# elizabethfong/SparkSmithWaterman

Hardware: AMD Instinct MI355X
Metric: GCUPS (higher is better)
Workload: dtype int32

## Files before the change

### include/swmi.h

```cpp
#ifndef SWMI_H
#define SWMI_H

#include <stddef.h>
#include <stdint.h>

#ifdef __cplusplus
extern "C" {
#endif

#define SWMI_ABI_VERSION 3

typedef enum swmi_status {
    SWMI_OK               =  0,
    SWMI_ERR_INVALID      = -1,
    SWMI_ERR_NO_DEVICE    = -2,
    SWMI_ERR_HIP          = -3,
    SWMI_ERR_NOMEM        = -4,
    SWMI_ERR_UNSUPPORTED  = -5,
    SWMI_ERR_RANGE        = -6
} swmi_status;

#define SWMI_ALIGN_LOCAL  0
#define SWMI_ALIGN_FIT    1
#define SWMI_ALIGN_GLOBAL 2

#define SWMI_TIE_SERIAL 0
#define SWMI_TIE_STRICT 1

typedef struct swmi_params {
    int32_t match;
    int32_t mismatch;
    int32_t gap;
    int32_t tie_mode;
    char    types[4];
} swmi_params;

typedef struct swmi_ctx    swmi_ctx;
typedef struct swmi_batch  swmi_batch;

int         swmi_abi_version(void);
const char *swmi_last_error(void);
int         swmi_device_count(int *count);
int         swmi_create(int device, swmi_ctx **out);
void        swmi_destroy(swmi_ctx *ctx);
void        swmi_default_params(swmi_params *p);

int         swmi_set_option(swmi_ctx *ctx, const char *name, int64_t value);

int         swmi_set_score_matrix(swmi_ctx *ctx, const uint8_t *alphabet, uint32_t n, const int32_t *scores);

int  swmi_batch_upload(swmi_ctx *ctx,
                       const uint8_t *ref_bytes, const uint64_t *ref_off, uint32_t n_refs,
                       const uint8_t *read_bytes, const uint64_t *read_off, uint32_t n_reads,
                       swmi_batch **out);
#define SWMI_SPEC_REVERSE 0x1u
#define SWMI_SPEC_WHOLE   0xFFFFFFFFu
typedef struct swmi_pair_spec {
    uint32_t ref, read;
    uint32_t ref_start, ref_len;
    uint32_t read_start, read_len;
    uint32_t flags;
    uint32_t reserved;
} swmi_pair_spec;
int  swmi_batch_upload_pairs(swmi_ctx *ctx,
                             const uint8_t *ref_bytes, const uint64_t *ref_off, uint32_t n_refs,
                             const uint8_t *read_bytes, const uint64_t *read_off, uint32_t n_reads,
                             const swmi_pair_spec *specs, uint64_t n_pairs, swmi_batch **out);
int  swmi_batch_set_pairs(swmi_ctx *ctx, swmi_batch *b, const swmi_pair_spec *specs, uint64_t n_pairs);
int  swmi_batch_pair_spec(const swmi_batch *b, uint64_t pair, swmi_pair_spec *spec);

int  swmi_batch_run(swmi_ctx *ctx, swmi_batch *b, const swmi_params *p);
void swmi_batch_free(swmi_ctx *ctx, swmi_batch *b);
int  swmi_batch_run_async(swmi_ctx *ctx, swmi_batch *b, const swmi_params *p);
int  swmi_batch_wait(swmi_ctx *ctx);

typedef struct swmi_timing {
    float    fill_ms, traceback_ms, d2h_ms, total_ms;
    uint32_t fill_launches, rerun_pairs;
    uint64_t cells;
    uint64_t dir_bytes;
    uint32_t strip_fallbacks;
    uint32_t col_chunks;
    uint32_t resident_pairs;
    uint32_t tfused_pairs;
} swmi_timing;
int  swmi_batch_timing(const swmi_batch *b, swmi_timing *t);
int  swmi_batch_mode(const swmi_batch *b, int *mode);

#define SWMI_PAIR_DEGENERATE 0x1u
#define SWMI_PAIR_TO_END     0x2u
uint64_t swmi_batch_n_pairs(const swmi_batch *b);
int      swmi_pair_score(const swmi_batch *b, uint64_t pair, int32_t *score);
int      swmi_pair_n_alignments(const swmi_batch *b, uint64_t pair, uint64_t *n, uint32_t *flags);
int      swmi_pair_rows_swept(const swmi_batch *b, uint64_t pair, uint32_t *rows);
int      swmi_pair_band_window(const swmi_batch *b, uint64_t pair, uint32_t strip, uint32_t *c_lo, uint32_t *c_hi);
int      swmi_batch_pair_results(const swmi_batch *b, int32_t *scores, uint64_t *n_alignments, uint64_t n);
int      swmi_pair_alignment(swmi_batch *b, uint64_t pair, uint64_t k,
                             int32_t *begin, int32_t *end_i, int32_t *end_j,
                             const char **ref_aln, const char **read_aln, uint32_t *len);
#define SWMI_CIGAR_M  0u
#define SWMI_CIGAR_I  1u
#define SWMI_CIGAR_D  2u
#define SWMI_CIGAR_EQ 7u
#define SWMI_CIGAR_X  8u
int      swmi_pair_cigar(swmi_batch *b, uint64_t pair, uint64_t k,
                         int32_t *begin, int32_t *end_i, int32_t *end_j,
                         const uint32_t **cigar, uint32_t *n_cigar, uint32_t *nm);

#define SWMI_SUBOPT_AUTO (-1)
int      swmi_pair_subopt(const swmi_batch *b, uint64_t pair, int32_t *score2, uint32_t *end2);
int      swmi_batch_pair_subopt(const swmi_batch *b, int32_t *score2, uint32_t *end2, uint64_t n);

typedef struct swmi_hit { int32_t score; uint32_t end_i, end_j, reserved; } swmi_hit;
int      swmi_pair_hits(const swmi_batch *b, uint64_t pair, swmi_hit *hits, uint32_t cap, uint32_t *n_hits);
int      swmi_batch_pair_hits(const swmi_batch *b, swmi_hit *hits, uint32_t cap_per_pair, uint32_t *n_hits, uint64_t n);

int      swmi_pair_end_score(const swmi_batch *b, uint64_t pair, int32_t *max_score, int32_t *end_score, uint32_t *end_col);
int      swmi_batch_pair_end_scores(const swmi_batch *b, int32_t *max_score, int32_t *end_score, uint32_t *end_col, uint64_t n);

int      swmi_batch_materialise_all(swmi_batch *b, uint64_t *n_alignments, uint64_t *n_chars);

int      swmi_ref_total(const swmi_batch *b, uint32_t ref, int32_t *total);
int      swmi_ref_totals(const swmi_batch *b, int32_t *totals, uint32_t n);
int      swmi_ref_n_match_sites(swmi_batch *b, uint32_t ref, uint64_t *n);
int      swmi_ref_match_site(swmi_batch *b, uint32_t ref, uint64_t k, int32_t *begin,
                             const char **ref_aln, const char **read_aln, uint32_t *len);

int      swmi_ref_sites_packed(swmi_batch *b, uint32_t ref_lo, uint32_t ref_hi,
                               int32_t *totals, uint64_t *degenerate, uint64_t *site_first,
                               int32_t *begins, uint32_t *lens, uint64_t *str_off, uint64_t sites_cap,
                               uint8_t *blob, uint64_t blob_cap, uint64_t *n_sites, uint64_t *blob_bytes);

int  swmi_align_batch(swmi_ctx *ctx, const swmi_params *p,
                      const uint8_t *ref_bytes, const uint64_t *ref_off, uint32_t n_refs,
                      const uint8_t *read_bytes, const uint64_t *read_off, uint32_t n_reads,
                      swmi_batch **out);

typedef struct swmi_stream swmi_stream;
typedef struct swmi_stream_stats {
    double   push_ms;
    double   parse_ms;
    double   upload_ms, run_ms;
    double   gpu_sweep_ms, gpu_traceback_ms;
    uint64_t bytes, cells;
    uint32_t chunks, pad;
} swmi_stream_stats;
int      swmi_stream_open(swmi_ctx *ctx, const swmi_params *p, const uint8_t *read_bytes, const uint64_t *read_off,
                          uint32_t n_reads, uint32_t slots, uint64_t chunk_bytes, swmi_stream **out);
int      swmi_stream_push(swmi_stream *s, const uint8_t *ref_bytes, const uint64_t *ref_off, uint32_t n_refs);
int      swmi_stream_push_file(swmi_stream *s, const char *path, const char *delimiter, uint32_t parse_threads);
int      swmi_stream_push_file_shard(swmi_stream *s, const char *path, const char *delimiter, uint32_t parse_threads,
                                     uint32_t shard, uint32_t n_shards);
int      swmi_stream_finish(swmi_stream *s);
uint64_t swmi_stream_n_refs(const swmi_stream *s);
uint32_t swmi_stream_n_chunks(const swmi_stream *s);
int      swmi_stream_chunk(swmi_stream *s, uint32_t k, swmi_batch **batch, uint64_t *first_ref);
int      swmi_stream_totals(const swmi_stream *s, int32_t *totals, uint64_t n);
int      swmi_stream_metadata(const swmi_stream *s, uint64_t ref, char *buf, size_t cap);
int      swmi_stream_ref_pos(const swmi_stream *s, uint64_t ref, uint64_t *pos);
int      swmi_stream_ref_sequence(const swmi_stream *s, uint64_t ref, uint8_t *buf, uint64_t cap, uint64_t *len);
int      swmi_stream_get_stats(const swmi_stream *s, swmi_stream_stats *st);
void     swmi_stream_close(swmi_stream *s);

#ifdef __cplusplus
}
#endif
#endif
```

### sparksmithwaterman_amd/_capi.py

```python
import ctypes as C
import os

_HERE = os.path.dirname(os.path.abspath(__file__))
LIB_PATH = os.environ.get("SWMI_LIB") or os.path.join(_HERE, "lib", "libswmi.so")

TIE_SERIAL = 0
TIE_STRICT = 1
ALIGN_LOCAL = 0
ALIGN_FIT = 1
ALIGN_GLOBAL = 2
BAND_MAX = 1 << 20
XDROP_MAX = (1 << 31) - 1
CIGAR_M, CIGAR_I, CIGAR_D, CIGAR_EQ, CIGAR_X = 0, 1, 2, 7, 8
CIGAR_CHARS = {CIGAR_M: "M", CIGAR_I: "I", CIGAR_D: "D", CIGAR_EQ: "=", CIGAR_X: "X"}
SUBOPT_AUTO = -1
END_BONUS_MAX = 1 << 30
HITS_MAX = 16
PAIR_DEGENERATE = 0x1
PAIR_TO_END = 0x2
SPEC_REVERSE = 0x1
SPEC_WHOLE = 0xFFFFFFFF
ERR_INVALID = -1
ERR_UNSUPPORTED = -5


class SwmiError(RuntimeError):
    def __init__(self, code, msg):
        super().__init__("swmi error %d: %s" % (code, msg))
        self.code = code


class Params(C.Structure):
    _fields_ = [("match", C.c_int32), ("mismatch", C.c_int32), ("gap", C.c_int32),
                ("tie_mode", C.c_int32), ("types", C.c_char * 4)]


class Timing(C.Structure):
    _fields_ = [("fill_ms", C.c_float), ("traceback_ms", C.c_float), ("d2h_ms", C.c_float),
                ("total_ms", C.c_float), ("fill_launches", C.c_uint32), ("rerun_pairs", C.c_uint32),
                ("cells", C.c_uint64), ("dir_bytes", C.c_uint64),
                ("strip_fallbacks", C.c_uint32), ("col_chunks", C.c_uint32),
                ("resident_pairs", C.c_uint32), ("tfused_pairs", C.c_uint32)]


class Hit(C.Structure):
    _fields_ = [("score", C.c_int32), ("end_i", C.c_uint32), ("end_j", C.c_uint32), ("reserved", C.c_uint32)]


class PairSpec(C.Structure):
    _fields_ = [("ref", C.c_uint32), ("read", C.c_uint32), ("ref_start", C.c_uint32), ("ref_len", C.c_uint32),
                ("read_start", C.c_uint32), ("read_len", C.c_uint32), ("flags", C.c_uint32), ("reserved", C.c_uint32)]


class StreamStats(C.Structure):
    _fields_ = [("push_ms", C.c_double), ("parse_ms", C.c_double), ("upload_ms", C.c_double), ("run_ms", C.c_double),
                ("gpu_sweep_ms", C.c_double), ("gpu_traceback_ms", C.c_double), ("bytes", C.c_uint64), ("cells", C.c_uint64),
                ("chunks", C.c_uint32), ("pad", C.c_uint32)]


_P = C.c_void_p
_u8p = C.POINTER(C.c_uint8)
_u64p = C.POINTER(C.c_uint64)
SYMBOLS = [
    ("swmi_abi_version", C.c_int, []),
    ("swmi_last_error", C.c_char_p, []),
    ("swmi_device_count", C.c_int, [C.POINTER(C.c_int)]),
    ("swmi_create", C.c_int, [C.c_int, C.POINTER(_P)]),
    ("swmi_destroy", None, [_P]),
    ("swmi_default_params", None, [C.POINTER(Params)]),
    ("swmi_set_option", C.c_int, [_P, C.c_char_p, C.c_int64]),
    ("swmi_set_score_matrix", C.c_int, [_P, C.c_char_p, C.c_uint32, C.POINTER(C.c_int32)]),
    ("swmi_batch_upload", C.c_int, [_P, C.c_char_p, _u64p, C.c_uint32, C.c_char_p, _u64p, C.c_uint32, C.POINTER(_P)]),
    ("swmi_batch_upload_pairs", C.c_int, [_P, C.c_char_p, _u64p, C.c_uint32, C.c_char_p, _u64p, C.c_uint32, C.POINTER(PairSpec),
                                          C.c_uint64, C.POINTER(_P)]),
    ("swmi_batch_set_pairs", C.c_int, [_P, _P, C.POINTER(PairSpec), C.c_uint64]),
    ("swmi_batch_pair_spec", C.c_int, [_P, C.c_uint64, C.POINTER(PairSpec)]),
    ("swmi_batch_run", C.c_int, [_P, _P, C.POINTER(Params)]),
    ("swmi_batch_run_async", C.c_int, [_P, _P, C.POINTER(Params)]),
    ("swmi_batch_wait", C.c_int, [_P]),
    ("swmi_batch_free", None, [_P, _P]),
    ("swmi_batch_timing", C.c_int, [_P, C.POINTER(Timing)]),
    ("swmi_batch_mode", C.c_int, [_P, C.POINTER(C.c_int)]),
    ("swmi_batch_n_pairs", C.c_uint64, [_P]),
    ("swmi_pair_score", C.c_int, [_P, C.c_uint64, C.POINTER(C.c_int32)]),
    ("swmi_pair_n_alignments", C.c_int, [_P, C.c_uint64, _u64p, C.POINTER(C.c_uint32)]),
    ("swmi_pair_alignment", C.c_int, [_P, C.c_uint64, C.c_uint64, C.POINTER(C.c_int32), C.POINTER(C.c_int32),
                                      C.POINTER(C.c_int32), C.POINTER(C.c_char_p), C.POINTER(C.c_char_p),
                                      C.POINTER(C.c_uint32)]),
    ("swmi_pair_cigar", C.c_int, [_P, C.c_uint64, C.c_uint64, C.POINTER(C.c_int32), C.POINTER(C.c_int32), C.POINTER(C.c_int32),
                                  C.POINTER(C.POINTER(C.c_uint32)), C.POINTER(C.c_uint32), C.POINTER(C.c_uint32)]),
    ("swmi_pair_rows_swept", C.c_int, [_P, C.c_uint64, C.POINTER(C.c_uint32)]),
    ("swmi_pair_band_window", C.c_int, [_P, C.c_uint64, C.c_uint32, C.POINTER(C.c_uint32), C.POINTER(C.c_uint32)]),
    ("swmi_batch_pair_results", C.c_int, [_P, C.POINTER(C.c_int32), _u64p, C.c_uint64]),
    ("swmi_pair_subopt", C.c_int, [_P, C.c_uint64, C.POINTER(C.c_int32), C.POINTER(C.c_uint32)]),
    ("swmi_batch_pair_subopt", C.c_int, [_P, C.POINTER(C.c_int32), C.POINTER(C.c_uint32), C.c_uint64]),
    ("swmi_pair_hits", C.c_int, [_P, C.c_uint64, C.POINTER(Hit), C.c_uint32, C.POINTER(C.c_uint32)]),
    ("swmi_batch_pair_hits", C.c_int, [_P, C.POINTER(Hit), C.c_uint32, C.POINTER(C.c_uint32), C.c_uint64]),
    ("swmi_pair_end_score", C.c_int, [_P, C.c_uint64, C.POINTER(C.c_int32), C.POINTER(C.c_int32), C.POINTER(C.c_uint32)]),
    ("swmi_batch_pair_end_scores", C.c_int, [_P, C.POINTER(C.c_int32), C.POINTER(C.c_int32), C.POINTER(C.c_uint32), C.c_uint64]),
    ("swmi_batch_materialise_all", C.c_int, [_P, _u64p, _u64p]),
    ("swmi_ref_total", C.c_int, [_P, C.c_uint32, C.POINTER(C.c_int32)]),
    ("swmi_ref_totals", C.c_int, [_P, C.POINTER(C.c_int32), C.c_uint32]),
    ("swmi_ref_n_match_sites", C.c_int, [_P, C.c_uint32, _u64p]),
    ("swmi_ref_match_site", C.c_int, [_P, C.c_uint32, C.c_uint64, C.POINTER(C.c_int32), C.POINTER(C.c_char_p),
                                      C.POINTER(C.c_char_p), C.POINTER(C.c_uint32)]),
    ("swmi_ref_sites_packed", C.c_int, [_P, C.c_uint32, C.c_uint32, C.POINTER(C.c_int32), _u64p, _u64p, C.POINTER(C.c_int32),
                                        C.POINTER(C.c_uint32), _u64p, C.c_uint64, C.c_void_p, C.c_uint64, _u64p, _u64p]),
    ("swmi_stream_open", C.c_int, [_P, C.POINTER(Params), C.c_char_p, _u64p, C.c_uint32, C.c_uint32, C.c_uint64, C.POINTER(_P)]),
    ("swmi_stream_push", C.c_int, [_P, C.c_char_p, _u64p, C.c_uint32]),
    ("swmi_stream_push_file", C.c_int, [_P, C.c_char_p, C.c_char_p, C.c_uint32]),
    ("swmi_stream_push_file_shard", C.c_int, [_P, C.c_char_p, C.c_char_p, C.c_uint32, C.c_uint32, C.c_uint32]),
    ("swmi_stream_finish", C.c_int, [_P]),
    ("swmi_stream_n_refs", C.c_uint64, [_P]),
    ("swmi_stream_n_chunks", C.c_uint32, [_P]),
    ("swmi_stream_chunk", C.c_int, [_P, C.c_uint32, C.POINTER(_P), _u64p]),
    ("swmi_stream_totals", C.c_int, [_P, C.POINTER(C.c_int32), C.c_uint64]),
    ("swmi_stream_metadata", C.c_int, [_P, C.c_uint64, C.c_char_p, C.c_size_t]),
    ("swmi_stream_ref_pos", C.c_int, [_P, C.c_uint64, _u64p]),
    ("swmi_stream_ref_sequence", C.c_int, [_P, C.c_uint64, C.c_void_p, C.c_uint64, _u64p]),
    ("swmi_stream_get_stats", C.c_int, [_P, C.POINTER(StreamStats)]),
    ("swmi_stream_close", None, [_P]),
    ("swmi_align_batch", C.c_int, [_P, C.POINTER(Params), C.c_char_p, _u64p, C.c_uint32, C.c_char_p, _u64p,
                                   C.c_uint32, C.POINTER(_P)]),
]

_lib = None


def load():
    global _lib
    if _lib is None:
        if not os.path.exists(LIB_PATH):
            raise ImportError(
                "%s is missing: build it with `python -c 'import __graft_entry__ as g; g.build()'` "
                "(hipcc, gfx950).  There is no CPU fallback." % LIB_PATH)
        lib = C.CDLL(LIB_PATH)
        for name, res, args in SYMBOLS:
            f = getattr(lib, name)
            f.restype = res
            f.argtypes = args
        _lib = lib
    return _lib


def check(rc):
    if rc != 0:
        raise SwmiError(rc, load().swmi_last_error().decode("utf-8", "replace"))


def as_bytes(s):
    return bytes(s) if isinstance(s, (bytes, bytearray, memoryview)) else s.encode("latin-1")


def pack(seqs):
    bs = [as_bytes(s) for s in seqs]
    off = (C.c_uint64 * (len(bs) + 1))()
    t = 0
    for k, b in enumerate(bs):
        off[k] = t
        t += len(b)
    off[len(bs)] = t
    return b"".join(bs), off
```

### sparksmithwaterman_amd/aligner.py

```python
import ctypes as C
import weakref

from . import _capi
from ._capi import Params, Timing, StreamStats, PairSpec, SwmiError, check

DEFAULT_SCORES = (5, -3, -4)
DEFAULT_TYPES = ("a", "i", "d", "-")
CIGAR_M, CIGAR_I, CIGAR_D, CIGAR_EQ, CIGAR_X = _capi.CIGAR_M, _capi.CIGAR_I, _capi.CIGAR_D, _capi.CIGAR_EQ, _capi.CIGAR_X


def cigar_string(entries):
    return "".join("%d%s" % (int(n), op) for n, op in entries)


def make_params(align_scores=None, align_types=None, tie_mode=_capi.TIE_SERIAL):
    sc = DEFAULT_SCORES if align_scores is None else tuple(int(x) for x in align_scores)
    ty = DEFAULT_TYPES if align_types is None else tuple(align_types)
    if len(sc) != 3 or len(ty) != 4:
        raise ValueError("alignScores needs 3 entries and alignTypes 4")
    p = Params()
    p.match, p.mismatch, p.gap = sc
    p.tie_mode = tie_mode
    p.types = b"".join(_capi.as_bytes(t)[:1] for t in ty)
    return p
# ... 69 lines not shown
    def set_score_matrix(self, alphabet, scores=None):
        from . import matrix as _matrix
        if isinstance(alphabet, _matrix.ScoreMatrix) and scores is None:
            alphabet, scores = alphabet.alphabet, alphabet.scores
        sym, flat = _matrix.validate(alphabet, scores)
        arr = (C.c_int32 * len(flat))(*flat)
        check(self._lib.swmi_set_score_matrix(self._h, sym, len(sym), arr))
        self.score_matrix = (sym, tuple(flat))

    def clear_score_matrix(self):
        check(self._lib.swmi_set_score_matrix(self._h, None, 0, None))
        self.score_matrix = None

    def upload(self, refs, reads):
        return Batch(self, refs, reads)

    def upload_pairs(self, refs, reads, pairs):
        return PairBatch(self, refs, reads, pairs)

    def stream(self, reads, params=None, slots=0, chunk_bytes=0):
        return Stream(self, reads, params, slots, chunk_bytes)

    def close(self):
        if getattr(self, "_h", None):
            self._lib.swmi_destroy(self._h)
            self._h = None

    def __del__(self):
        try:
            self.close()
        except Exception:
            pass


class Batch:

    _owned = True

    @classmethod
    def _view(cls, lib, handle, n_refs, n_reads, owner):
        b = cls.__new__(cls)
        b._ctx, b._lib, b._h, b.n_refs, b.n_reads, b._owned = None, lib, handle, n_refs, n_reads, False
        b._owner = owner
        return b

    def __init__(self, ctx, refs, reads):
        self._ctx = ctx
        self._lib = ctx._lib
        self.n_refs, self.n_reads = len(refs), len(reads)
        rb, ro = _capi.pack(refs)
        qb, qo = _capi.pack(reads)
        h = C.c_void_p()
        check(self._lib.swmi_batch_upload(ctx._h, rb, ro, self.n_refs, qb, qo, self.n_reads, C.byref(h)))
        self._h = h

    def n_pairs(self):
        return self.n_refs * self.n_reads

    def run(self, params=None):
        p = params if params is not None else make_params()
        check(self._lib.swmi_batch_run(self._ctx._h, self._h, C.byref(p)))
        return self

    def run_async(self, params=None):
        p = params if params is not None else make_params()
        self._async_params = p
        check(self._lib.swmi_batch_run_async(self._ctx._h, self._h, C.byref(p)))
        return self

    def wait(self):
        check(self._lib.swmi_batch_wait(self._ctx._h))
        return self

    def timing(self):
        t = Timing()
        check(self._lib.swmi_batch_timing(self._h, C.byref(t)))
        return t

    def pipeline_mode(self):
        v = C.c_int()
        check(self._lib.swmi_batch_mode(self._h, C.byref(v)))
        return v.value

    def score(self, pair):
        v = C.c_int32()
        check(self._lib.swmi_pair_score(self._h, pair, C.byref(v)))
        return v.value

    def n_alignments(self, pair):
        n, f = C.c_uint64(), C.c_uint32()
        check(self._lib.swmi_pair_n_alignments(self._h, pair, C.byref(n), C.byref(f)))
        return n.value, f.value

    def rows_swept(self, pair):
        v = C.c_uint32()
        check(self._lib.swmi_pair_rows_swept(self._h, pair, C.byref(v)))
        return v.value

    def band_window(self, pair, strip):
        lo, hi = C.c_uint32(), C.c_uint32()
        check(self._lib.swmi_pair_band_window(self._h, pair, strip, C.byref(lo), C.byref(hi)))
        return lo.value, hi.value

    def alignment(self, pair, k, with_cell=False):
        b, ei, ej = C.c_int32(), C.c_int32(), C.c_int32()
        r, q, ln = C.c_char_p(), C.c_char_p(), C.c_uint32()
        check(self._lib.swmi_pair_alignment(self._h, pair, k, C.byref(b), C.byref(ei), C.byref(ej),
                                            C.byref(r), C.byref(q), C.byref(ln)))
        rec = (b.value, (r.value.decode("latin-1"), q.value.decode("latin-1")))
        return rec + ((ei.value, ej.value),) if with_cell else rec

    def alignments(self, pair, with_cell=False):
        n, _ = self.n_alignments(pair)
        return [self.alignment(pair, k, with_cell) for k in range(n)]

    def cigar(self, pair, k):
        b, ei, ej = C.c_int32(), C.c_int32(), C.c_int32()
        p, n, nm = C.POINTER(C.c_uint32)(), C.c_uint32(), C.c_uint32()
        check(self._lib.swmi_pair_cigar(self._h, pair, k, C.byref(b), C.byref(ei), C.byref(ej), C.byref(p), C.byref(n), C.byref(nm)))
        ent = [(p[x] >> 4, _capi.CIGAR_CHARS.get(p[x] & 15, "?")) for x in range(n.value)]
        return b.value, ei.value, ej.value, ent, nm.value

    def cigars(self, pair):
        n, _ = self.n_alignments(pair)
        return [self.cigar(pair, k) for k in range(n)]

    def pair_results(self):
        import numpy as np
        n = self.n_pairs()
        sc = np.empty(n, dtype=np.int32)
        na = np.empty(n, dtype=np.uint64)
        check(self._lib.swmi_batch_pair_results(self._h, sc.ctypes.data_as(C.POINTER(C.c_int32)),
                                                na.ctypes.data_as(C.POINTER(C.c_uint64)), n))
        return sc, na

    def scores(self):
        import numpy as np
        n = self.n_pairs()
        sc = np.empty(n, dtype=np.int32)
        check(self._lib.swmi_batch_pair_results(self._h, sc.ctypes.data_as(C.POINTER(C.c_int32)), None, n))
        return sc

    def subopt(self, pair):
        s2, e2 = C.c_int32(), C.c_uint32()
        check(self._lib.swmi_pair_subopt(self._h, pair, C.byref(s2), C.byref(e2)))
        return s2.value, e2.value

    def subopts(self):
        import numpy as np
        n = self.n_pairs()
        s2 = np.empty(n, dtype=np.int32)
        e2 = np.empty(n, dtype=np.uint32)
        check(self._lib.swmi_batch_pair_subopt(self._h, s2.ctypes.data_as(C.POINTER(C.c_int32)),
                                               e2.ctypes.data_as(C.POINTER(C.c_uint32)), n))
        return s2, e2

    def hits(self, pair):
        n = C.c_uint32()
        arr = (_capi.Hit * _capi.HITS_MAX)()
        check(self._lib.swmi_pair_hits(self._h, pair, arr, _capi.HITS_MAX, C.byref(n)))
        return [(arr[k].score, arr[k].end_i, arr[k].end_j) for k in range(n.value)]

    def hits_all(self, k=_capi.HITS_MAX):
        import numpy as np
        n = self.n_pairs()
        cnt = np.empty(n, dtype=np.uint32)
# ... 235 lines not shown
```

### sparksmithwaterman_amd/csrc/swmi_ctx.cpp

```cpp
#include <cstdarg>
#include <cstdio>
#include <cstdlib>

#include "swmi_host.h"
#include "swmi_launch.h"

static thread_local std::string g_err;

int swmi_host::fail(int code, const char *fmt, ...) {
    char buf[512];
    va_list ap;
    va_start(ap, fmt);
    vsnprintf(buf, sizeof buf, fmt, ap);
    va_end(ap);
    g_err = buf;
    return code;
}

int swmi_io_fail(int code, const std::string &msg) { return fail(code, "%s", msg.c_str()); }

static const uint8_t *code_table();

extern "C" int swmi_abi_version(void) { return SWMI_ABI_VERSION; }

// ... 35 lines not shown
    if (device < 0 || device >= n) return fail(SWMI_ERR_INVALID, "device %d out of range [0,%d)", device, n);
    hipDeviceProp_t prop;
    e = hipGetDeviceProperties(&prop, device);
    if (e != hipSuccess) return fail(SWMI_ERR_NO_DEVICE, "hipGetDeviceProperties: %s", hipGetErrorString(e));
    if (strncmp(prop.gcnArchName, "gfx950", 6) != 0)
        return fail(SWMI_ERR_NO_DEVICE, "device %d is %s; the kernels are built for gfx950 (MI355X) only",
                    device, prop.gcnArchName);
    e = hipSetDevice(device);
    if (e != hipSuccess) return fail(SWMI_ERR_NO_DEVICE, "hipSetDevice: %s", hipGetErrorString(e));
    swmi_ctx *c = new swmi_ctx;
    c->device = device;
    e = hipStreamCreateWithFlags(&c->stream, hipStreamNonBlocking);
    if (e != hipSuccess) { c->stream = nullptr; ctx_release(c); return fail(SWMI_ERR_HIP, "hipStreamCreate: %s", hipGetErrorString(e)); }
    for (auto &ev : c->ev) {
        e = hipEventCreate(&ev);
        if (e != hipSuccess) { ev = nullptr; ctx_release(c); return fail(SWMI_ERR_HIP, "hipEventCreate: %s", hipGetErrorString(e)); }
    }
    { int r = c->h_err.reserve(64); if (r) { ctx_release(c); return r; } }
    { static const char *ee = getenv("SWMI_EXT_EVENTS"); if (ee) c->ext_events = atoi(ee) != 0; }
    *(volatile uint32_t *)c->h_err.p = 0u;
    { int r = c->d_lut.reserve(256); if (r) { ctx_release(c); return r; } }
    e = hipMemcpy(c->d_lut.p, code_table(), 256, hipMemcpyHostToDevice);
    if (e != hipSuccess) { ctx_release(c); return fail(SWMI_ERR_HIP, "code table upload: %s", hipGetErrorString(e)); }
    *out = c;
    return SWMI_OK;
}

extern "C" void swmi_destroy(swmi_ctx *ctx) {
    if (!ctx) return;
    (void)hipSetDevice(ctx->device);
    if (ctx->worker.joinable()) {
        {
            std::unique_lock<std::mutex> lk(ctx->job_mu);
            ctx->job_cv.wait(lk, [&] { return ctx->job_state.load() != 1; });
            ctx->job_state.store(3);
        }
        ctx->job_cv.notify_all();
        ctx->worker.join();
    }
    ctx_release(ctx);
}

extern "C" int swmi_set_option(swmi_ctx *ctx, const char *name, int64_t value) {
    if (!ctx || !name) return fail(SWMI_ERR_INVALID, "null argument");
    std::lock_guard<std::mutex> g(ctx->mu);
    if (!strcmp(name, "cell_cap")) {
        if (value < 1 || value > (1 << 20)) return fail(SWMI_ERR_INVALID, "cell_cap out of range");
        ctx->cell_cap = (uint32_t)value;
        ctx->cell_cap_set = true;
    } else if (!strcmp(name, "max_workspace_bytes")) {
        if (value < (1 << 20)) return fail(SWMI_ERR_INVALID, "max_workspace_bytes too small");
        ctx->max_workspace_bytes = (uint64_t)value;
    } else if (!strcmp(name, "mode")) {
        if (value < -1 || value > 2) return fail(SWMI_ERR_INVALID, "mode must be -1 (automatic), 0, 1 or 2");
        ctx->mode = value < 0 ? 1u : (uint32_t)value;
    } else if (!strcmp(name, "auto_ties_x100")) {
        if (value < 100) return fail(SWMI_ERR_INVALID, "auto_ties_x100 out of range");
        ctx->auto_ties_x100 = (uint32_t)value;
    } else if (!strcmp(name, "spin_us")) {
        if (value < 0) return fail(SWMI_ERR_INVALID, "spin_us out of range");
        ctx->spin_us = value;
    } else if (!strcmp(name, "debug_strip_spins")) {
        ctx->dbg_strip_spins = (uint32_t)value;
    } else if (!strcmp(name, "debug_reverse_strips")) {
        ctx->dbg_reverse_strips = value != 0;
    } else if (!strcmp(name, "debug_async_delay_us")) {
        if (value < 0 || value > 10000000) return fail(SWMI_ERR_INVALID, "debug_async_delay_us out of range");
        ctx->dbg_async_delay_us = (uint32_t)value;
    } else if (!strcmp(name, "tfused")) {
        if (value < -1 || value > 1) return fail(SWMI_ERR_INVALID, "tfused must be -1 (automatic), 0 or 1");
        ctx->tfused = (int)value;
    } else if (!strcmp(name, "resident")) {
        if (value < -1 || value > 1) return fail(SWMI_ERR_INVALID, "resident must be -1 (automatic), 0 or 1");
        ctx->resident = (int)value;
    } else if (!strcmp(name, "scores_only")) {
        ctx->scores_only = value != 0;
    } else if (!strcmp(name, "stream_keep_records")) {
        ctx->stream_keep_records = value != 0;
    } else if (!strcmp(name, "device_strings")) {
        ctx->device_strings = value != 0;
    } else if (!strcmp(name, "tb_split")) {
        if (value < -1 || value > 1) return fail(SWMI_ERR_INVALID, "tb_split must be -1 (automatic), 0 or 1");
        ctx->tb_split = (int)value;
    } else if (!strcmp(name, "col_chunks")) {
        if (value < 0 || value > 4096) return fail(SWMI_ERR_INVALID, "col_chunks out of range");
        ctx->col_chunks = (uint32_t)value;
    } else if (!strcmp(name, "zero_copy")) {
        ctx->zero_copy = value != 0;
    } else if (!strcmp(name, "profiling")) {
        if (value < 0 || value > 2) return fail(SWMI_ERR_INVALID, "profiling must be 0, 1 (every stage) or 2 (the sweep only)");
        ctx->profiling = (int)value;
    } else if (!strcmp(name, "gap_open")) {
        if (value > 0) return fail(SWMI_ERR_INVALID, "gap_open must be <= 0 (a penalty), got %lld", (long long)value);
        if (value < INT32_MIN) return fail(SWMI_ERR_INVALID, "gap_open out of range");
        ctx->gap_open = (int32_t)value;
    } else if (!strcmp(name, "affine")) {
        if (value != -1 && value != 1) return fail(SWMI_ERR_INVALID, "affine must be -1 (when gap_open != 0) or 1 (always)");
        ctx->affine = (int)value;
    } else if (!strcmp(name, "align_mode")) {
        if (value != SWMI_ALIGN_LOCAL && value != SWMI_ALIGN_FIT && value != SWMI_ALIGN_GLOBAL)
            return fail(SWMI_ERR_INVALID, "align_mode must be 0 (local), 1 (fit) or 2 (global), got %lld", (long long)value);
        ctx->modes.align_mode = (int)value;
    } else if (!strcmp(name, "long_reads")) {
        if (value != 0 && value != 1) return fail(SWMI_ERR_INVALID, "long_reads must be 0 or 1, got %lld", (long long)value);
        ctx->modes.long_reads = (int)value;
    } else if (!strcmp(name, "band")) {
        if (value < 0 || value > (int64_t)SWMI_AFF_BAND_MAX)
            return fail(SWMI_ERR_INVALID, "band must be 0 (none) or a half-width of 1 .. %u columns, got %lld", SWMI_AFF_BAND_MAX, (long long)value);
        ctx->modes.band = (int)value;
    } else if (!strcmp(name, "extend")) {
        if (value != 0 && value != 1) return fail(SWMI_ERR_INVALID, "extend must be 0 or 1, got %lld", (long long)value);
        ctx->modes.extend = (int)value;
    } else if (!strcmp(name, "xdrop")) {
        if (value < 0 || value > 0x7FFFFFFFll)
            return fail(SWMI_ERR_INVALID, "xdrop must be 0 (off) or a threshold of 1 .. 2^31 - 1, got %lld", (long long)value);
        ctx->modes.xdrop = (int)value;
    } else if (!strcmp(name, "band_adapt")) {
        if (value != 0 && value != 1) return fail(SWMI_ERR_INVALID, "band_adapt must be 0 or 1, got %lld", (long long)value);
        ctx->modes.band_adapt = (int)value;
    } else if (!strcmp(name, "gap_open2")) {
        if (value > 0) return fail(SWMI_ERR_INVALID, "gap_open2 must be <= 0 (a penalty; 0: one-piece gaps), got %lld", (long long)value);
        if (value < INT32_MIN) return fail(SWMI_ERR_INVALID, "gap_open2 out of range");
        ctx->modes.gap_open2 = (int)value;
    } else if (!strcmp(name, "gap2")) {
        if (value > 0) return fail(SWMI_ERR_INVALID, "gap2 must be <= 0 (the second piece's per-base extension), got %lld", (long long)value);
        if (value < INT32_MIN) return fail(SWMI_ERR_INVALID, "gap2 out of range");
        ctx->modes.gap2 = (int)value;
    } else if (!strcmp(name, "cigar")) {
        if (value < 0 || value > 2) return fail(SWMI_ERR_INVALID, "cigar must be 0 (off), 1 (M/I/D) or 2 (=/X/I/D), got %lld", (long long)value);
        ctx->modes.cigar = (int)value;
    } else if (!strcmp(name, "subopt")) {
        if (value < SWMI_SUBOPT_AUTO || value > (1ll << 30))
            return fail(SWMI_ERR_INVALID, "subopt must be 0 (off), a mask half-width of 1 .. 2^30 columns or -1 (SWMI_SUBOPT_AUTO), got %lld", (long long)value);
        ctx->modes.subopt = (int)value;
    } else if (!strcmp(name, "hits")) {
        if (value < 0 || value > (int64_t)SWMI_HITS_MAX)
            return fail(SWMI_ERR_INVALID, "hits must be 0 (off) or 1 .. %u entries per pair, got %lld", SWMI_HITS_MAX, (long long)value);
        ctx->modes.hits = (int)value;
    } else if (!strcmp(name, "end_bonus")) {
        if (value < 0 || value > (1ll << 30))
            return fail(SWMI_ERR_INVALID, "end_bonus must be 0 (off) or a bonus of 1 .. 2^30, got %lld", (long long)value);
        ctx->modes.end_bonus = (int)value;
    } else if (!strcmp(name, "arena_words_per_pair")) {
        if (value < 1) return fail(SWMI_ERR_INVALID, "arena_words_per_pair out of range");
        ctx->arena_words_per_pair = (uint64_t)value;
    } else {
        return fail(SWMI_ERR_INVALID, "unknown option '%s'", name);
    }
    return SWMI_OK;
}

extern "C" int swmi_set_score_matrix(swmi_ctx *ctx, const uint8_t *alphabet, uint32_t n, const int32_t *scores) {
    if (!ctx) return fail(SWMI_ERR_INVALID, "null context");
    if (n == 0) {
        std::lock_guard<std::mutex> g(ctx->mat_mu);
        ctx->matrix.reset();
        return SWMI_OK;
    }
    if (n > SWMI_MAT_MAX_SYMBOLS) return fail(SWMI_ERR_INVALID, "a score matrix has at most %u symbols, got %u", SWMI_MAT_MAX_SYMBOLS, n);
    if (!alphabet || !scores) return fail(SWMI_ERR_INVALID, "alphabet or scores is null");
    const uint8_t *T = code_table();
    uint32_t cls[256];
    for (uint32_t c = 0; c < 256; c++) cls[c] = n;
    for (uint32_t i = 0; i < n; i++) {
        const uint8_t c = T[alphabet[i]];
        if (cls[c] != n)
// ... 277 lines not shown
```

### sparksmithwaterman_amd/csrc/swmi_device.h

```cpp
#pragma once
#include <stdint.h>

#if defined(__HIPCC__)
#define SWMI_HD __host__ __device__
#else
#define SWMI_HD
#endif

#define SWMI_SEQ_PAD_WORDS 24u
#define SWMI_RMAX          4
#ifndef SWMI_CK_BLOCKS
#define SWMI_CK_BLOCKS     2u
#endif
#define SWMI_CODE_PAD      0x1FFu

#define SWMI_LDS_BYTES (160u * 1024u)
#define SWMI_EMIT_SCRATCH_WORDS 128u
#define SWMI_TB_BLOCKS 16u
#define SWMI_TB_REFWIN_WORDS 96u
#define SWMI_RES_CELL_CAP 128u

#define SWMI_DIR_D 0u
#define SWMI_DIR_I 1u
#define SWMI_DIR_A 2u

#define SWMI_F_DEGENERATE   0x1u
#define SWMI_F_CELL_OVF     0x2u
#define SWMI_F_ARENA_OVF    0x4u
#define SWMI_F_DONE         0x8u
#define SWMI_F_TO_END       0x10u
#define SWMI_F_STRIPS_SHIFT 8u
#define SWMI_F_STRIPS_MASK  0xFFFFFF00u

struct SeqDesc {
    uint32_t len;
    uint32_t boff;
    uint32_t acgt;
    uint32_t pad;
};

struct PairDesc {
    uint32_t ref_id;
    uint32_t read_id;
    uint32_t out_id;
    uint32_t pad;
    uint64_t dir_off;
    uint64_t seam_off;
};

#define SWMI_PAD_COLS 0x80000000u
#define SWMI_PAD_RESIDENT 0x40000000u

struct ColItem {
    uint32_t pair;
    uint32_t col0;
    uint32_t g_lo, g_hi;
};

struct StripItem {
    uint32_t pair, strip;
    uint32_t col0, g_lo, g_hi;
    uint32_t prog;
    uint32_t priv_stride;
    uint32_t pad;
    uint64_t priv_off;
};

struct PairOut {
    int32_t  score;
    uint32_t flags;
    uint64_t n_cells;
};

struct EndOut {
    int32_t  max_score;
    int32_t  end_score;
    uint32_t end_col;
};

struct AlnRec {
    uint32_t out_id;
    uint32_t rank;
    int32_t  begin;
    int32_t  end_i, end_j;
    uint32_t n_ops;
    uint32_t off_lo, off_hi;
};
#define SWMI_RECTAB_WORDS 8u

struct ArenaHdr {
    unsigned long long reserved;
    unsigned long long pad;
};
#define SWMI_HDR_WORD_BITS 36u
#define SWMI_HDR_WORD_MASK ((1ull << SWMI_HDR_WORD_BITS) - 1ull)

struct FillArgs {
    const uint32_t *seqw;
    const SeqDesc  *refs;
    const SeqDesc  *reads;
    const PairDesc *pairs;
    uint32_t       *dir;
    int32_t        *seam;
    PairOut        *out;
    uint2          *cells;
    const uint64_t *cells_off;
    const uint32_t *cells_cap;
    ArenaHdr       *hdr;
    unsigned long long *dbg;
    uint32_t        dbg_thr0;
    uint32_t        dbg_pad;
    uint32_t        n_pairs;
    uint32_t        cell_cap;
    int32_t         match, mismatch, gap;
    uint32_t        strict;
    uint32_t        mode;
    uint32_t        skip_multi;
    const StripItem *strip_items;
    uint32_t       *progress;
    uint32_t        n_strip_items;
    uint32_t        n_out;
    uint32_t       *err_host;
    const ColItem  *col_items;
    uint32_t        n_col_items;
    uint32_t        strip_spins;
    uint32_t       *q_reset;
};

struct TraceArgs {
    const uint32_t *seqw;
    const SeqDesc  *refs;
    const SeqDesc  *reads;
    const PairDesc *pairs;
    const uint32_t *dir;
    PairOut        *out;
    const uint2    *cells;
    const uint64_t *cells_off;
    const uint32_t *cells_cap;
    ArenaHdr       *hdr;
    uint32_t       *arena;
    uint64_t        arena_cap_words;
    uint32_t        n_pairs;
    uint32_t        cell_cap;
    int32_t         match, mismatch, gap;
    uint32_t        strict;
    uint32_t        lds_words;
    uint32_t        lds_read_words;
    unsigned long long *dbg;
    const int32_t  *seam;
    PairOut        *out_host;
    uint32_t       *ovf_host;
    uint32_t        mode;
    uint32_t        pad2;
    const uint32_t *win_off;
    uint32_t       *q_count;
    uint4          *q_items;
    uint32_t        q_cap;
    uint32_t        pad4;
    const uint8_t  *raw;
    const uint64_t *raw_off;
    uint32_t        raw_reads_at;
    uint32_t        rec_tab_cap;
    AlnRec         *rec_tab;
};

struct ResidentArgs {
    const uint32_t *res_items;
    uint32_t        n_res;
    uint32_t        res_lds_words;
    uint32_t        res_cell_cap;
    uint32_t        res_ops_words;
};

struct TFusedArgs {
    const uint32_t *items;
    uint32_t        n_items;
    uint32_t        lds_words;
    uint32_t        tile_words;
    uint32_t        cell_cap;
    uint32_t        pad0;
    uint32_t        ref_words;
    uint32_t        read_words;
    uint32_t        stage_words;
    uint32_t        debug_marks;
    uint32_t        n_helpers;
};
#define SWMI_TF_HELPERS 2u
#define SWMI_TF_BMAX   40u
#ifndef SWMI_TF_BR
#define SWMI_TF_BR     4u
#endif
#define SWMI_TF_MAX_M  256u
SWMI_HD static inline uint32_t swmi_tf_cols_per_lane(uint32_t n) {
    uint32_t b = (n + 63u) / 64u;
    b = (b + 1u) & ~1u;
    return b < 2u ? 2u : b;
}
SWMI_HD static inline uint64_t swmi_tf_ck_words(uint32_t m) { return ((uint64_t)m + 64u) * 64u; }

#define SWMI_RANK_BY_CELL 0xFFFFFFFFu
#define SWMI_DETECT_LCAP  64u

SWMI_HD static inline uint32_t swmi_rows_per_lane(uint32_t m) {
    uint32_t r = (m + 63u) / 64u;
    return r < 1u ? 1u : (r > SWMI_RMAX ? SWMI_RMAX : r);
}
SWMI_HD static inline uint64_t swmi_dir_words(uint32_t m, uint32_t n, uint32_t mode, bool tfused = false) {
    uint32_t R = swmi_rows_per_lane(m);
    uint64_t strips = ((uint64_t)m + 64u * R - 1u) / (64u * R);
    uint64_t wblocks = ((uint64_t)n + 63u + 15u) / 16u;
    if (mode == 0) return strips * wblocks * R * 64u;
    uint64_t n_ck = (wblocks + SWMI_CK_BLOCKS - 1u) / SWMI_CK_BLOCKS;
    uint64_t words = strips * (n_ck * (R + 2u) * 64u + (mode == 1 ? ((n_ck + 63u) & ~(uint64_t)63u) : 0u));
    if (tfused && mode == 1 && m <= 256u && n <= 64u * 40u && ((uint64_t)m + 64u) * 64u > words) words = ((uint64_t)m + 64u) * 64u;
    return words;
}
#define SWMI_AFF_RMAX     16u
#define SWMI_AFF_MAX_READ (64u * SWMI_AFF_RMAX)
#define SWMI_AFF_TB_SLOTS 4u
#define SWMI_AFF_TILE_WORDS 4096u
SWMI_HD static inline uint32_t swmi_aff_rows_per_lane(uint32_t m) {
    uint32_t r = (m + 63u) / 64u;
    return r < 1u ? 1u : r;
}
SWMI_HD static inline uint32_t swmi_aff_blocks(uint32_t m, uint32_t n) {
    const uint32_t R = swmi_aff_rows_per_lane(m), lact = m ? (m + R - 1u) / R : 1u;
    return (uint32_t)(((uint64_t)n + lact - 1u + 7u) / 8u);
}
SWMI_HD static inline uint32_t swmi_aff_strips(uint32_t m) { return m ? (m + SWMI_AFF_MAX_READ - 1u) / SWMI_AFF_MAX_READ : 1u; }
SWMI_HD static inline uint32_t swmi_aff_strip_blocks(uint32_t n) { return (uint32_t)(((uint64_t)n + 63u + 7u) / 8u); }
SWMI_HD static inline uint64_t swmi_aff_strip_words(uint32_t n) { return (uint64_t)swmi_aff_strip_blocks(n) * SWMI_AFF_RMAX * 64u; }
#define SWMI_AFF_BAND_MAX (1u << 20)
#define SWMI_AFF_BAND_NEG (-2013265920)
SWMI_HD static inline uint32_t swmi_aff_band_lo(uint32_t s, uint32_t w) {
    const uint64_t a = (uint64_t)SWMI_AFF_MAX_READ * s;
    return a > w ? (uint32_t)(a + 1u - w) : 1u;
}
SWMI_HD static inline uint32_t swmi_aff_band_hi(uint32_t s, uint32_t n, uint32_t w) {
    const uint64_t a = (uint64_t)SWMI_AFF_MAX_READ * ((uint64_t)s + 1u) + w;
    return a < n ? (uint32_t)a : n;
}
SWMI_HD static inline uint32_t swmi_aff_band_blocks(uint32_t s, uint32_t n, uint32_t w) {
    return swmi_aff_strip_blocks(swmi_aff_band_hi(s, n, w) - swmi_aff_band_lo(s, w) + 1u);
}
SWMI_HD static inline uint64_t swmi_aff_band_blocks_before(uint32_t s, uint32_t n, uint32_t w) {
    const uint64_t sa = (uint64_t)w / SWMI_AFF_MAX_READ + 1u;
// ... 58 lines not shown
```

### sparksmithwaterman_amd/csrc/swmi_diag.cpp

```cpp
#include <chrono>
#include <cstdio>
#include <cstdlib>
#include <unistd.h>

#include "swmi_host.h"

int swmi_host::dump_traceback_diagnostics(swmi_batch *b, const TraceArgs &ta, size_t np, size_t n_tf) {
    if (!ta.dbg) return SWMI_OK;
    std::vector<unsigned long long> d(np * 4);
    HIP_TRY(hipMemcpy(d.data(), ta.dbg, np * 32, hipMemcpyDeviceToHost));
    if (n_tf) {
        double t0 = 0, t1 = 0, t2 = 0, t3 = 0, t4 = 0, t5 = 0; unsigned long long mx = 0;
        for (size_t k = 0; k < np; k++) {
            t0 += d[4*k]; t1 += d[4*k+1] & 0xFFFFFFFFull; t2 += d[4*k+1] >> 32; t3 += d[4*k+2] >> 16; t4 += d[4*k+3] >> 32; t5 += d[4*k+3] & 0xFFFFFFFFull;
            mx = std::max(mx, d[4*k]);
        }
        fprintf(stderr, "[swmi tfused dbg] ticks per sweeper wavefront: lifetime mean=%.0f max=%llu = prologue %.0f + sweep %.0f + first block task %.0f (%.2f block tasks per wavefront) + waiting for tasks %.0f + rest (more tasks, walk items) %.0f\n",
                t0 / np, mx, t2 / np, t1 / np, t3 / np, t5 / np, t4 / np, (t0 - t1 - t2 - t3 - t4) / np);
        {
            std::vector<size_t> idx(np);
            for (size_t k = 0; k < np; k++) idx[k] = k;
            std::sort(idx.begin(), idx.end(), [&](size_t x, size_t y) { return d[4 * x] < d[4 * y]; });
            auto at = [&](double q) { return d[4 * idx[std::min<size_t>(np - 1, (size_t)(q * np))]]; };
            fprintf(stderr, "[swmi tfused dbg]   lifetime p10=%llu p50=%llu p90=%llu p99=%llu max=%llu\n", at(0.10), at(0.50), at(0.90), at(0.99), d[4 * idx[np - 1]]);
            for (size_t t = 0; t < std::min<size_t>(np, 6); t++) {
                const size_t k = idx[np - 1 - t];
                fprintf(stderr, "[swmi tfused dbg]   slow wavefront (pair %zu): lifetime %llu, sweep %llu, first block task %llu, block tasks taken %llu, waiting %llu, alignments of its pair %llu\n",
                        k, d[4 * k], d[4 * k + 1] & 0xFFFFFFFFull, d[4 * k + 2] >> 16, d[4 * k + 3] & 0xFFFFFFFFull, d[4 * k + 3] >> 32,
                        (unsigned long long)((const PairOut *)((const uint8_t *)b->h_result.p + result_out_off()))[k].n_cells);
            }
        }
    }
    double a0 = 0, a1 = 0, a2 = 0, a3 = 0; unsigned long long mx = 0;
    double a4 = 0;
    for (size_t k = 0; k < np; k++) { a0 += d[4*k]; a1 += d[4*k+1] & 0xFFFFFFFFull; a2 += d[4*k+2] & 0xFFFF; a4 += d[4*k+2] >> 16; a3 += d[4*k+3] & 0xFFFFFFFFull; mx = std::max(mx, d[4*k]); }
    fprintf(stderr, "[swmi tb dbg] wave ticks mean=%.0f max=%llu; walk ticks mean=%.0f; staging ticks mean=%.0f; steps mean=%.1f; iterations mean=%.2f\n",
            a0 / np, mx, a1 / np, a4 / np, a2 / np, a3 / np);
    const PairOut *po_dbg = (const PairOut *)((const uint8_t *)b->h_result.p + result_out_off());
    double cs[4] = {0, 0, 0, 0}, cw[4] = {0, 0, 0, 0}; unsigned long long cm[4] = {0, 0, 0, 0}; size_t cn[4] = {0, 0, 0, 0};
    for (size_t k = 0; k < np; k++) {
        const size_t c = std::min<uint64_t>(po_dbg[k].n_cells, 4) - (po_dbg[k].n_cells ? 1 : 0);
        cs[c] += d[4 * k]; cw[c] += d[4 * k + 1] & 0xFFFFFFFFull; cm[c] = std::max(cm[c], d[4 * k]); cn[c]++;
    }
    {
        std::vector<size_t> idx(np);
        for (size_t k = 0; k < np; k++) idx[k] = k;
        const size_t top = std::min<size_t>(np, 6);
        std::partial_sort(idx.begin(), idx.begin() + top, idx.end(), [&](size_t x, size_t y) { return d[4 * x] > d[4 * y]; });
        for (size_t t = 0; t < top; t++)
            fprintf(stderr, "[swmi tb dbg]   slow pair %zu: ticks=%llu walk=%llu staging=%llu in %llu stagings, steps=%llu iterations=%llu alignments=%llu\n", idx[t],
                    d[4 * idx[t]], d[4 * idx[t] + 1] & 0xFFFFFFFFull, d[4 * idx[t] + 2] >> 16, d[4 * idx[t] + 3] >> 32, d[4 * idx[t] + 2] & 0xFFFF,
                    d[4 * idx[t] + 3] & 0xFFFFFFFFull, (unsigned long long)po_dbg[idx[t]].n_cells);
        for (size_t t = 0; t < top; t++)
            fprintf(stderr, "[swmi tb dbg]     ... of the staging time of pair %zu, %llu ticks waiting for helpers\n", idx[t], d[4 * idx[t] + 1] >> 32);
    }
    for (int c = 0; c < 4; c++)
        if (cn[c]) fprintf(stderr, "[swmi tb dbg]   %d%s alignment(s): %zu pairs, wave ticks mean=%.0f max=%llu, walk(slot 0) mean=%.0f\n",
                           c + 1, c == 3 ? "+" : "", cn[c], cs[c] / cn[c], cm[c], cw[c] / cn[c]);
    return SWMI_OK;
}

int swmi_host::dump_fill_diagnostics(swmi_batch *b, const FillArgs &fa, size_t np) {
    if (!fa.dbg) return SWMI_OK;
    std::vector<unsigned long long> d(np * 2);
    HIP_TRY(hipMemcpy(d.data(), fa.dbg, np * 16, hipMemcpyDeviceToHost));
#ifdef SWMI_STRIP_DIAG
    for (size_t k = 0; k < np && k < 8; k++)
        fprintf(stderr, "[swmi strip dbg] pair %zu: strip 0 lifetime %llu ticks, %llu waiting before publications; strip 1 lifetime %llu, "
                "%llu polls, %llu ticks in polls, %llu waiting for seam groups\n", k, d[2 * k] >> 32, d[2 * k] & 0xFFFFFFFFull,
                d[2 * k + 1] >> 40, (d[2 * k + 1] >> 32) & 0xFF, (d[2 * k + 1] >> 16) & 0xFFFF, d[2 * k + 1] & 0xFFFF);
#endif
    unsigned long long ev = 0, cyc = 0, evmax = 0, cmax = 0, cmin = ~0ull;
    for (size_t k = 0; k < np; k++) {
        ev += d[2 * k]; cyc += d[2 * k + 1];
        evmax = std::max(evmax, d[2 * k]); cmax = std::max(cmax, d[2 * k + 1]); cmin = std::min(cmin, d[2 * k + 1]);
    }
    fprintf(stderr, "[swmi fill dbg] pairs=%zu slow-path entries mean=%.1f max=%llu; wave ticks mean=%.0f min=%llu max=%llu\n",
            np, (double)ev / np, evmax, (double)cyc / np, cmin, cmax);
    if (b->eff_mode == 1) {
        std::unordered_map<unsigned long long, int> per_simd, per_cu;
        for (size_t k = 0; k < np; k++) {
            const unsigned long long hw = d[2 * k] & 0xFFFFFFFFull, xcc = (d[2 * k] >> 32) & 0xF;
            const unsigned long long simd = (hw >> 4) & 3, cu = (hw >> 8) & 15, sh = (hw >> 12) & 1, se = (hw >> 13) & 7;
            const unsigned long long cukey = (xcc << 16) | (se << 8) | (sh << 4) | cu;
            per_cu[cukey]++; per_simd[(cukey << 4) | simd]++;
        }
        int h_simd[9] = {0}, h_cu[17] = {0};
        for (auto &kv : per_simd) h_simd[std::min(kv.second, 8)]++;
        for (auto &kv : per_cu) h_cu[std::min(kv.second, 16)]++;
        fprintf(stderr, "[swmi fill dbg] placement: %zu CUs, %zu SIMDs used; SIMDs by waves held: 1:%d 2:%d 3:%d 4+:%d; CUs by waves held: 1-4:%d 5-8:%d 9+:%d\n",
                per_cu.size(), per_simd.size(), h_simd[1], h_simd[2], h_simd[3], h_simd[4] + h_simd[5] + h_simd[6] + h_simd[7] + h_simd[8],
                h_cu[1] + h_cu[2] + h_cu[3] + h_cu[4], h_cu[5] + h_cu[6] + h_cu[7] + h_cu[8], h_cu[9] + h_cu[10] + h_cu[11] + h_cu[12] + h_cu[13] + h_cu[14] + h_cu[15] + h_cu[16]);
    }
    return SWMI_OK;
}

void swmi_host::watchdog_wait(hipStream_t st, const swmi_batch *b, const char *limit_s) {
    const auto w0 = std::chrono::steady_clock::now();
    while (hipStreamQuery(st) == hipErrorNotReady)
        if (std::chrono::duration<double>(std::chrono::steady_clock::now() - w0).count() > atof(limit_s)) {
            const volatile uint32_t *hm = (const volatile uint32_t *)b->h_result.p;
            fprintf(stderr, "[swmi watchdog] launch still running after %s s; marks:", limit_s);
            for (int k = 0; k < 12; k++) fprintf(stderr, " %08x", hm ? hm[k] : 0u);
            fprintf(stderr, "\n");
            fflush(stderr);
            _exit(3);
        }
}
```

### sparksmithwaterman_amd/csrc/swmi_host.h

```cpp
#pragma once
#include <hip/hip_runtime.h>

#include <algorithm>
#include <atomic>
#include <condition_variable>
#include <cstdint>
#include <cstring>
#include <memory>
#include <mutex>
#include <string>
#include <thread>
#include <type_traits>
#include <unordered_map>
#include <vector>

#include "../../include/swmi.h"
#include "swmi_device.h"
#include "swmi_io_internal.h"

namespace swmi_host __attribute__((visibility("hidden"))) {
int fail(int code, const char *fmt, ...);
int check_offsets(const uint64_t *off, uint32_t n, const char *what);
int upload_device(swmi_ctx *ctx, swmi_batch *b, hipStream_t st, const uint8_t *ref_src, const uint8_t *read_src);
int settle_raw(swmi_batch *b);
// ... 45 lines not shown
        if (e != hipSuccess) { (void)hipHostFree(p); p = nullptr; return fail(SWMI_ERR_HIP, "hipHostGetDevicePointer: %s", hipGetErrorString(e)); }
        cap = bytes;
        return SWMI_OK;
    }
    void release() { if (p) (void)hipHostFree(p); p = nullptr; dp = nullptr; cap = 0; }
    PinnedBuf() = default;
    PinnedBuf(const PinnedBuf &) = delete;
    PinnedBuf &operator=(const PinnedBuf &) = delete;
    ~PinnedBuf() { release(); }
};

struct ScoreMatrix {
    uint64_t gen = 0;
    uint32_t n = 0;
    int32_t max_entry = 0;
    std::vector<uint32_t> image;
};

struct __attribute__((visibility("hidden"))) RunModes {
    int align_mode = SWMI_ALIGN_LOCAL;
    int long_reads = 0;
    int band = 0;
    int extend = 0;
    int xdrop = 0;
    int band_adapt = 0;
    int gap_open2 = 0;
    int gap2 = 0;
    int cigar = 0;
    int subopt = 0;
    int hits = 0;
    int end_bonus = 0;
    bool two_piece() const { return gap_open2 != 0; }
    uint32_t kernel_mode() const { return extend && align_mode == SWMI_ALIGN_GLOBAL ? 3u : (uint32_t)align_mode; }
    bool operator==(const RunModes &o) const { return memcmp(this, &o, sizeof(RunModes)) == 0; }
};
static_assert(std::has_unique_object_representations_v<RunModes>, "RunModes is compared bytewise: no padding, no floating point");
static inline int64_t swmi_adapt_low(uint64_t m, uint64_t n, int64_t gap_open, int64_t gap) {
    const int64_t ns = (int64_t)((m + SWMI_AFF_MAX_READ - 1) / SWMI_AFF_MAX_READ);
    return (2 * ns + 1) * gap_open + (ns * (int64_t)SWMI_AFF_MAX_READ + (int64_t)n) * gap;
}
static inline bool swmi_adapt_bound_ok(uint64_t m, uint64_t n, int64_t gap_open, int64_t gap) {
    return swmi_adapt_low(m, n, gap_open, gap) >= -((int64_t)1 << 30);
}
static inline AffGeom aff_geom(const RunModes &md) {
    return AffGeom{md.band > 0 ? (uint32_t)md.band : 0u, md.band > 0 && md.band_adapt != 0, md.two_piece(), md.subopt != 0, md.subopt != 0 && md.hits != 0};
}
struct __attribute__((visibility("hidden"))) SchedKey {
    int eff_mode = -1;
    bool tfused = false;
    AffGeom geom{};
    SchedKey() = default;
    SchedKey(uint32_t mode, bool tf, const RunModes &md) : eff_mode((int)mode), tfused(tf), geom(mode == 3 ? aff_geom(md) : AffGeom{}) {}
    bool operator==(const SchedKey &o) const { return eff_mode == o.eff_mode && tfused == o.tfused && geom == o.geom; }
};
struct __attribute__((visibility("hidden"))) RunOptions {
    RunModes modes;
    std::shared_ptr<const ScoreMatrix> mat;
};

struct swmi_ctx {
    int device = 0;
    hipStream_t stream = nullptr;
    std::mutex mu;
    uint32_t cell_cap = 64;
    uint64_t max_workspace_bytes = 32ull << 30;
    int profiling = 0;
    uint32_t mode = 1;
    int zero_copy = 1;
    uint64_t arena_words_per_pair = 160;
    uint64_t arena_copy_wpp = 160;
    uint64_t recs_per_pair_x16 = 32;
    hipEvent_t ev[6] = {nullptr, nullptr, nullptr, nullptr, nullptr, nullptr};
    PinnedBuf h_err;
    DevBuf d_hdr_ring;
    uint32_t hdr_next = 0;
    DevBuf d_lut;
    int64_t spin_us = 2000;
    uint32_t dbg_strip_spins = 0;
    uint32_t dbg_reverse_strips = 0;
    uint32_t dbg_async_delay_us = 0;
    uint32_t auto_ties_x100 = 300;
    uint32_t col_chunks = 0;
    int tb_split = -1;
    bool ext_events = false;
    int tfused = -1;
    int resident = -1;
    int scores_only = 0;
    int stream_keep_records = 1;
    int device_strings = 1;
    bool cell_cap_set = false;
    int32_t gap_open = 0;
    int affine = -1;
    RunModes modes;
    std::mutex mat_mu;
    std::shared_ptr<const ScoreMatrix> matrix;
    std::thread worker;
    std::mutex job_mu;
    std::condition_variable job_cv;
    std::atomic<int> job_state{0};
    swmi_batch *job_batch = nullptr;
    swmi_params job_params{};
    RunOptions job_opt;
    uint32_t job_delay_us = 0;
    int job_rc = 0;
    std::string job_err;
};

static inline RunOptions run_options(swmi_ctx *ctx) {
    std::lock_guard<std::mutex> g(ctx->mat_mu);
    return RunOptions{ctx->modes, ctx->matrix};
}

struct HostAln {
    uint32_t rank;
    int32_t begin, end_i, end_j;
    uint32_t n_ops;
    const uint32_t *rec = nullptr;
    int64_t str_id = -1;
};

struct PairRes {
    int32_t score = 0;
    uint32_t flags = 0;
    uint64_t n_cells = 0;
    uint32_t strips = 0;
    uint64_t first = 0;
    uint64_t count = 0;
};

struct SiteRef { uint64_t pair; uint64_t k; int32_t begin; };

struct Work {
    uint32_t pair;
    uint64_t cells;
    uint64_t dir_words;
    uint64_t seam_words;
};

struct __attribute__((visibility("hidden"))) PlanKey {
    bool valid = false;
    size_t lo = 0, hi = 0;
    const void *work = nullptr;
    swmi_params params{};
    uint32_t eff_mode = 0;
    uint32_t col_chunks = 0;
    bool reverse_strips = false;
    int resident = -1, tfused = -1;
    bool exact = false;
    bool scores_only = false;
    uint64_t mat_gen = 0;
    RunModes modes;
    const void *d_pairs = nullptr;
    size_t pairs_bytes = 0;
    bool operator==(const PlanKey &o) const {
        return valid == o.valid && lo == o.lo && hi == o.hi && work == o.work && memcmp(&params, &o.params, sizeof(swmi_params)) == 0 &&
               eff_mode == o.eff_mode && col_chunks == o.col_chunks && reverse_strips == o.reverse_strips && resident == o.resident &&
               tfused == o.tfused && exact == o.exact && scores_only == o.scores_only && mat_gen == o.mat_gen &&
               modes == o.modes && d_pairs == o.d_pairs && pairs_bytes == o.pairs_bytes;
    }
};

struct __attribute__((visibility("hidden"))) ChunkPlan {
    uint64_t dir_words = 0, seam_words = 0;
    uint64_t seam_priv_words = 0;
    uint32_t max_path = 0, max_read = 0;
    size_t n_strip_items = 0;
    size_t n_strip_chunks = 0;
    size_t n_col_items = 0;
    uint64_t n_windows = 0;
    size_t n_res = 0;
    uint32_t res_lds_words = 0, res_ops_words = 0;
    size_t n_tf = 0;
    uint32_t tf_max_m = 0, tf_max_n = 0, tf_max_path = 0;
    uint32_t aff_r_min = 0xFFFFFFFFu, aff_r_max = 0;
    size_t aff_n_long = 0;
};

struct swmi_batch {
    uint32_t n_refs = 0, n_reads = 0;
    bool paired = false;
    uint32_t n_src_refs = 0, n_src_reads = 0;
    std::vector<swmi_pair_spec> specs;
    bool sources_on_device = false;
    DevBuf d_src_off;
    std::vector<uint8_t> ref_bytes, read_bytes;
    const uint8_t *src_map = nullptr;
    std::vector<swmi_io_recpos> src_recs;
    std::unordered_map<uint32_t, std::vector<uint8_t>> src_cache;
    std::vector<uint64_t> ref_off, read_off;
    std::vector<SeqDesc> ref_desc, read_desc;
    DevBuf d_raw, d_raw_off;
    DevBuf d_seqw, d_refs, d_reads, d_pairs, d_dir, d_seam, d_result, d_cells, d_cells_off, d_cells_cap, d_dbg, d_dbg2;
    DevBuf d_strip_items, d_progress;
    DevBuf d_col_items;
    DevBuf d_win_off, d_queue;
    DevBuf d_tf_items;
    DevBuf d_res_items;
    bool views_built = false;
    bool tb_split_used = false;
    bool acgt_known = false;
    PinnedBuf h_result;
    swmi_params params{};
    bool has_run = false;
    int auto_choice = -1;
    swmi_params auto_params{};
    std::vector<Work> work;
    SchedKey work_key;
    uint32_t eff_mode = 1;
    int32_t gap_open = 0;
    RunOptions opt;
    DevBuf d_mat;
    uint64_t d_mat_gen = 0;
    uint64_t work_cells = 0;
    std::vector<uint8_t> pairs_on_device;
    const void *pairs_dev_ptr = nullptr;
    PlanKey plan_key;
    ChunkPlan plan;
    std::vector<PairRes> pairs;
    bool has_sub = false;
    std::vector<SuboptOut> sub;
    int hits_k = 0;
    std::vector<HitEnt> hitv;
    bool has_endb = false;
    std::vector<EndOut> endv;
    std::vector<uint32_t> win_tab;
    std::vector<uint64_t> win_at;
    struct RawChunk { size_t at, words; size_t tab_at, n_rec; size_t lo; std::vector<uint32_t> wpos; };
    std::vector<uint32_t> raw;
    std::vector<AlnRec> rtab;
    const uint32_t *raw_ext = nullptr;
    const AlnRec *rtab_ext = nullptr;
    uint64_t raw_ext_records = 0, raw_ext_cap = 0;
    std::vector<RawChunk> raw_chunks;
    bool indexed = false;
    bool rec_strings = false;
    int rec_cigar = 0;
    bool scores_only = false;
    bool records_dropped = false;
    std::vector<HostAln> alns;
    std::vector<char> str_buf;
    std::vector<uint64_t> str_at;
    std::vector<int8_t> ref_view_ready;
    std::vector<std::vector<SiteRef>> ref_sites;
    std::vector<uint64_t> ref_degenerate;
    swmi_timing timing{};
};

static inline uint64_t batch_n_pairs(const swmi_batch *b) { return b->paired ? (uint64_t)b->n_refs : (uint64_t)b->n_refs * b->n_reads; }
static inline uint32_t pair_ref(const swmi_batch *b, uint64_t pair) { return b->paired ? (uint32_t)pair : (uint32_t)(pair / b->n_reads); }
static inline uint32_t pair_read(const swmi_batch *b, uint64_t pair) { return b->paired ? (uint32_t)pair : (uint32_t)(pair % b->n_reads); }

struct RunState {
    swmi_ctx *ctx;
    swmi_batch *b;
    FillArgs fa{};
    TraceArgs ta{};
    float fill_ms = 0, tb_ms = 0, d2h_ms = 0;
    uint32_t launches = 0;
    double enqueue_us = 0, wait_us = 0, copyout_us = 0, prep_us = 0, prep_upload_us = 0;
    bool one_wave_sweep = false;
    bool tb_split = false;
    bool defer_copy = false;
    bool keep = true;
};

static inline size_t result_out_off() { return 64; }
static inline size_t result_sub_off(size_t np) { return 64 + np * sizeof(PairOut); }
static inline size_t result_hits_off(size_t np) { return result_sub_off(np) + np * sizeof(SuboptOut); }
static inline size_t result_tab_off(size_t np, size_t sub) { return (64 + np * (sizeof(PairOut) + sub) + 255) & ~(size_t)255; }
static inline size_t result_arena_off(size_t np, uint64_t tab_cap, size_t sub) { return (result_tab_off(np, sub) + tab_cap * sizeof(AlnRec) + 255) & ~(size_t)255; }
static inline uint64_t rec_words(uint32_t n_ops, bool strings) {
    return strings ? 2 * ((uint64_t)n_ops / 4 + 1) : ((uint64_t)n_ops + 15) / 16;
}
static inline bool payload_end(const swmi_batch *b, const AlnRec &e, const uint32_t *arena, uint64_t words, uint64_t &end) {
    const uint64_t off = ((uint64_t)e.off_hi << 32) | e.off_lo;
    if (!b->rec_cigar) { end = off + rec_words(e.n_ops, b->rec_strings); return end <= words; }
    if (off + 2 > words || off + 2 < off) return false;
    end = off + 2 + arena[off];
    return end <= words;
}
// ... 1 lines not shown
```

### sparksmithwaterman_amd/csrc/swmi_launch.h

```cpp
#pragma once
#include <hip/hip_runtime.h>
#include <stdint.h>
#include "swmi_device.h"

template <class K>
static inline void swmi_allow_big_lds(K kernel) {
    (void)hipFuncSetAttribute(reinterpret_cast<const void *>(kernel), hipFuncAttributeMaxDynamicSharedMemorySize, 160 * 1024);
}

extern "C" hipError_t swmi_launch_fill(const FillArgs *a, hipStream_t st, hipEvent_t ev_start, hipEvent_t ev_stop);
extern "C" hipError_t swmi_launch_traceback(const TraceArgs *a, hipStream_t st, hipEvent_t ev_start, hipEvent_t ev_stop);
extern "C" hipError_t swmi_launch_traceback_split(const TraceArgs *a, uint32_t n_windows, hipStream_t st);
extern "C" hipError_t swmi_launch_resident(const TraceArgs *a, const ResidentArgs *x, hipStream_t st);
extern "C" hipError_t swmi_launch_tfused(const TraceArgs *a, const TFusedArgs *x, hipStream_t st);
struct AffRun {
    int32_t gap_open;
    int32_t gap_open2, gap2;
    uint32_t mode;
    uint32_t band;
    uint32_t xdrop;
    uint32_t adapt;
    const uint32_t *mat;
    uint32_t nn;
    uint32_t cigar;
    int32_t subopt;
    uint32_t hits;
    uint32_t end_bonus;
};
enum : uint32_t {
    AFF_F_MATRIX = 1u << 0, AFF_F_LONG = 1u << 1, AFF_F_BAND = 1u << 2, AFF_F_XDROP = 1u << 3, AFF_F_ADAPT = 1u << 4,
    AFF_F_TWO = 1u << 5, AFF_F_SUBOPT = 1u << 6, AFF_F_ENDB = 1u << 7, AFF_F_HITS = 1u << 8
};
constexpr uint32_t aff_flags(bool matrix, bool lng, bool band, bool xdrop, bool adapt, bool two, bool subopt, bool endb, bool hits) {
    return (matrix ? AFF_F_MATRIX : 0u) | (lng ? AFF_F_LONG : 0u) | (band ? AFF_F_BAND : 0u) | (xdrop ? AFF_F_XDROP : 0u) |
           (adapt ? AFF_F_ADAPT : 0u) | (two ? AFF_F_TWO : 0u) | (subopt ? AFF_F_SUBOPT : 0u) | (endb ? AFF_F_ENDB : 0u) | (hits ? AFF_F_HITS : 0u);
}
constexpr uint32_t aff_key(uint32_t shape, uint32_t mode, uint32_t flags) { return flags | mode << 9 | shape << 11; }
constexpr bool aff_flags_ok(uint32_t mode, uint32_t f) {
    const bool xdrop_or_adapt = f & (AFF_F_XDROP | AFF_F_ADAPT);
    if (mode > 3u) return false;
    if ((f & AFF_F_BAND) && !(f & AFF_F_LONG)) return false;
    if ((f & AFF_F_XDROP) && !((f & AFF_F_LONG) && mode == 3u)) return false;
    if ((f & AFF_F_ADAPT) && !((f & AFF_F_BAND) && mode == 3u)) return false;
    if ((f & AFF_F_TWO) && (mode < 2u || (f & AFF_F_MATRIX) || xdrop_or_adapt)) return false;
    if ((f & AFF_F_SUBOPT) && mode != 0u) return false;
    if ((f & AFF_F_HITS) && !(f & AFF_F_SUBOPT)) return false;
    if ((f & AFF_F_ENDB) && (mode != 3u || xdrop_or_adapt || (f & AFF_F_TWO))) return false;
    return true;
}
static inline uint32_t aff_run_flags(const AffRun &r, uint32_t long_reads) {
    return aff_flags(r.mat != nullptr, long_reads != 0u, long_reads && r.band, long_reads && r.xdrop, long_reads && r.adapt,
                     r.gap_open2 != 0, r.subopt != 0, r.end_bonus != 0u, r.hits != 0u);
}
static inline bool aff_run_ok(const AffRun &r, uint32_t long_reads) {
    if (r.band > SWMI_AFF_BAND_MAX || r.xdrop > 0x7FFFFFFFu || r.adapt > 1u || r.cigar > 2u) return false;
    if (r.mat && (r.nn < 2u || r.nn > SWMI_MAT_NN_MAX)) return false;
    if (r.subopt < -1 || r.subopt > (1 << 30) || r.hits > SWMI_HITS_MAX || r.end_bonus > (1u << 30)) return false;
    if ((r.gap_open2 || r.end_bonus) && (r.xdrop || r.adapt)) return false;
    return aff_flags_ok(r.mode, aff_run_flags(r, long_reads));
}
extern "C" int swmi_affine_run_ok(const AffRun *r, uint32_t long_reads);
extern "C" const char *swmi_affine_sweep_name(const AffRun *r, uint32_t long_reads, uint32_t shape);
extern "C" const char *swmi_affine_traceback_name(const AffRun *r, uint32_t long_reads);
extern "C" hipError_t swmi_launch_affine_sweep(const FillArgs *a, const AffRun *r, uint32_t long_reads, uint32_t r_min, uint32_t r_max,
                                               hipStream_t st);
extern "C" hipError_t swmi_launch_affine_traceback(const TraceArgs *a, const AffRun *r, uint32_t long_reads, uint32_t tile_words,
                                                   uint32_t ops_words, hipStream_t st);
struct SuboptArgs {
    const SeqDesc *refs, *reads;
    const PairDesc *pairs;
    const uint32_t *dir;
    const PairOut *out;
    SuboptOut *sub;
    SuboptOut *sub_host;
    uint32_t n_pairs;
    uint32_t band;
    int32_t subopt;
};
extern "C" hipError_t swmi_launch_subopt(const SuboptArgs *a, hipStream_t st);
struct HitsArgs {
    SuboptArgs s;
    HitEnt *hits;
    HitEnt *hits_host;
    uint32_t k;
};
extern "C" hipError_t swmi_launch_hits(const HitsArgs *a, hipStream_t st);
extern "C" hipError_t swmi_launch_encode(const uint8_t *raw, const uint64_t *raw_off, SeqDesc *desc, uint32_t *seqw,
                                         const uint8_t *lut, uint32_t n_seq, hipStream_t st);
extern "C" hipError_t swmi_launch_gather(uint8_t *raw, const uint64_t *src_off, const uint64_t *raw_off, SeqDesc *desc, uint32_t *seqw,
                                         const uint8_t *lut, uint32_t n_seg, hipStream_t st);
```

### sparksmithwaterman_amd/csrc/swmi_run.cpp

```cpp
#include <chrono>
#include <cstdio>
#include <cstdlib>
#include <functional>
#include <numeric>

#include "swmi_host.h"
#include "swmi_launch.h"
#include "swmi_plan.h"

static int keep_chunk_records(RunState &rs, const AlnRec *tab, uint64_t n_rec, const uint32_t *arena, uint64_t arena_cap, size_t lo) {
    swmi_batch *b = rs.b;
    if (rs.defer_copy && b->raw_chunks.empty()) {
        b->raw_ext = arena; b->rtab_ext = tab; b->raw_ext_records = n_rec; b->raw_ext_cap = arena_cap;
        b->raw_chunks.push_back(swmi_batch::RawChunk{0, 0, 0, (size_t)n_rec, lo, {}});
        return SWMI_OK;
    }
    uint64_t used = 0;
    for (uint64_t k = 0; k < n_rec; k++) {
        uint64_t end;
        if (!payload_end(b, tab[k], arena, arena_cap, end)) return fail(SWMI_ERR_HIP, "record payloads overrun the arena");
        used = std::max(used, end);
    }
    b->raw_chunks.push_back(swmi_batch::RawChunk{b->raw.size(), (size_t)used, b->rtab.size(), (size_t)n_rec, lo, {}});
    b->raw.insert(b->raw.end(), arena, arena + used);
    b->rtab.insert(b->rtab.end(), tab, tab + n_rec);
    return SWMI_OK;
}

namespace {
struct Launch {
    size_t np = 0, lo = 0;
    const std::vector<uint64_t> *cells_exact = nullptr;
    std::vector<uint64_t> coff;
    std::vector<uint32_t> ccap;
    uint32_t cell_cap = 0;
    uint64_t cells_total = 0;
    bool split = false;
    bool zc = false;
    bool sweep_only = false;
    bool sub = false;
    bool endb = false;
    uint32_t hits = 0;
    size_t hit_bytes() const { return hits ? (1u + hits) * sizeof(HitEnt) : 0; }
    size_t sub_bytes() const { return sub ? sizeof(SuboptOut) + hit_bytes() : endb ? sizeof(EndOut) : 0; }
    bool time_all = false;
    uint64_t arena_cap = 0, tab_cap = 0;
    int attempt = 0;
    uint8_t *res = nullptr;
    size_t t_off = 0, a_off = 0;
    uint64_t q_cap = 0;
    bool whole_only = false;
    bool ext_timing = false;
    uint64_t copy_words = 0, copy_recs = 0;
};
}

static inline bool dbg_fill_on() {
    static const bool on = getenv("SWMI_DEBUG_FILL") != nullptr;
    return on;
}

static int size_cell_lists(RunState &rs, Launch &L) {
    swmi_ctx *ctx = rs.ctx;
    swmi_batch *b = rs.b;
    const size_t np = L.np;
    int rc;
    L.cell_cap = ctx->cell_cap;
    if (L.cells_exact) {
        L.coff.resize(np); L.ccap.resize(np);
        for (size_t k = 0; k < np; k++) {
            L.coff[k] = L.cells_total;
            L.ccap[k] = (uint32_t)std::min<uint64_t>((*L.cells_exact)[L.lo + k], 0xFFFFFFFFu);
            L.cells_total += L.ccap[k];
        }
        if ((rc = b->d_cells_off.reserve(np * 8))) return rc;
        if ((rc = b->d_cells_cap.reserve(np * 4))) return rc;
        HIP_TRY(hipMemcpyAsync(b->d_cells_off.p, L.coff.data(), np * 8, hipMemcpyHostToDevice, ctx->stream));
        HIP_TRY(hipMemcpyAsync(b->d_cells_cap.p, L.ccap.data(), np * 4, hipMemcpyHostToDevice, ctx->stream));
    } else {
        if (!ctx->cell_cap_set) L.cell_cap = (uint32_t)std::min<uint64_t>(65536, std::max<uint64_t>(L.cell_cap, (4ull << 20) / np));
        L.cells_total = (uint64_t)np * L.cell_cap;
    }
    return b->d_cells.reserve(std::max<uint64_t>(L.cells_total, 1) * sizeof(uint2));
}

static int build_fill_args(RunState &rs, Launch &L) {
    swmi_ctx *ctx = rs.ctx;
    swmi_batch *b = rs.b;
    const ChunkPlan &plan = b->plan;
    int rc;
    FillArgs &fa = rs.fa;
    fa.seqw = b->d_seqw.as<uint32_t>();
    fa.refs = b->d_refs.as<SeqDesc>();
    fa.reads = b->d_reads.as<SeqDesc>();
    fa.pairs = b->d_pairs.as<PairDesc>();
    fa.dir = b->d_dir.as<uint32_t>();
    fa.seam = b->d_seam.as<int32_t>();
    fa.out = (PairOut *)(L.res + result_out_off());
    fa.cells = b->d_cells.as<uint2>();
    fa.cells_off = L.cells_exact ? b->d_cells_off.as<uint64_t>() : nullptr;
    fa.cells_cap = L.cells_exact ? b->d_cells_cap.as<uint32_t>() : nullptr;
    fa.hdr = (ArenaHdr *)L.res;
    fa.dbg = nullptr;
    fa.dbg_pad = 0;
    if (dbg_fill_on()) {
        if ((rc = b->d_dbg.reserve(L.np * 16))) return rc;
        fa.dbg = b->d_dbg.as<unsigned long long>();
        fa.dbg_thr0 = getenv("SWMI_DEBUG_THR0") ? (uint32_t)atoi(getenv("SWMI_DEBUG_THR0")) : 1u;
        fa.dbg_pad = getenv("SWMI_DEBUG_SKIP") ? 1u : 0u;
    }
    fa.n_pairs = (uint32_t)L.np;
    fa.cell_cap = L.cell_cap;
    fa.match = b->params.match; fa.mismatch = b->params.mismatch; fa.gap = b->params.gap;
    fa.strict = b->params.tie_mode == SWMI_TIE_STRICT;
    fa.mode = b->eff_mode;
    const bool pipe = plan.n_strip_items && !rs.one_wave_sweep;
    fa.skip_multi = pipe ? 1u : 0u;
    fa.strip_items = pipe ? b->d_strip_items.as<StripItem>() : nullptr;
    fa.progress = pipe ? b->d_progress.as<uint32_t>() : nullptr;
    fa.n_strip_items = pipe ? (uint32_t)plan.n_strip_items : 0u;
    fa.err_host = (uint32_t *)ctx->h_err.dp;
    fa.n_out = (uint32_t)L.np;
    if (L.attempt == 0) b->timing.col_chunks += (uint32_t)plan.n_col_items + (pipe ? (uint32_t)plan.n_strip_chunks : 0u);
    fa.col_items = plan.n_col_items ? b->d_col_items.as<ColItem>() : nullptr;
    fa.n_col_items = (uint32_t)plan.n_col_items;
    fa.strip_spins = ctx->dbg_strip_spins;
    L.q_cap = std::min<uint64_t>(std::max<uint64_t>(L.cells_total, 1), 1ull << 24);
    if (L.split && (rc = b->d_queue.reserve(256 + L.q_cap * sizeof(uint4)))) return rc;
    fa.q_reset = L.split ? b->d_queue.as<uint32_t>() : nullptr;
    return SWMI_OK;
}

static int build_trace_args(RunState &rs, Launch &L) {
    swmi_ctx *ctx = rs.ctx;
    swmi_batch *b = rs.b;
    const ChunkPlan &plan = b->plan;
    const FillArgs &fa = rs.fa;
    int rc;
    TraceArgs &ta = rs.ta;
    ta.seqw = fa.seqw; ta.refs = fa.refs; ta.reads = fa.reads; ta.pairs = fa.pairs;
    ta.dir = fa.dir; ta.out = fa.out; ta.cells = fa.cells;
    ta.cells_off = fa.cells_off; ta.cells_cap = fa.cells_cap;
    ta.hdr = (ArenaHdr *)L.res;
    ta.arena = (uint32_t *)(L.res + L.a_off);
    ta.arena_cap_words = L.arena_cap;
    ta.rec_tab = (AlnRec *)(L.res + L.t_off);
    ta.rec_tab_cap = (uint32_t)std::min<uint64_t>(L.tab_cap, 0xFFFFFFFFu);
    ta.n_pairs = fa.n_pairs; ta.cell_cap = fa.cell_cap;
    ta.match = fa.match; ta.mismatch = fa.mismatch; ta.gap = fa.gap; ta.strict = fa.strict;
    ta.lds_words = (plan.max_path + 3) / 4 + 1;
    ta.seam = fa.seam;
    ta.mode = b->eff_mode;
    ta.pad2 = 0;
    ta.lds_read_words = (plan.max_read + 3) / 4 + 1;
    ta.out_host = nullptr;
    ta.ovf_host = (uint32_t *)ctx->h_err.dp + 4;
    ((volatile uint32_t *)ctx->h_err.p)[4] = 0u; ((volatile uint32_t *)ctx->h_err.p)[5] = 0u;
    ta.win_off = nullptr; ta.q_count = nullptr; ta.q_items = nullptr; ta.q_cap = 0; ta.pad4 = 0;
    const int cigar = b->eff_mode == 3 ? b->opt.modes.cigar : 0;
    const bool strings = !cigar && ctx->device_strings != 0 && b->d_raw.p != nullptr;
    ta.raw = strings ? b->d_raw.as<uint8_t>() : nullptr;
    ta.raw_off = strings ? b->d_raw_off.as<uint64_t>() : nullptr;
    ta.raw_reads_at = b->n_refs + 1u;
    b->rec_strings = strings;
    b->rec_cigar = cigar;
    if (L.zc) {
        if ((rc = b->h_result.reserve(L.a_off + L.arena_cap * 4))) return rc;
        uint8_t *hd = (uint8_t *)b->h_result.dp;
        *(volatile uint32_t *)b->h_result.p = 0u;
        ((volatile uint32_t *)b->h_result.p)[1] = 0u;
        ta.ovf_host = (uint32_t *)hd;
        ta.out_host = (PairOut *)(hd + result_out_off());
        ta.arena = (uint32_t *)(hd + L.a_off);
        ta.rec_tab = (AlnRec *)(hd + L.t_off);
    }
    ta.dbg = nullptr;
    if (dbg_fill_on()) {
        if ((rc = b->d_dbg2.reserve(L.np * 32))) return rc;
        HIP_TRY(hipMemsetAsync(b->d_dbg2.p, 0, L.np * 32, ctx->stream));
        ta.dbg = b->d_dbg2.as<unsigned long long>();
    }
    L.whole_only = L.zc && plan.n_tf + plan.n_res == L.np;
    if (L.whole_only) {
        const uint32_t slots = 1024;
        if (!ctx->d_hdr_ring.p || ctx->hdr_next >= slots) {
            if ((rc = ctx->d_hdr_ring.reserve((size_t)slots * 64))) return rc;
            HIP_TRY(hipMemsetAsync(ctx->d_hdr_ring.p, 0, (size_t)slots * 64, ctx->stream));
            ctx->hdr_next = 0;
        }
        ta.hdr = (ArenaHdr *)(ctx->d_hdr_ring.as<uint8_t>() + (size_t)ctx->hdr_next++ * 64);
    }
    return SWMI_OK;
}

static ResidentArgs resident_args(const swmi_batch *b) {
    const ChunkPlan &plan = b->plan;
    ResidentArgs xa;
    xa.res_items = plan.n_res ? b->d_res_items.as<uint32_t>() : nullptr;
    xa.n_res = (uint32_t)plan.n_res; xa.res_lds_words = plan.res_lds_words; xa.res_cell_cap = SWMI_RES_CELL_CAP; xa.res_ops_words = plan.res_ops_words;
    return xa;
}

static TFusedArgs tfused_args(const swmi_batch *b) {
    const ChunkPlan &plan = b->plan;
    TFusedArgs xt{};
    xt.items = plan.n_tf ? b->d_tf_items.as<uint32_t>() : nullptr;
    xt.n_items = (uint32_t)plan.n_tf;
    xt.cell_cap = 16;
    xt.tile_words = ((plan.tf_max_m + 63u + 15u) / 16u) * 64u * SWMI_TF_BR;
    xt.ref_words = (plan.tf_max_n + 3u) / 4u + 1u;
    xt.read_words = (plan.tf_max_m + 3u) / 4u + 1u;
    xt.stage_words = (plan.tf_max_path + 3u) / 4u + 1u + SWMI_EMIT_SCRATCH_WORDS;
    static const bool tf_marks = getenv("SWMI_DEBUG_MARKS") != nullptr;
    xt.debug_marks = tf_marks ? 1u : 0u;
    xt.lds_words = (xt.tile_words + 2u * xt.cell_cap + xt.stage_words + xt.ref_words + xt.read_words + 3u) & ~3u;
    static const int tf_helpers = getenv("SWMI_TF_HELPERS") ? atoi(getenv("SWMI_TF_HELPERS")) : 2;
    const uint64_t region = 4ull * xt.lds_words, budget = SWMI_LDS_BYTES - 4ull * 1024;
    const uint64_t left = budget > 4 * region ? budget - 4 * region : 0;
    xt.n_helpers = (uint32_t)std::min<uint64_t>((uint64_t)std::max(0, std::min(tf_helpers, (int)SWMI_TF_HELPERS)), region ? left / region : 0);
    return xt;
}

static inline AffRun aff_run(const swmi_batch *b) {
    const RunModes &md = b->opt.modes;
    AffRun r{};
    r.gap_open = b->gap_open;
    r.gap_open2 = md.gap_open2; r.gap2 = md.gap_open2 ? md.gap2 : 0;
    r.mode = md.kernel_mode();
    r.band = (uint32_t)md.band; r.xdrop = (uint32_t)md.xdrop; r.adapt = (uint32_t)md.band_adapt;
    r.mat = b->opt.mat ? b->d_mat.as<uint32_t>() : nullptr;
    r.nn = b->opt.mat ? b->opt.mat->n + 1u : 0u;
    r.cigar = (uint32_t)md.cigar;
    r.subopt = md.subopt;
    r.hits = (uint32_t)md.hits;
    r.end_bonus = (uint32_t)md.end_bonus;
    return r;
}

static int enqueue_launches(RunState &rs, Launch &L, const ResidentArgs &xa, const TFusedArgs &xt) {
    swmi_ctx *ctx = rs.ctx;
    swmi_batch *b = rs.b;
// ... 115 lines not shown
    const uint8_t *h = (const uint8_t *)b->h_result.p;
    ArenaHdr hdr_copy{};
    const ArenaHdr *hdr = (const ArenaHdr *)h;
    bool overflow = false;
    if (zc) {
        overflow = *(const volatile uint32_t *)h != 0u;
        if (overflow) {
            HIP_TRY(hipMemcpy(&hdr_copy, rs.ta.hdr, sizeof hdr_copy, hipMemcpyDeviceToHost));
            hdr = &hdr_copy;
        }
    }
    const uint64_t hdr_words = zc && !overflow ? 0 : hdr->reserved & SWMI_HDR_WORD_MASK;
    const uint64_t hdr_recs = zc && !overflow ? 0 : hdr->reserved >> SWMI_HDR_WORD_BITS;
    if (!zc) overflow = hdr_words > L.arena_cap || hdr_recs > L.tab_cap;
    if (overflow) {
        const size_t keep = np * (sizeof(PairOut) + (L.endb || L.hits ? L.sub_bytes() : 0));
        if (zc) {
            saved_outs.resize(keep);
            HIP_TRY(hipMemcpy(saved_outs.data(), L.res + result_out_off(), saved_outs.size(), hipMemcpyDeviceToHost));
        } else {
            saved_outs.assign(h + result_out_off(), h + result_out_off() + keep);
        }
        for (size_t k = 0; k < np; k++) {
            PairOut &so = ((PairOut *)saved_outs.data())[k];
            so.flags &= ~SWMI_F_ARENA_OVF;
            if (L.split && !(so.flags & SWMI_F_DEGENERATE)) { so.n_cells = 0; so.flags &= ~SWMI_F_CELL_OVF; }
        }
        L.arena_cap = std::max<uint64_t>(L.arena_cap, hdr_words + 1024);
        L.tab_cap = std::max<uint64_t>(L.tab_cap, hdr_recs + 64);
        if (L.arena_cap >= SWMI_HDR_WORD_MASK || L.tab_cap >= (1ull << (64u - SWMI_HDR_WORD_BITS)) - 1ull)
            return fail(SWMI_ERR_UNSUPPORTED, "one launch would hold %llu alignment records in %llu arena dwords: lower max_workspace_bytes so that the batch runs in smaller launches",
                        (unsigned long long)L.tab_cap, (unsigned long long)L.arena_cap);
        ctx->arena_words_per_pair = std::max<uint64_t>(ctx->arena_words_per_pair, L.arena_cap / np + 1);
        ctx->recs_per_pair_x16 = std::max<uint64_t>(ctx->recs_per_pair_x16, L.tab_cap * 16 / np + 1);
        retry = true;
        return SWMI_OK;
    }
    outs.assign((const PairOut *)(h + result_out_off()), (const PairOut *)(h + result_out_off()) + np);
    for (auto &o : outs) o.flags &= ~SWMI_F_ARENA_OVF;
    uint64_t n_rec = 0;
    if (zc) {
        for (auto &o : outs)
            if (!(o.flags & (SWMI_F_DEGENERATE | SWMI_F_CELL_OVF))) n_rec += o.n_cells;
    } else {
        n_rec = hdr_recs;
    }
    if (n_rec > L.tab_cap) return fail(SWMI_ERR_HIP, "more records than the table holds");
    const AlnRec *tab = (const AlnRec *)(h + L.t_off);
    const uint32_t *aw = (const uint32_t *)(h + L.a_off);
    if (!zc) {
        if (n_rec > L.copy_recs)
            HIP_TRY(hipMemcpy((uint8_t *)b->h_result.p + L.t_off + L.copy_recs * sizeof(AlnRec), L.res + L.t_off + L.copy_recs * sizeof(AlnRec),
                              (n_rec - L.copy_recs) * sizeof(AlnRec), hipMemcpyDeviceToHost));
        if (hdr_words > L.copy_words)
            HIP_TRY(hipMemcpy((uint8_t *)b->h_result.p + L.a_off + L.copy_words * 4, L.res + L.a_off + L.copy_words * 4,
                              (hdr_words - L.copy_words) * 4, hipMemcpyDeviceToHost));
        ctx->arena_copy_wpp = hdr_words * 5 / (4 * np) + 2;
        ctx->recs_per_pair_x16 = std::max<uint64_t>(ctx->recs_per_pair_x16, n_rec * 20 / np + 1);
    }
    if (rs.keep) {
        if ((rc = keep_chunk_records(rs, tab, n_rec, aw, L.arena_cap, L.lo))) return rc;
        rs.copyout_us += us_between(t_done, Clock::now());
    }
    return SWMI_OK;
}

static int fetch_windows(swmi_batch *b, const std::vector<Work> &work, size_t lo) {
    const ChunkPlan &plan = b->plan;
    if (b->eff_mode != 3 || !b->opt.modes.band_adapt || !plan.aff_n_long) return SWMI_OK;
    const size_t np = b->pairs_on_device.size() / sizeof(PairDesc);
    const PairDesc *pd = (const PairDesc *)b->pairs_on_device.data();
    const AffGeom g = aff_geom(b->opt.modes);
    if (b->win_at.size() != b->pairs.size()) b->win_at.assign(b->pairs.size(), 0);
    for (size_t k = np - plan.aff_n_long; k < np; k++) {
        const uint32_t pair = work[lo + pd[k].out_id].pair;
        const uint32_t m = b->read_desc[pd[k].read_id].len, n = b->ref_desc[pd[k].ref_id].len, ns = swmi_aff_strips(m);
        if (!b->win_at[pair]) { b->win_at[pair] = b->win_tab.size() + 1; b->win_tab.resize(b->win_tab.size() + ns, 0u); }
        HIP_TRY(hipMemcpy(b->win_tab.data() + (b->win_at[pair] - 1), b->d_dir.as<uint32_t>() + pd[k].dir_off + swmi_aff_pair_table_off(m, n, g),
                          (size_t)ns * sizeof(uint32_t), hipMemcpyDeviceToHost));
    }
    return SWMI_OK;
}

static int run_chunk(RunState &rs, const std::vector<Work> &work, size_t lo, size_t hi,
                     const std::vector<uint64_t> *cells_exact, std::vector<PairOut> &outs) {
    swmi_ctx *ctx = rs.ctx;
    swmi_batch *b = rs.b;
    const size_t np = hi - lo;
    int rc;
    if ((rc = prepare_chunk(rs, work, lo, hi, cells_exact))) return rc;
    const ChunkPlan &plan = b->plan;
    if (plan.seam_words) HIP_TRY(hipMemsetAsync(b->d_seam.p, 0, plan.seam_words * 4, ctx->stream));

    Launch L;
    L.np = np; L.lo = lo; L.cells_exact = cells_exact;
    if ((rc = size_cell_lists(rs, L))) return rc;
    {
        const uint64_t need = b->eff_mode == 3 ? 4ull * (SWMI_AFF_TILE_WORDS + ((uint64_t)plan.max_path + 15) / 16 + 1 + SWMI_EMIT_SCRATCH_WORDS)
                                               : traceback_lds_bytes(b->eff_mode, plan.max_path, plan.max_read);
        if (need > SWMI_LDS_BYTES)
            return fail(SWMI_ERR_UNSUPPORTED, "a pair of %u bases in total needs %llu bytes of LDS for the traceback (limit %u)",
                        plan.max_path, (unsigned long long)need, SWMI_LDS_BYTES);
    }
    L.split = rs.tb_split && !cells_exact && b->eff_mode == 1 && plan.n_windows < 0xFFFFFFFFull;
    L.zc = ctx->zero_copy != 0;
    L.sweep_only = ctx->scores_only != 0 && !cells_exact;
    L.time_all = ctx->profiling == 1;
    L.sub = b->eff_mode == 3 && b->opt.modes.subopt != 0;
    L.hits = L.sub ? (uint32_t)b->opt.modes.hits : 0u;
    L.endb = b->eff_mode == 3 && b->opt.modes.end_bonus != 0;

    const auto c0 = Clock::now();
    L.arena_cap = std::max<uint64_t>(np * ctx->arena_words_per_pair, 1024);
    L.tab_cap = std::max<uint64_t>(np * ctx->recs_per_pair_x16 / 16 + 64, 256);
    std::vector<uint8_t> saved_outs;
    for (L.attempt = 0;; L.attempt++) {
        if (L.attempt > 4) return fail(SWMI_ERR_HIP, "the record arena overflowed %d times in a row; results discarded", L.attempt);
        L.t_off = result_tab_off(np, L.sub_bytes()); L.a_off = result_arena_off(np, L.tab_cap, L.sub_bytes());
        if ((rc = b->d_result.reserve(L.a_off + L.arena_cap * 4))) return rc;
        L.res = b->d_result.as<uint8_t>();
        if (L.attempt > 0) {
            HIP_TRY(hipMemsetAsync(L.res, 0, 64, ctx->stream));
            HIP_TRY(hipMemcpyAsync(L.res + result_out_off(), saved_outs.data(), saved_outs.size(), hipMemcpyHostToDevice, ctx->stream));
        }
        if ((rc = build_fill_args(rs, L))) return rc;
        if ((rc = build_trace_args(rs, L))) return rc;
        if ((rc = enqueue_launches(rs, L, resident_args(b), tfused_args(b)))) return rc;
        static const char *watchdog = getenv("SWMI_DEBUG_WATCHDOG");
        if (watchdog) watchdog_wait(ctx->stream, b, watchdog);
        const auto c1 = Clock::now();
        if ((rc = wait_for_stream(ctx))) return rc;
        const auto c2 = Clock::now();
        volatile uint32_t *giveup = L.zc ? (volatile uint32_t *)b->h_result.p + 1 : (volatile uint32_t *)ctx->h_err.p + 5;
        if (*giveup != 0u) {
            const uint32_t code = *giveup;
            *giveup = 0u;
            return fail(SWMI_ERR_HIP, "sw_tfused_kernel: internal wait abandoned (code %08x); results discarded", code);
        }
        if (*(volatile uint32_t *)ctx->h_err.p != 0u) {
            *(volatile uint32_t *)ctx->h_err.p = 0u;
            if (rs.one_wave_sweep)
                return fail(SWMI_ERR_HIP, "the sweep raised its error flag without the strip pipeline; results discarded");
            rs.one_wave_sweep = true;
            b->timing.strip_fallbacks++;
            return run_chunk(rs, work, lo, hi, cells_exact, outs);
        }
        rs.enqueue_us += us_between(c0, c1);
        rs.wait_us += us_between(c1, c2);
        if (ctx->profiling) {
            float ms = 0;
            if (L.attempt == 0 || L.whole_only) { HIP_TRY(hipEventElapsedTime(&ms, ctx->ev[0], ctx->ev[1])); rs.fill_ms += ms; }
            if (L.time_all) { HIP_TRY(hipEventElapsedTime(&ms, ctx->ev[L.ext_timing ? 2 : 1], ctx->ev[3])); rs.tb_ms += ms; }
            if (L.time_all && !L.zc) { HIP_TRY(hipEventElapsedTime(&ms, ctx->ev[3], ctx->ev[4])); rs.d2h_ms += ms; }
        }
        if (rs.ta.dbg && (rc = dump_traceback_diagnostics(b, rs.ta, np, plan.n_tf))) return rc;
        if (rs.fa.dbg && L.attempt == 0 && (rc = dump_fill_diagnostics(b, rs.fa, np))) return rc;
        if (L.attempt == 0 && (rc = fetch_windows(b, work, lo))) return rc;
        if (L.sub) {
            const SuboptOut *hs = (const SuboptOut *)((const uint8_t *)b->h_result.p + result_sub_off(np));
            for (size_t k = 0; k < np; k++) b->sub[work[lo + k].pair] = hs[k];
        }
        if (L.hits) {
            const HitEnt *hh = (const HitEnt *)((const uint8_t *)b->h_result.p + result_hits_off(np));
            const size_t per = 1u + L.hits;
            for (size_t k = 0; k < np; k++) std::copy(hh + k * per, hh + (k + 1) * per, b->hitv.begin() + (size_t)work[lo + k].pair * per);
        }
        if (L.endb) {
            const EndOut *he = (const EndOut *)((const uint8_t *)b->h_result.p + result_sub_off(np));
            for (size_t k = 0; k < np; k++) b->endv[work[lo + k].pair] = he[k];
        }
        if (L.sweep_only) { collect_scores(b, work, L, outs); return SWMI_OK; }
        bool retry;
        if ((rc = collect_launch(rs, L, c2, saved_outs, outs, retry)) || !retry) return rc;
    }
}

static int check_band(const swmi_ctx *ctx, const swmi_batch *b, const swmi_params *p, const RunModes &md, uint64_t rows, int64_t S,
                      uint64_t max_n, int64_t go, int64_t ge) {
    const int align_mode = md.align_mode, band = md.band;
    const int64_t w = band;
    uint64_t min_n = UINT64_MAX, min_long = UINT64_MAX, max_m = 0;
    for (uint32_t r = 0; r < b->n_refs; r++)
        if (b->ref_desc[r].len) min_n = std::min<uint64_t>(min_n, b->ref_desc[r].len);
    for (uint32_t q = 0; q < b->n_reads; q++) {
        const uint64_t m = b->read_desc[q].len;
        if (m > SWMI_AFF_MAX_READ) min_long = std::min(min_long, m);
        max_m = std::max(max_m, m);
    }
    const int64_t last_lo = (int64_t)rows - SWMI_AFF_MAX_READ + 1 - w;
    if (!md.band_adapt && (int64_t)min_n < last_lo)
        return fail(SWMI_ERR_UNSUPPORTED, "band %d: the last strip of the longest read (%llu bases) starts at column %lld, past the end of the "
                    "shortest reference (%llu)", band, (unsigned long long)max_m, (long long)last_lo, (unsigned long long)min_n);
    const uint64_t min_rows = (uint64_t)SWMI_AFF_MAX_READ * swmi_aff_strips((uint32_t)min_long);
    if (align_mode == SWMI_ALIGN_GLOBAL && !md.extend && max_n > min_rows + (uint64_t)w)
        return fail(SWMI_ERR_UNSUPPORTED, "band %d, align_mode global: the end of the longest reference (%llu) lies outside the band of a read of "
                    "%llu bases (at most %llu)", band, (unsigned long long)max_n, (unsigned long long)min_long, (unsigned long long)(min_rows + w));
    if (align_mode != SWMI_ALIGN_LOCAL && (int64_t)rows * S > ((int64_t)1 << 29))
        return fail(SWMI_ERR_UNSUPPORTED, "band %d, align_mode fit / global: the longest read (%llu bases) is swept as %llu rows, and %llu * %lld (the "
                    "largest |score|) is above 2^29", band, (unsigned long long)max_m, (unsigned long long)rows, (unsigned long long)rows, (long long)S);
    if (md.band_adapt) {
        const int64_t low = swmi_adapt_low(max_m, max_n, ctx->gap_open, p->gap);
        if (!swmi_adapt_bound_ok(max_m, max_n, ctx->gap_open, p->gap))
            return fail(SWMI_ERR_UNSUPPORTED, "band %d, band_adapt: (2 * ceil(m / 1024) + 1) * gap_open + (1024 * ceil(m / 1024) + n) * gap = %lld for the "
                        "longest read (%llu) and reference (%llu) is below -2^30", band, (long long)low, (unsigned long long)max_m, (unsigned long long)max_n);
    } else if (align_mode == SWMI_ALIGN_GLOBAL) {
        const int64_t low = 3 * go + (int64_t)(rows + max_n) * ge;
        if (low < -((int64_t)1 << 30))
            return fail(SWMI_ERR_UNSUPPORTED, "band %d, align_mode global: 3 * gap_open + (1024 * ceil(m / 1024) + n) * gap = %lld for the longest "
                        "read (%llu) and reference (%llu) is below -2^30", band, (long long)low, (unsigned long long)max_m, (unsigned long long)max_n);
    }
    const uint64_t bytes = swmi_aff_pair_dir_words((uint32_t)max_m, (uint32_t)max_n, aff_geom(md)) * 4;
    if (bytes > ctx->max_workspace_bytes && md.two_piece())
        return fail(SWMI_ERR_UNSUPPORTED, "band %d, gap_open2: the two-plane direction field of the longest read (%llu) against the longest reference (%llu) "
                    "takes %llu bytes (twice the one-piece field), more than max_workspace_bytes (%llu)", band, (unsigned long long)max_m,
                    (unsigned long long)max_n, (unsigned long long)bytes, (unsigned long long)ctx->max_workspace_bytes);
    if (bytes > ctx->max_workspace_bytes)
        return fail(SWMI_ERR_UNSUPPORTED, "band %d: the direction field of the longest read (%llu) against the longest reference (%llu) takes %llu "
                    "bytes, more than max_workspace_bytes (%llu)", band, (unsigned long long)max_m, (unsigned long long)max_n,
                    (unsigned long long)bytes, (unsigned long long)ctx->max_workspace_bytes);
    return SWMI_OK;
}

static int check_run_params(const swmi_ctx *ctx, const swmi_batch *b, const swmi_params *p, bool affine, const RunOptions &opt) {
    const RunModes &md = opt.modes;
    const ScoreMatrix *mat = opt.mat.get();
    if (md.subopt != 0 && md.align_mode != SWMI_ALIGN_LOCAL)
        return fail(SWMI_ERR_UNSUPPORTED, "subopt = %d needs align_mode local (0), got align_mode %d", md.subopt, md.align_mode);
    if (md.hits != 0 && md.subopt == 0)
        return fail(SWMI_ERR_UNSUPPORTED, "hits = %d needs a run under subopt (the mask half-width, or -1), got subopt 0", md.hits);
    if (md.end_bonus != 0) {
        if (!(md.extend && md.align_mode == SWMI_ALIGN_GLOBAL))
            return fail(SWMI_ERR_UNSUPPORTED, "end_bonus = %d needs an extend run (align_mode global (2) with extend = 1), got align_mode %d, extend %d",
                        md.end_bonus, md.align_mode, md.extend);
        if (md.xdrop > 0) return fail(SWMI_ERR_UNSUPPORTED, "end_bonus = %d: the to-end score under xdrop is not supported (a stopped pair has no row m)", md.end_bonus);
        if (md.band_adapt) return fail(SWMI_ERR_UNSUPPORTED, "end_bonus = %d: the to-end score under band_adapt is not supported", md.end_bonus);
        if (md.two_piece()) return fail(SWMI_ERR_UNSUPPORTED, "end_bonus = %d: the to-end score with two-piece gaps (gap_open2) is not supported", md.end_bonus);
    }
    if (p->tie_mode != SWMI_TIE_SERIAL && p->tie_mode != SWMI_TIE_STRICT)
        return fail(SWMI_ERR_INVALID, "unknown tie_mode %d", p->tie_mode);
    if (p->types[0] == p->types[1] || p->types[0] == p->types[2] || p->types[1] == p->types[2])
        return fail(SWMI_ERR_UNSUPPORTED, "alignTypes a/i/d must be pairwise distinct");
    if (md.extend && md.align_mode != SWMI_ALIGN_GLOBAL)
        return fail(SWMI_ERR_UNSUPPORTED, "extend = 1 needs align_mode global (2), got align_mode %d", md.align_mode);
    if (md.xdrop > 0 && !(md.extend && md.align_mode == SWMI_ALIGN_GLOBAL))
        return fail(SWMI_ERR_UNSUPPORTED, "xdrop = %d needs an extend run (align_mode global (2) with extend = 1), got align_mode %d, extend %d",
                    md.xdrop, md.align_mode, md.extend);
    if (md.band_adapt && !(md.band > 0 && md.extend && md.align_mode == SWMI_ALIGN_GLOBAL))
        return fail(SWMI_ERR_UNSUPPORTED, "band_adapt = 1 needs a banded extend run (band > 0, align_mode global (2) with extend = 1), got band %d, "
                    "align_mode %d, extend %d", md.band, md.align_mode, md.extend);
    if (md.two_piece()) {
        if (md.align_mode != SWMI_ALIGN_GLOBAL)
            return fail(SWMI_ERR_UNSUPPORTED, "gap_open2 = %d needs align_mode global (2), with or without extend; got align_mode %d", md.gap_open2, md.align_mode);
        if (mat) return fail(SWMI_ERR_UNSUPPORTED, "gap_open2 = %d: two-piece gaps with a score matrix are not supported", md.gap_open2);
        if (md.xdrop > 0) return fail(SWMI_ERR_UNSUPPORTED, "gap_open2 = %d: two-piece gaps under xdrop are not supported", md.gap_open2);
        if (md.band_adapt) return fail(SWMI_ERR_UNSUPPORTED, "gap_open2 = %d: two-piece gaps under band_adapt are not supported", md.gap_open2);
    }
// ... 83 lines not shown
        rs0.ctx = ctx; rs0.b = b;
        rs0.tb_split = true;
        rs0.keep = false;
        std::vector<PairOut> o0;
        int rc = run_chunk(rs0, sample, 0, sample.size(), nullptr, o0);
        if (rc) return rc;
        uint64_t cells = 0, live = 0;
        for (auto &o : o0)
            if (!(o.flags & SWMI_F_DEGENERATE)) { cells += o.n_cells; live++; }
        if (live && cells * 100 >= (uint64_t)ctx->auto_ties_x100 * live) choice = 0;
        b->plan_key = PlanKey{};
        b->timing = swmi_timing{};
    }
    b->auto_choice = choice;
    b->auto_params = *p;
    return SWMI_OK;
}

static void build_schedule(const swmi_ctx *ctx, swmi_batch *b) {
    const SchedKey key(b->eff_mode, ctx->tfused == 1, b->opt.modes);
    if (b->work_key == key) return;
    const uint32_t n_refs = b->n_refs, n_reads = b->n_reads;
    b->work.clear();
    b->work.reserve(batch_n_pairs(b));
    b->work_cells = 0;
    std::vector<uint32_t> ro(b->paired ? 0u : n_refs), qo(b->paired ? 0u : n_reads);
    std::iota(ro.begin(), ro.end(), 0u);
    std::iota(qo.begin(), qo.end(), 0u);
    std::stable_sort(ro.begin(), ro.end(), [&](uint32_t a, uint32_t c) { return b->ref_desc[a].len > b->ref_desc[c].len; });
    std::stable_sort(qo.begin(), qo.end(), [&](uint32_t a, uint32_t c) { return b->read_desc[a].len > b->read_desc[c].len; });
    const bool refs_uniform = !ro.empty() && b->ref_desc[ro.front()].len == b->ref_desc[ro.back()].len;
    const bool aff = b->eff_mode == 3, tf = key.tfused;
    const AffGeom g = key.geom;
    auto seam_words = [aff, g](uint32_t m, uint32_t n) { return aff ? swmi_aff_pair_seam_words(m, n, g) : swmi_seam_words(m, n); };
    auto dir_words = [&](uint32_t m, uint32_t n) { return aff ? swmi_aff_pair_dir_words(m, n, g) : swmi_dir_words(m, n, b->eff_mode, tf); };
    auto add = [&](uint32_t r, uint32_t q, uint32_t n, uint32_t m, uint64_t dw, uint64_t sw) {
        Work w;
        w.pair = b->paired ? r : r * n_reads + q;
        w.cells = (uint64_t)m * n;
        w.dir_words = dw; w.seam_words = sw;
        b->work_cells += w.cells;
        b->work.push_back(w);
    };
    if (b->paired) {
        for (uint32_t k = 0; k < n_refs; k++) {
            const uint32_t m = b->read_desc[k].len, n = b->ref_desc[k].len;
            if (m && n) add(k, k, n, m, 0, 0);
        }
        std::stable_sort(b->work.begin(), b->work.end(), [](const Work &a, const Work &c) { return a.cells > c.cells; });
        uint32_t last_m = 0xFFFFFFFFu, last_n = 0xFFFFFFFFu;
        uint64_t dw = 0, sw = 0;
        for (Work &w : b->work) {
            const uint32_t m = b->read_desc[w.pair].len, n = b->ref_desc[w.pair].len;
            if (m != last_m || n != last_n) { dw = dir_words(m, n); sw = seam_words(m, n); last_m = m; last_n = n; }
            w.dir_words = dw; w.seam_words = sw;
        }
    } else if (refs_uniform) {
        for (uint32_t q : qo) {
            const uint32_t m = b->read_desc[q].len;
            if (m == 0) continue;
            const uint32_t n = n_refs ? b->ref_desc[ro[0]].len : 0;
            if (n == 0) break;
            const uint64_t dw = dir_words(m, n), sw = seam_words(m, n);
            for (uint32_t r : ro) add(r, q, n, m, dw, sw);
        }
    } else {
        uint32_t last_m = 0xFFFFFFFFu;
        uint64_t dw = 0, sw = 0;
        for (uint32_t r : ro) {
            const uint32_t n = b->ref_desc[r].len;
            if (n == 0) continue;
            last_m = 0xFFFFFFFFu;
            for (uint32_t q : qo) {
                const uint32_t m = b->read_desc[q].len;
                if (m == 0) continue;
                if (m != last_m) { dw = dir_words(m, n); sw = seam_words(m, n); last_m = m; }
                add(r, q, n, m, dw, sw);
            }
        }
    }
    b->work_key = key;
}

static size_t next_launch(const std::vector<Work> &work, size_t lo, uint64_t cap_bytes, uint64_t &words) {
    words = 0;
    size_t hi = lo;
    while (hi < work.size() && (hi == lo || (words + work[hi].dir_words) * 4 <= cap_bytes)) {
        words += work[hi].dir_words;
        hi++;
    }
    return hi;
}

static int rerun_overflowed(RunState &rs, const std::vector<Work> &work, const std::vector<size_t> &ovf, std::vector<PairOut> &outs) {
    swmi_batch *b = rs.b;
    int rc;
    if ((rc = settle_raw(b))) return rc;
    std::vector<Work> w2;
    std::vector<uint64_t> exact;
    for (size_t pos : ovf) { w2.push_back(work[pos]); exact.push_back(b->pairs[work[pos].pair].n_cells); }
    for (size_t lo = 0, hi; lo < w2.size(); lo = hi) {
        uint64_t words;
        hi = next_launch(w2, lo, rs.ctx->max_workspace_bytes, words);
        if ((rc = run_chunk(rs, w2, lo, hi, &exact, outs))) return rc;
        swmi_batch::RawChunk &rc2 = b->raw_chunks.back();
        rc2.wpos.resize(hi - lo);
        for (size_t k = 0; k < hi - lo; k++) rc2.wpos[k] = (uint32_t)ovf[lo + k];
        for (size_t k = 0; k < hi - lo; k++) b->pairs[w2[lo + k].pair].n_cells = outs[k].n_cells;
        for (size_t k = 0; k < hi - lo; k++)
            if (b->pairs[w2[lo + k].pair].strips != outs[k].flags >> SWMI_F_STRIPS_SHIFT)
                return fail(SWMI_ERR_HIP, "the exact-size re-run swept another number of strips");
        for (size_t k = 0; k < hi - lo; k++)
            if (outs[k].flags & SWMI_F_CELL_OVF)
                return fail(SWMI_ERR_HIP, "cell list overflowed again on the exact-size re-run");
    }
    b->timing.rerun_pairs = (uint32_t)ovf.size();
    return SWMI_OK;
}

static int batch_run(swmi_ctx *ctx, swmi_batch *b, const swmi_params *p, RunOptions opt) {
    if (!ctx || !b || !p) return fail(SWMI_ERR_INVALID, "null argument");
    std::lock_guard<std::mutex> g(ctx->mu);
    const bool affine = ctx->affine == 1 || ctx->gap_open != 0 || opt.mat != nullptr || opt.modes.align_mode != SWMI_ALIGN_LOCAL || opt.modes.band > 0 ||
                        opt.modes.cigar != 0 || opt.modes.subopt != 0;
    int rc;
    if ((rc = check_run_params(ctx, b, p, affine, opt))) return rc;
    static const bool host_dbg = getenv("SWMI_DEBUG_HOST") != nullptr;
    const auto h0 = Clock::now();
    {
        int cur = -1;
        if (hipGetDevice(&cur) != hipSuccess || cur != ctx->device) HIP_TRY(hipSetDevice(ctx->device));
    }
    b->params = *p;
    b->has_run = false;
    b->scores_only = ctx->scores_only != 0;

    const uint32_t n_refs = b->paired ? 0u : b->n_refs;
    b->pairs.assign(batch_n_pairs(b), PairRes{});
    b->win_tab.clear(); b->win_at.clear();
    b->has_sub = opt.modes.subopt != 0;
    b->sub.assign(b->has_sub ? batch_n_pairs(b) : 0, SuboptOut{0, 0u});
    b->hits_k = b->has_sub ? opt.modes.hits : 0;
    b->hitv.assign(b->hits_k ? batch_n_pairs(b) * (size_t)(1 + b->hits_k) : 0, HitEnt{0, 0u, 0u, 0u});
    b->has_endb = opt.modes.end_bonus != 0;
    b->endv.assign(b->has_endb ? batch_n_pairs(b) : 0, EndOut{0, 0, 0u});
    b->alns.clear(); b->str_at.clear();
    b->raw.clear(); b->rtab.clear(); b->raw_chunks.clear(); b->indexed = false;
    b->raw_ext = nullptr; b->rtab_ext = nullptr;
    if (b->views_built || b->ref_view_ready.size() != n_refs) {
        b->ref_view_ready.assign(n_refs, 0);
        b->ref_sites.assign(n_refs, {});
        b->ref_degenerate.assign(n_refs, 0);
        b->views_built = false;
    }
    b->timing = swmi_timing{};

    b->eff_mode = (ctx->mode == 1 && (p->mismatch > 0 || p->gap > 0)) ? 2u : ctx->mode;
    b->gap_open = ctx->gap_open;
    if (affine) b->eff_mode = 3;
    b->opt = std::move(opt);
    if (b->opt.mat && b->d_mat_gen != b->opt.mat->gen) {
        if ((rc = b->d_mat.reserve((size_t)swmi_aff_mat_words(SWMI_MAT_NN_MAX) * 4))) return rc;
        b->d_mat_gen = 0;
        HIP_TRY(hipMemcpyAsync(b->d_mat.p, b->opt.mat->image.data(), b->opt.mat->image.size() * 4, hipMemcpyHostToDevice, ctx->stream));
        HIP_TRY(hipStreamSynchronize(ctx->stream));
        b->d_mat_gen = b->opt.mat->gen;
    }
    if ((rc = choose_traceback_grain(ctx, b, p))) return rc;
    if (b->eff_mode == 0) {
        uint64_t max_m, max_n;
        longest_sequences(b, max_m, max_n);
        if (traceback_lds_bytes(0, path_bound(max_n, max_m, *p, p->match), max_m) > SWMI_LDS_BYTES)
            b->eff_mode = (p->mismatch > 0 || p->gap > 0) ? 2u : 1u;
    }
    build_schedule(ctx, b);
    const std::vector<Work> &work = b->work;
    const auto h1 = Clock::now();
    RunState rs;
    rs.ctx = ctx; rs.b = b;
    rs.tb_split = b->eff_mode == 1 &&
                  (ctx->tb_split == 1 || (ctx->tb_split < 0 && (work.size() < 64 || (work.size() <= 256 && b->auto_choice == 0 &&
                                                                                      memcmp(&b->auto_params, p, sizeof(swmi_params)) == 0))));
    b->tb_split_used = rs.tb_split;

    std::vector<PairOut> outs;
    std::vector<size_t> ovf;
    uint64_t dir_bytes = 0;
    for (size_t lo = 0, hi; lo < work.size(); lo = hi) {
        uint64_t words;
        hi = next_launch(work, lo, ctx->max_workspace_bytes, words);
        dir_bytes += words * 4;
        rs.defer_copy = lo == 0 && hi == work.size();
        rc = run_chunk(rs, work, lo, hi, nullptr, outs);
        rs.defer_copy = false;
        if (rc) return rc;
        for (size_t k = 0; k < hi - lo; k++) {
            PairRes &pr = b->pairs[work[lo + k].pair];
            pr.score = outs[k].score;
            pr.flags = ((outs[k].flags & SWMI_F_DEGENERATE) ? SWMI_PAIR_DEGENERATE : 0u) | ((outs[k].flags & SWMI_F_TO_END) ? SWMI_PAIR_TO_END : 0u);
            pr.n_cells = outs[k].n_cells;
            pr.strips = outs[k].flags >> SWMI_F_STRIPS_SHIFT;
            if (outs[k].flags & SWMI_F_CELL_OVF) ovf.push_back(lo + k);
        }
    }
    const auto h2 = Clock::now();
    if (!ovf.empty() && (rc = rerun_overflowed(rs, work, ovf, outs))) return rc;

    b->timing.fill_ms = rs.fill_ms; b->timing.traceback_ms = rs.tb_ms; b->timing.d2h_ms = rs.d2h_ms;
    b->timing.total_ms = rs.fill_ms + rs.tb_ms + rs.d2h_ms;
    b->timing.fill_launches = rs.launches;
    b->timing.cells = b->work_cells;
    b->timing.dir_bytes = dir_bytes;
    b->has_run = true;
    if (host_dbg)
        fprintf(stderr, "[swmi host] setup %.1f us, chunks (launch+wait+parse) %.1f us [prepare %.1f, its uploads %.1f, enqueue %.1f, wait %.1f, copy-out %.1f], grouping %.1f us\n",
                us_between(h0, h1), us_between(h1, h2), rs.prep_us, rs.prep_upload_us, rs.enqueue_us, rs.wait_us, rs.copyout_us, us_between(h2, Clock::now()));
    return SWMI_OK;
}

extern "C" int swmi_batch_run(swmi_ctx *ctx, swmi_batch *b, const swmi_params *p) {
    if (!ctx || !b || !p) return fail(SWMI_ERR_INVALID, "null argument");
    return batch_run(ctx, b, p, run_options(ctx));
}

static void swmi_worker_loop(swmi_ctx *ctx) {
    for (;;) {
        int st = 0;
        for (int spin = 0; spin < 4000 && (st = ctx->job_state.load(std::memory_order_acquire)) != 1 && st != 3; ++spin)
            __builtin_ia32_pause();
        if (st != 1 && st != 3) {
            std::unique_lock<std::mutex> lk(ctx->job_mu);
            ctx->job_cv.wait(lk, [&] { const int v = ctx->job_state.load(); return v == 1 || v == 3; });
            st = ctx->job_state.load();
        }
        if (st == 3) return;
        if (ctx->job_delay_us) std::this_thread::sleep_for(std::chrono::microseconds(ctx->job_delay_us));
        const int rc = batch_run(ctx, ctx->job_batch, &ctx->job_params, std::move(ctx->job_opt));
        ctx->job_rc = rc;
        ctx->job_err = rc ? swmi_last_error() : "";
        { std::lock_guard<std::mutex> lk(ctx->job_mu); ctx->job_state.store(2, std::memory_order_release); }
        ctx->job_cv.notify_all();
    }
}

extern "C" int swmi_batch_run_async(swmi_ctx *ctx, swmi_batch *b, const swmi_params *p) {
    if (!ctx || !b || !p) return fail(SWMI_ERR_INVALID, "null argument");
    if (ctx->job_state.load(std::memory_order_acquire) != 0)
        return fail(SWMI_ERR_INVALID, "a run is already in flight on this context: call swmi_batch_wait first");
    if (!ctx->worker.joinable()) ctx->worker = std::thread(swmi_worker_loop, ctx);
    ctx->job_batch = b;
    ctx->job_params = *p;
    ctx->job_opt = run_options(ctx);
    ctx->job_delay_us = ctx->dbg_async_delay_us;
    { std::lock_guard<std::mutex> lk(ctx->job_mu); ctx->job_state.store(1, std::memory_order_release); }
    ctx->job_cv.notify_all();
    return SWMI_OK;
}

extern "C" int swmi_batch_wait(swmi_ctx *ctx) {
    if (!ctx) return fail(SWMI_ERR_INVALID, "null argument");
    int st = ctx->job_state.load(std::memory_order_acquire);
    if (st == 0) return fail(SWMI_ERR_INVALID, "no run in flight on this context");
    for (int spin = 0; spin < 20000 && st != 2; ++spin) {
        __builtin_ia32_pause();
        st = ctx->job_state.load(std::memory_order_acquire);
    }
    if (st != 2) {
        std::unique_lock<std::mutex> lk(ctx->job_mu);
        ctx->job_cv.wait(lk, [&] { return ctx->job_state.load() == 2; });
    }
    const int rc = ctx->job_rc;
    const std::string err = ctx->job_err;
    ctx->job_state.store(0, std::memory_order_release);
    if (rc) return fail(rc, "%s", err.c_str());
    return SWMI_OK;
}

extern "C" int swmi_batch_mode(const swmi_batch *b, int *mode) {
    if (!b || !mode) return fail(SWMI_ERR_INVALID, "null argument");
    if (!b->has_run) return fail(SWMI_ERR_INVALID, "batch has no results (run it first)");
    *mode = (int)b->eff_mode;
    return SWMI_OK;
}

extern "C" int swmi_batch_timing(const swmi_batch *b, swmi_timing *t) {
    if (!b || !t) return fail(SWMI_ERR_INVALID, "null argument");
    *t = b->timing;
    return SWMI_OK;
}

extern "C" int swmi_align_batch(swmi_ctx *ctx, const swmi_params *p,
                                const uint8_t *ref_bytes, const uint64_t *ref_off, uint32_t n_refs,
                                const uint8_t *read_bytes, const uint64_t *read_off, uint32_t n_reads,
                                swmi_batch **out) {
    int rc = swmi_batch_upload(ctx, ref_bytes, ref_off, n_refs, read_bytes, read_off, n_reads, out);
    if (rc) return rc;
    rc = swmi_batch_run(ctx, *out, p);
    if (rc) { swmi_batch_free(ctx, *out); *out = nullptr; }
    return rc;
}
```

### sparksmithwaterman_amd/csrc/swmi_sweep.hip

```cpp
#include <hip/hip_runtime.h>
#include <hip/hip_ext.h>
#include <stdint.h>
#include <stdlib.h>
#include "swmi_device.h"
#include "swmi_launch.h"
#include "swmi_cells.h"

typedef uint32_t Words4 __attribute__((ext_vector_type(4)));
typedef const Words4 __attribute__((address_space(4))) *ConstWords4;

#define SWMI_PIPE_PUBLISH 2u
template <int R, bool ACGT, bool STRICT, bool MULTI, int MODE, bool PIPE = false>
__device__ __forceinline__ void fill_pair(const FillArgs &A, const PairDesc pd, const uint32_t lane, const uint32_t my_strip = 0u,
                                          const StripItem *item = nullptr) {
    const SeqDesc rd = A.refs[pd.ref_id];
    const SeqDesc qd = A.reads[pd.read_id];
    const uint32_t n_full = PIPE ? uni(rd.len) : rd.len, m = PIPE ? uni(qd.len) : qd.len;
    const uint32_t col0 = PIPE ? uni(item->col0) : 0u;
    const uint32_t g_lo = PIPE ? uni(item->g_lo) : 0u, g_hi = PIPE ? uni(item->g_hi) : 0xFFFFFFFFu;
    const uint32_t priv_stride = PIPE ? uni(item->priv_stride) : 0u;
    const uint32_t *__restrict__ refw = A.seqw + (PIPE ? uni(rd.boff) + (col0 >> 2) : rd.boff);
    const uint32_t *__restrict__ readw = A.seqw + qd.boff;
    const int match = A.match, mismatch = A.mismatch, gap = A.gap;
    constexpr uint32_t HMODE = MODE == SWMI_MODE_FIELD ? 0u : (MODE == SWMI_MODE_WINMAX ? 1u : 2u);
// ... 107 lines not shown
            const uint32_t tbg = tb + (col0 >> 4);
            const uint32_t gw = tbg / SWMI_CK_BLOCKS;
            if (MODE == SWMI_MODE_WINMAX && (tbg % SWMI_CK_BLOCKS) == 0u && tb > 0u) {
                if (gw > g_lo && gw <= g_hi) close_window(gw - 1u); else S.lmax = -1;
            }
            if ((MODE == SWMI_MODE_SCORE || MODE == SWMI_MODE_WINMAX) && (tbg % SWMI_CK_BLOCKS) == 0u && gw >= g_lo && gw < g_hi) {
                uint32_t *__restrict__ ck = wsp + (uint64_t)gw * (R + 2) * WAVE;
#pragma unroll
                for (int k = 0; k < R; ++k) ck[k * WAVE] = (uint32_t)S.h[k];
                ck[R * WAVE] = (uint32_t)S.nprev;
                ck[(R + 1) * WAVE] = (uint32_t)S.rb;
            }
            if (reads_seam && (tb & 3u) == 0u) {
                SWMI_SD(const unsigned long long dg1 = __builtin_amdgcn_s_memtime();)
                seam_grp = seam_grp_next;
                SWMI_SD(asm volatile("s_waitcnt vmcnt(0)" : "+v"(seam_grp) :: "memory"); dg_grp += __builtin_amdgcn_s_memtime() - dg1;)
            }
            if (reads_seam && (tb & 3u) == 2u) seam_grp_next = load_group(tb / 4u + 1u);
            const int seamv = reads_seam ? __builtin_amdgcn_ds_bpermute((int)(((tb & 3u) << 6) + ((lane & 15u) << 2)), seam_grp) : 0;
            const bool steady = (t0 + 1u >= lact) && (t0 + 15u < n);
            uint32_t *pub_slot = PIPE ? progress + s : nullptr;
            const uint32_t pub_val = (PIPE && feeds_seam && tb > 0u && (tb % SWMI_PIPE_PUBLISH) == 0u) ? tb : 0u;
            if (steady)
                fill_block16<R, ACGT, STRICT, MULTI, false, MODE, PIPE>(S, w, t0, lane, lane_eff, n, m, row0, gap, match, mismatch,
                                                                        seamv, reads_seam, feeds_seam, seam_out, cells, ccap,
                                                                        pub_slot, pub_val, seam_sh, own_lo, own_hi);
            else
                fill_block16<R, ACGT, STRICT, MULTI, true, MODE, PIPE>(S, w, t0, lane, lane_eff, n, m, row0, gap, match, mismatch,
                                                                       seamv, reads_seam, feeds_seam, seam_out, cells, ccap,
                                                                       pub_slot, pub_val, seam_sh, own_lo, own_hi);
            if (PIPE && feeds_seam && tb + 1u == nblk) {
                asm volatile("s_waitcnt vmcnt(0)" ::: "memory");
                if (lane == 0) __hip_atomic_store(progress + s, nblk, __ATOMIC_RELAXED, __HIP_MEMORY_SCOPE_AGENT);
            }

            if (MODE == SWMI_MODE_FIELD) {
                const int miss = (int)(t0 + 15u) - ((int)(lane + n) - 1);
#pragma unroll
                for (int k = 0; k < R; ++k) {
                    uint32_t v = S.acc[k];
                    if (miss > 0 && miss < 16) v <<= 2 * miss;
                    wsp[((uint64_t)tb * R + k) * WAVE] = v;
                }
            }
        }
        if (MODE == SWMI_MODE_WINMAX) {
            const uint32_t gl = (nblk - 1u + (col0 >> 4)) / SWMI_CK_BLOCKS;
            if (gl >= g_lo && gl < g_hi) close_window(gl);
        }
#ifdef SWMI_STRIP_DIAG
        if (PIPE && A.dbg && lane == 0 && s < 2u) {
            const unsigned long long tot = __builtin_amdgcn_s_memtime() - t_start;
            A.dbg[2 * pd.out_id + s] = s == 0u ? (tot << 32) | (S.dg_pub & 0xFFFFFFFFull)
                                               : (tot << 40) | ((dg_polls & 0xFFull) << 32) | ((dg_poll & 0xFFFFull) << 16) | (dg_grp & 0xFFFFull);
        }
#endif
        if (S.ev_prev != 0) {
            handle_pending<R>(S, S.h, 16u * nblk - 1u, lane_eff, n, row0, m, cells, ccap);
            S.ev_prev = 0;
        }
        if (MULTI) __threadfence();
    }

    if (PIPE) {
        if (lane == 0 && pair_max > 0) atomicMax(&A.out[pd.out_id].score, pair_max);
        return;
    }
    if (lane == 0) {
        PairOut o;
        if (MODE == SWMI_MODE_WINMAX) {
            if (pair_max <= 0) { o.score = 0; o.flags = SWMI_F_DEGENERATE; o.n_cells = (uint64_t)m * n_full; }
            else               { o.score = pair_max; o.flags = 0u; o.n_cells = 0; }
        } else if (S.cnt == 0) { o.score = 0; o.flags = SWMI_F_DEGENERATE; o.n_cells = (uint64_t)m * n_full; }
        else            { o.score = S.thr; o.flags = S.cnt > ccap ? SWMI_F_CELL_OVF : 0u; o.n_cells = S.cnt; }
        A.out[pd.out_id] = o;
        if (A.dbg) {
            A.dbg[2 * pd.out_id] = S.events;
            A.dbg[2 * pd.out_id + 1] = __builtin_amdgcn_s_memtime() - t_start;
        }
    }
}

template <int R, bool COLS>
__device__ __forceinline__ void sweep_fast(const FillArgs &A, const PairDesc pd, const uint32_t lane, const ColItem ci) {
    const SeqDesc rd = A.refs[pd.ref_id];
    const SeqDesc qd = A.reads[pd.read_id];
    const uint32_t n_full = rd.len, m = qd.len;
    const StripGeom G = strip_geom<R>(m, n_full, 1u);
    const uint32_t col0 = COLS ? ci.col0 : 0u;
    const uint32_t g_lo = COLS ? ci.g_lo : 0u, g_hi = COLS ? ci.g_hi : G.n_ck;
    const bool last = g_hi >= G.n_ck;
    const uint32_t n = (last ? n_full : 16u * SWMI_CK_BLOCKS * g_hi) - col0;
    const uint32_t *__restrict__ refw = A.seqw + rd.boff + (col0 >> 2);
    const uint32_t *__restrict__ readw = A.seqw + qd.boff;
    const uint32_t lact = m >= G.rps ? WAVE : (m + R - 1) / R;
    const uint32_t lane_eff = lane < lact ? lane : 0x40000000u;
    const uint32_t T = n + lact - 1;
    const uint32_t nblk = last ? (T + 15u) / 16u : n / 16u;
    const uint32_t gm = (uint32_t)(-(int64_t)A.gap);
    const int one = 1;
    int pair_max = 0;

    const unsigned long long dbg_t0 = A.dbg ? __builtin_amdgcn_s_memtime() : 0ull;
    SweepState<R> S;
    build_profiles<R>(S.q, readw, lane * R, m, A.match, A.mismatch);
#pragma unroll
    for (int k = 0; k < R; ++k) {
        S.h[k] = 0; S.g[k] = 0; S.hp[k] = 0;
    }
    S.lmax = -1;
    const uint4 *__restrict__ refq = reinterpret_cast<const uint4 *>(refw);
    uint4 wnext = refq[0];
    S.rby = 0;
    S.rbx = wave_shr1((int)(1u << (wnext.x & 31u)), 0);

    uint32_t *__restrict__ wsp = A.dir + pd.dir_off + lane;
    auto close_window = [&](uint32_t g) {
        const int wm = wave_max_i32(lane < lact ? S.lmax : -1);
        if (lane == 0) A.dir[pd.dir_off + G.wmax_off + g] = (uint32_t)wm;
        pair_max = pair_max > wm ? pair_max : wm;
        S.lmax = -1;
    };
    int steady_max = -1;
    bool closed = false;
    for (uint32_t tb = 0; tb < nblk; ++tb) {
        const uint32_t tbg = tb + (col0 >> 4);
        if ((tbg % SWMI_CK_BLOCKS) == 0u) {
            const uint32_t g = tbg / SWMI_CK_BLOCKS;
            if (tb > 0u && !closed) {
                if (g > g_lo) close_window(g - 1u); else S.lmax = -1;
            }
            closed = false;
#if !defined(SWMI_NO_ASM) && SWMI_CK_BLOCKS == 2u
            const uint32_t nwin = n > 16u * tb ? (n - 16u * tb) / 32u : 0u;
            if (g >= g_lo && nwin > 0u) {
                uint32_t cko = (g * (uint32_t)(R + 2) * WAVE + lane) * 4u;
                uint32_t wmo = ((uint32_t)G.wmax_off + g - 1u) * 4u;
                uint32_t rfo = tb * 16u;
                const uint32_t lact_s = uni(lact);
                int wm_last;
                uint32_t wx = wnext.x, wy = wnext.y, wz = wnext.z, ww = wnext.w;
                SweepWindowAsm<R>::run(S.h, S.g, S.hp, S.q, S.rbx, S.rby, wx, wy, wz, ww, one, gm, S.lmax, wm_last, steady_max,
                                       cko, wmo, rfo, uni64((uint64_t)(uintptr_t)(A.dir + pd.dir_off)), uni64((uint64_t)(uintptr_t)refq),
                                       lact_s >= WAVE ? ~0ull : (1ull << lact_s) - 1ull, uni(nwin - 1u));
                wnext = make_uint4(wx, wy, wz, ww);
                const int wm = wave_max_i32(wm_last);
                if (lane == 0) A.dir[pd.dir_off + G.wmax_off + g + nwin - 1u] = (uint32_t)wm;
                tb += 2u * nwin - 1u;
                closed = true;
                continue;
            }
#endif
            if (g >= g_lo) {
                uint32_t *__restrict__ ck = wsp + (uint64_t)g * (R + 2) * WAVE;
#pragma unroll
                for (int k = 0; k < R; ++k) ck[k * WAVE] = (uint32_t)S.h[k];
                ck[R * WAVE] = (uint32_t)wave_shr1_zero(S.g[R - 1]);
                ck[(R + 1) * WAVE] = (uint32_t)S.rby;
            }
        }
        const uint4 w = wnext;
        wnext = refq[tb + 1];
        const uint32_t t0 = 16u * tb;
#ifndef SWMI_NO_ASM
        if (t0 + 15u < n) {
            SweepStep4Asm<R>::run(S.h, S.g, S.hp, S.q, S.rbx, S.rby, w.x, w.y, one, gm, S.lmax);
            SweepStep4Asm<R>::run(S.h, S.g, S.hp, S.q, S.rbx, S.rby, w.y, w.z, one, gm, S.lmax);
            SweepStep4Asm<R>::run(S.h, S.g, S.hp, S.q, S.rbx, S.rby, w.z, w.w, one, gm, S.lmax);
            SweepStep4Asm<R>::run(S.h, S.g, S.hp, S.q, S.rbx, S.rby, w.w, wnext.x, one, gm, S.lmax);
        } else
#endif
        {
            sweep_tail_block<R>(S, w, wnext.x, t0, lane_eff, n, one, gm);
        }
    }
    if (!closed) {
        const uint32_t gl = (nblk - 1u + (col0 >> 4)) / SWMI_CK_BLOCKS;
        if (gl >= g_lo) close_window(gl);
    }
    {
        const int sm = wave_max_i32(steady_max);
        pair_max = pair_max > sm ? pair_max : sm;
    }
    if (lane != 0) return;
    if (A.dbg) {
        A.dbg[2 * pd.out_id] = (unsigned long long)__builtin_amdgcn_s_getreg((4 ) | (0 << 6) | (31 << 11)) |
                               ((unsigned long long)__builtin_amdgcn_s_getreg((20 ) | (0 << 6) | (31 << 11)) << 32);
        A.dbg[2 * pd.out_id + 1] = __builtin_amdgcn_s_memtime() - dbg_t0;
    }
    PairOut *o = &A.out[pd.out_id];
    if (COLS) {
        if (pair_max > 0) atomicMax(&o->score, pair_max);
        return;
    }
    PairOut v;
    if (pair_max <= 0) { v.score = 0; v.flags = SWMI_F_DEGENERATE; v.n_cells = (uint64_t)m * n_full; }
    else               { v.score = pair_max; v.flags = 0u; v.n_cells = 0; }
    *o = v;
}

template <bool COLS>
__device__ __forceinline__ void sweep_fast_dispatch(const FillArgs &A, const PairDesc pd, uint32_t lane, uint32_t m, const ColItem ci) {
    const uint32_t R = swmi_rows_per_lane(m);
    if (R == 1)      sweep_fast<1, COLS>(A, pd, lane, ci);
    else if (R == 2) sweep_fast<2, COLS>(A, pd, lane, ci);
    else if (R == 3) sweep_fast<3, COLS>(A, pd, lane, ci);
    else             sweep_fast<4, COLS>(A, pd, lane, ci);
}

template <bool ACGT, bool STRICT, int MODE>
__device__ __forceinline__ void fill_dispatch(const FillArgs &A, const PairDesc pd, uint32_t lane, uint32_t m) {
    const uint32_t R = swmi_rows_per_lane(m);
    if (R == 1)      fill_pair<1, ACGT, STRICT, false, MODE>(A, pd, lane);
    else if (R == 2) fill_pair<2, ACGT, STRICT, false, MODE>(A, pd, lane);
    else if (R == 3) fill_pair<3, ACGT, STRICT, false, MODE>(A, pd, lane);
    else if (m <= WAVE * SWMI_RMAX) fill_pair<SWMI_RMAX, ACGT, STRICT, false, MODE>(A, pd, lane);
    else             fill_pair<SWMI_RMAX, ACGT, STRICT, true, MODE>(A, pd, lane);
}

template <int MODE>
__device__ __forceinline__ void fill_entry(const FillArgs &A) {
    const uint32_t pair = blockIdx.x * FILL_WAVES + (threadIdx.x >> 6);
    if (pair >= A.n_pairs) return;
    const uint32_t lane = threadIdx.x & 63u;
    if (pair == 0 && lane == 0 && A.hdr) { A.hdr->reserved = 0; A.hdr->pad = 0; }
    if (pair == 0 && lane == 0 && A.q_reset) *A.q_reset = 0u;
    const PairDesc pd = A.pairs[pair];
    if (MODE == SWMI_MODE_WINMAX && (pd.pad & SWMI_PAD_RESIDENT)) return;
    const SeqDesc rd = A.refs[pd.ref_id];
    const SeqDesc qd = A.reads[pd.read_id];
    if (MODE == SWMI_MODE_WINMAX && A.skip_multi && qd.len > WAVE * SWMI_RMAX) {
        if (lane == 0) { PairOut z; z.score = 0; z.flags = 0u; z.n_cells = 0; A.out[pd.out_id] = z; }
        return;
    }
    const bool acgt = rd.acgt && qd.acgt &&
                      SWMI_SCORES_FIT(A);
    if (MODE == SWMI_MODE_WINMAX && qd.len <= WAVE * SWMI_RMAX && (pd.pad & SWMI_PAD_COLS)) {
        if (lane == 0) { PairOut z; z.score = 0; z.flags = 0u; z.n_cells = 0; A.out[pd.out_id] = z; }
        return;
    }
    if (MODE == SWMI_MODE_WINMAX && acgt && qd.len <= WAVE * SWMI_RMAX && A.gap <= 0) {
        sweep_fast_dispatch<false>(A, pd, lane, qd.len, ColItem{0u, 0u, 0u, 0u});
        return;
    }
    if (MODE == SWMI_MODE_SCORE || MODE == SWMI_MODE_WINMAX) {
        if (acgt) fill_dispatch<true, false, MODE>(A, pd, lane, qd.len);
        else      fill_dispatch<false, false, MODE>(A, pd, lane, qd.len);
    } else if (acgt) {
        if (A.strict) fill_dispatch<true, true, MODE>(A, pd, lane, qd.len);
        else          fill_dispatch<true, false, MODE>(A, pd, lane, qd.len);
    } else {
        if (A.strict) fill_dispatch<false, true, MODE>(A, pd, lane, qd.len);
        else          fill_dispatch<false, false, MODE>(A, pd, lane, qd.len);
    }
}

extern "C" __global__ void __launch_bounds__(WAVE * FILL_WAVES)
sw_fill_kernel(const FillArgs A) { fill_entry<SWMI_MODE_FIELD>(A); }

extern "C" __global__ void __launch_bounds__(WAVE * FILL_WAVES)
sw_fill_score_kernel(const FillArgs A) { fill_entry<SWMI_MODE_SCORE>(A); }

extern "C" __global__ void __launch_bounds__(WAVE * FILL_WAVES) __attribute__((amdgpu_waves_per_eu(4, 4)))
sw_sweep_winmax_kernel(const FillArgs A) { fill_entry<SWMI_MODE_WINMAX>(A); }

extern "C" __global__ void __launch_bounds__(WAVE * FILL_WAVES)
sw_sweep_winmax_strips_kernel(const FillArgs A) {
    const uint32_t item = blockIdx.x * FILL_WAVES + (threadIdx.x >> 6);
    if (item >= A.n_strip_items) return;
    const uint32_t lane = threadIdx.x & 63u;
    const StripItem *it = A.strip_items + item;
    const PairDesc pd = A.pairs[it->pair];
    const SeqDesc rd = A.refs[pd.ref_id];
    const SeqDesc qd = A.reads[pd.read_id];
    const bool acgt = rd.acgt && qd.acgt &&
                      SWMI_SCORES_FIT(A);
    const uint32_t strip = __builtin_amdgcn_readfirstlane(it->strip);
    if (acgt) fill_pair<SWMI_RMAX, true, false, true, SWMI_MODE_WINMAX, true>(A, pd, lane, strip, it);
    else      fill_pair<SWMI_RMAX, false, false, true, SWMI_MODE_WINMAX, true>(A, pd, lane, strip, it);
}

extern "C" __global__ void __launch_bounds__(WAVE * FILL_WAVES)
sw_sweep_winmax_cols_kernel(const FillArgs A) {
    const uint32_t item = blockIdx.x * FILL_WAVES + (threadIdx.x >> 6);
    if (item >= A.n_col_items) return;
    const uint32_t lane = threadIdx.x & 63u;
    const ColItem ci = A.col_items[item];
    const PairDesc pd = A.pairs[ci.pair];
    sweep_fast_dispatch<true>(A, pd, lane, A.reads[pd.read_id].len, ci);
}

static size_t spread_lds(uint32_t n_groups) {
    static const int on = getenv("SWMI_LDS_SPREAD") ? atoi(getenv("SWMI_LDS_SPREAD")) : 1;
    if (!on || n_groups == 0 || n_groups > 4u * 256u) return 0;
    const uint32_t per_cu = (n_groups + 255u) / 256u;
    return ((size_t)(160u * 1024u) / (per_cu + 1u) / 1024u + 1u) * 1024u;
}

extern "C" hipError_t swmi_launch_fill(const FillArgs *a, hipStream_t st, hipEvent_t ev_start, hipEvent_t ev_stop) {
    if (a->n_pairs == 0) return hipSuccess;
    static const bool attrs = [] {
        swmi_allow_big_lds(sw_fill_kernel); swmi_allow_big_lds(sw_fill_score_kernel); swmi_allow_big_lds(sw_sweep_winmax_kernel);
        swmi_allow_big_lds(sw_sweep_winmax_strips_kernel); swmi_allow_big_lds(sw_sweep_winmax_cols_kernel);
        return true;
    }();
    (void)attrs;
    const dim3 grid((a->n_pairs + FILL_WAVES - 1) / FILL_WAVES), block(WAVE * FILL_WAVES);
    const size_t lds = spread_lds(grid.x);
    if (a->mode == 0)      hipLaunchKernelGGL(sw_fill_kernel, grid, block, lds, st, *a);
    else if (a->mode == 1) {
        if (ev_start && ev_stop && !(a->skip_multi && a->n_strip_items) && !a->n_col_items) {
            hipExtLaunchKernelGGL(sw_sweep_winmax_kernel, grid, block, (uint32_t)lds, st, ev_start, ev_stop, 0u, *a);
            return hipGetLastError();
        }
        hipLaunchKernelGGL(sw_sweep_winmax_kernel, grid, block, a->n_col_items || a->n_strip_items ? 0 : lds, st, *a);
        if (a->skip_multi && a->n_strip_items) {
            const uint32_t g = (a->n_strip_items + FILL_WAVES - 1) / FILL_WAVES;
            hipLaunchKernelGGL(sw_sweep_winmax_strips_kernel, dim3(g), block, spread_lds(g), st, *a);
        }
        if (a->n_col_items) {
            const uint32_t g = (a->n_col_items + FILL_WAVES - 1) / FILL_WAVES;
            hipLaunchKernelGGL(sw_sweep_winmax_cols_kernel, dim3(g), block, spread_lds(g), st, *a);
        }
    }
    else                   hipLaunchKernelGGL(sw_fill_score_kernel, grid, block, lds, st, *a);
    return hipGetLastError();
}
```

### sparksmithwaterman_amd/csrc/swmi_traceback.hip

```cpp
#include <hip/hip_runtime.h>
#include <hip/hip_ext.h>
#include <stdint.h>
#include <stdlib.h>
#include "swmi_device.h"
#include "swmi_emit.h"
#include "swmi_launch.h"
#include "swmi_walk.h"

template <int R>
__device__ __forceinline__ void coop_helper(const TraceArgs &A, const PairDesc pd, const uint32_t lane, const uint32_t wave,
                                            const uint32_t nw, const uint32_t ts, const uint32_t n_waves_all,
                                            uint32_t *__restrict__ tiles, volatile uint32_t *__restrict__ shared) {
    const SeqDesc rd = A.refs[pd.ref_id];
    const SeqDesc qd = A.reads[pd.read_id];
    const uint32_t n = rd.len, m = qd.len;
    const uint32_t *__restrict__ refw = A.seqw + rd.boff;
    const uint32_t *__restrict__ readw = A.seqw + qd.boff;
    const StripGeom G = strip_geom<R>(m, n, 1u);
    const bool acgt = rd.acgt && qd.acgt && SWMI_SCORES_FIT(A);
    const uint32_t team = (wave - nw) % nw, q = 1u + (wave - nw) / nw;
    uint32_t last = 0;
    for (;;) {
        uint32_t seq;
        while ((seq = __hip_atomic_load(const_cast<uint32_t *>(&shared[7u + 4u * team]), __ATOMIC_RELAXED, __HIP_MEMORY_SCOPE_WORKGROUP)) == last)
// ... 75 lines not shown
        if (lane == 0) {
            po.n_cells = cnt;
            if (cnt > ccap) po.flags |= SWMI_F_CELL_OVF;
            A.out[pd.out_id] = po;
            if (A.out_host) A.out_host[pd.out_id] = po;
            shared[0] = cnt;
            shared[3] = staged;
        }
        if (lane < SWMI_TB_SLOTS) { shared[7u + 4u * lane] = 0u; shared[20u + lane] = 0u; }
        asm volatile("s_waitcnt vmcnt(0)" ::: "memory");
    };
    const uint64_t cbase = A.cells_off ? A.cells_off[pd.out_id] : (uint64_t)pd.out_id * A.cell_cap;
    uint2 *__restrict__ cells = const_cast<uint2 *>(A.cells) + cbase;

    const uint32_t seg = ccap / SWMI_TB_SLOTS;
    if (ncand >= 2u && ncand <= SWMI_TB_SLOTS && ncand <= n_waves && seg >= 1u) {
        const uint32_t nw = ncand, ts = n_waves / nw;
        if (wave < nw) {
            const uint32_t g = wave == 0u ? gc[0] : wave == 1u ? gc[1] : wave == 2u ? gc[2] : gc[3];
            const uint32_t nq0 = g + 1u < ts ? g + 1u : ts;
            const uint32_t wlo0 = (g + 1u - nq0) * SWMI_CK_BLOCKS;
            uint32_t *my = walker_lds + wave * per_walker;
            for (uint32_t w = lane; w < (m + 3u) / 4u; w += WAVE) my[A.lds_words + w] = readw[w];
            stage_ref(my + A.lds_words + A.lds_read_words, wlo0, nq0);
            const uint32_t c = replay_any<R, true, false>(A, pd, n, m, acgt, refw, readw, G, 0u, g * SWMI_CK_BLOCKS, lane,
                                                   tiles + wave * ts * WIN_WORDS + (nq0 - 1u) * SWMI_CK_BLOCKS * R * WAVE,
                                                   po.score, 0u, cells + wave * seg, seg);
            if (lane == 0) { shared[24u + wave] = c; shared[28u + wave] = wlo0; }
            asm volatile("s_waitcnt vmcnt(0)" ::: "memory");
        } else {
            const uint32_t team = (wave - nw) % nw, q = 1u + (wave - nw) / nw;
            const uint32_t g = team == 0u ? gc[0] : team == 1u ? gc[1] : team == 2u ? gc[2] : gc[3];
            const uint32_t nq0 = g + 1u < ts ? g + 1u : ts;
            if (q < nq0)
                (void)replay_any<R, false, false>(A, pd, n, m, acgt, refw, readw, G, 0u, (g - q) * SWMI_CK_BLOCKS, lane,
                                           tiles + team * ts * WIN_WORDS + (nq0 - 1u - q) * SWMI_CK_BLOCKS * R * WAVE,
                                           0, 0u, nullptr, 0u);
        }
        __syncthreads();
        bool one_each = true;
        for (uint32_t w = 0; w < nw; ++w) one_each = one_each && shared[24u + w] == 1u;
        if (one_each) {
            if (wave == 0) {
                uint2 c = make_uint2(0, 0);
                if (lane < nw) { c.x = ld_l2(&cells[lane * seg].x); c.y = ld_l2(&cells[lane * seg].y); }
                if (lane < nw) cells[lane] = c;
                publish(nw, 1u);
            }
            __syncthreads();
            return wave < nw ? shared[28u + wave] : 0xFFFFFFFFu;
        }
        __syncthreads();
    }

    const bool pre = ncand == 1u;
    const uint32_t nq0 = gc[0] + 1u < n_waves ? gc[0] + 1u : n_waves;
    const uint32_t wlo0 = (gc[0] + 1u - nq0) * SWMI_CK_BLOCKS;
    if (wave == 0) {
        if (n_waves == 1u) {
            for (uint32_t w = lane; w < (m + 3u) / 4u; w += WAVE) walker_lds[A.lds_words + w] = readw[w];
            if (pre) stage_ref(walker_lds + A.lds_words + A.lds_read_words, wlo0, nq0);
        }
        const uint32_t cnt = detect_cells<R, false>(A, pd, po, lane, pre ? tiles + (nq0 - 1u) * SWMI_CK_BLOCKS * R * WAVE : tiles);
        publish(cnt, (pre && cnt == 1u) ? 1u : 0u);
    } else {
        if (wave < SWMI_TB_SLOTS)
            for (uint32_t w = lane; w < (m + 3u) / 4u; w += WAVE) walker_lds[wave * per_walker + A.lds_words + w] = readw[w];
        if (wave == n_waves - 1u)
            for (uint32_t w = lane; w < (m + 3u) / 4u; w += WAVE) walker_lds[A.lds_words + w] = readw[w];
        if (pre) {
            if (wave < nq0)
                (void)replay_any<R, false, false>(A, pd, n, m, acgt, refw, readw, G, 0u, wlo0 + (wave - 1u) * SWMI_CK_BLOCKS, lane,
                                           tiles + (wave - 1u) * SWMI_CK_BLOCKS * R * WAVE, 0, 0u, nullptr, 0u);
            if (wave == n_waves - 1u) stage_ref(walker_lds + A.lds_words + A.lds_read_words, wlo0, nq0);
        }
    }
    __syncthreads();
    return (pre && wave == 0) ? wlo0 : 0xFFFFFFFFu;
}

extern "C" __global__ void __launch_bounds__(WAVE * SWMI_TB_WAVES) __attribute__((amdgpu_waves_per_eu(4, 4)))
sw_traceback_winmax_kernel(const TraceArgs A) {
    extern __shared__ uint32_t wm_lds[];
    const uint32_t pair = blockIdx.x;
    if (pair >= A.n_pairs) return;
    const uint32_t wave = threadIdx.x >> 6, lane = threadIdx.x & 63u;
    const PairDesc pd = A.pairs[pair];
    PairOut po = A.out[pd.out_id];
    if (finish_pair(A, pd, po) && wave == 0 && lane == 0) A.out[pd.out_id] = po;
    if (po.flags & (SWMI_F_DEGENERATE | SWMI_F_DONE)) {
        if (A.out_host && wave == 0 && lane == 0) A.out_host[pd.out_id] = po;
        return;
    }
    const uint32_t n_waves = blockDim.x >> 6;
    const uint32_t per_walker = A.lds_words + A.lds_read_words + SWMI_TB_REFWIN_WORDS;
    constexpr uint32_t WIN_WORDS = SWMI_CK_BLOCKS * SWMI_RMAX * WAVE;
    uint32_t *shared = wm_lds;
    uint32_t *tiles = wm_lds + 32;
    const uint32_t R = swmi_rows_per_lane(A.reads[pd.read_id].len);
    const uint32_t ccap = A.cells_cap ? A.cells_cap[pd.out_id] : A.cell_cap;
    const uint32_t tile_sets = A.pad2 ? 2u : 1u;
    uint32_t *tiles2 = A.pad2 ? tiles + n_waves * WIN_WORDS : nullptr;
    uint32_t *walker_lds0 = tiles + tile_sets * n_waves * WIN_WORDS;
    if (!swmi_common_pair(A, A.refs[pd.ref_id], A.reads[pd.read_id])) {
        if (wave == 0) {
            uint32_t c;
            if (R == 1)      c = detect_cells<1>(A, pd, po, lane, tiles);
            else if (R == 2) c = detect_cells<2>(A, pd, po, lane, tiles);
            else if (R == 3) c = detect_cells<3>(A, pd, po, lane, tiles);
            else             c = detect_cells<4>(A, pd, po, lane, tiles);
            if (lane == 0) {
                po.n_cells = c;
                if (c > ccap) po.flags |= SWMI_F_CELL_OVF;
                A.out[pd.out_id] = po;
                if (A.out_host) A.out_host[pd.out_id] = po;
                shared[0] = c;
            }
            asm volatile("s_waitcnt vmcnt(0)" ::: "memory");
        }
        __syncthreads();
        const uint32_t c = shared[0];
        uint32_t nwr = c < SWMI_TB_SLOTS ? c : SWMI_TB_SLOTS;
        if (nwr > n_waves) nwr = n_waves;
        if (c > ccap || wave >= nwr) return;
        po.n_cells = c;
        uint32_t *lds = walker_lds0 + wave * per_walker;
        uint32_t *tile = tiles + wave * WIN_WORDS;
        if (R == 1)      traceback_pair<1, 1, false>(A, pd, po, lane, wave, nwr, lds, tile, nullptr, 1u);
        else if (R == 2) traceback_pair<2, 1, false>(A, pd, po, lane, wave, nwr, lds, tile, nullptr, 1u);
        else if (R == 3) traceback_pair<3, 1, false>(A, pd, po, lane, wave, nwr, lds, tile, nullptr, 1u);
        else             traceback_pair<4, 1, false>(A, pd, po, lane, wave, nwr, lds, tile, nullptr, 1u);
        return;
    }
    uint32_t pre_wlo;
    if (R == 1)      pre_wlo = winmax_detect<1>(A, pd, po, lane, wave, n_waves, ccap, tiles, walker_lds0, per_walker, shared);
    else if (R == 2) pre_wlo = winmax_detect<2>(A, pd, po, lane, wave, n_waves, ccap, tiles, walker_lds0, per_walker, shared);
    else if (R == 3) pre_wlo = winmax_detect<3>(A, pd, po, lane, wave, n_waves, ccap, tiles, walker_lds0, per_walker, shared);
    else             pre_wlo = winmax_detect<4>(A, pd, po, lane, wave, n_waves, ccap, tiles, walker_lds0, per_walker, shared);
    const uint32_t cnt = shared[0];
    if (shared[3] != 1u) pre_wlo = 0xFFFFFFFFu;
    if (cnt > ccap || cnt == 0u) return;
    po.n_cells = cnt;
    uint32_t nw = cnt < SWMI_TB_SLOTS ? cnt : SWMI_TB_SLOTS;
    if (nw > n_waves) nw = n_waves;
    const uint32_t ts = n_waves / nw;
    if (ts == 1u) {
        if (wave >= nw) return;
        uint32_t *lds = walker_lds0 + wave * per_walker;
        uint32_t *tile = tiles + wave * WIN_WORDS;
        if (R == 1)      traceback_pair<1, 1, false, false>(A, pd, po, lane, wave, nw, lds, tile, nullptr, 1u, pre_wlo, true);
        else if (R == 2) traceback_pair<2, 1, false, false>(A, pd, po, lane, wave, nw, lds, tile, nullptr, 1u, pre_wlo, true);
        else if (R == 3) traceback_pair<3, 1, false, false>(A, pd, po, lane, wave, nw, lds, tile, nullptr, 1u, pre_wlo, true);
        else             traceback_pair<4, 1, false, false>(A, pd, po, lane, wave, nw, lds, tile, nullptr, 1u, pre_wlo, true);
        return;
    }
    if (wave < nw) {
        uint32_t *lds = walker_lds0 + wave * per_walker;
        uint32_t *tile = tiles + wave * ts * WIN_WORDS;
        uint32_t *tile2 = tiles2 ? tiles2 + wave * ts * WIN_WORDS : nullptr;
        if (R == 1)      traceback_pair<1, 1, true, false>(A, pd, po, lane, wave, nw, lds, tile, shared, ts, pre_wlo, true, nullptr, tile2);
        else if (R == 2) traceback_pair<2, 1, true, false>(A, pd, po, lane, wave, nw, lds, tile, shared, ts, pre_wlo, true, nullptr, tile2);
        else if (R == 3) traceback_pair<3, 1, true, false>(A, pd, po, lane, wave, nw, lds, tile, shared, ts, pre_wlo, true, nullptr, tile2);
        else             traceback_pair<4, 1, true, false>(A, pd, po, lane, wave, nw, lds, tile, shared, ts, pre_wlo, true, nullptr, tile2);
    } else {
        if (R == 1)      coop_helper<1>(A, pd, lane, wave, nw, ts, n_waves, tiles, shared);
        else if (R == 2) coop_helper<2>(A, pd, lane, wave, nw, ts, n_waves, tiles, shared);
        else if (R == 3) coop_helper<3>(A, pd, lane, wave, nw, ts, n_waves, tiles, shared);
        else             coop_helper<4>(A, pd, lane, wave, nw, ts, n_waves, tiles, shared);
// ... 254 lines not shown
                const uint32_t op = isA ? SWMI_DIR_A : (isI ? SWMI_DIR_I : SWMI_DIR_D);
                cur |= op << (2u * (nops & 15u));
                ++nops;
                if ((nops & 15u) == 0u) { if (nops <= max_ops) my_ops[(nops >> 4) - 1u] = cur; cur = 0; }
                i -= (isA || isI) ? 1u : 0u;
                j -= (isA || !isI) ? 1u : 0u;
                active = (int)score > 0 && i != 0u && j != 0u;
            }
        }
        if ((nops & 15u) != 0u && nops <= max_ops) my_ops[nops >> 4] = cur;
        WAVE_SYNC();
        const uint32_t opw = A.raw ? 0u : (nops + 15u) / 16u;
        const uint32_t words = mine ? swmi_payload_words(nops, A.raw != nullptr) : 0u;
        const uint32_t incl = wave_scan_add_u32(words);
        const uint32_t total = (uint32_t)__builtin_amdgcn_readlane((int)incl, 63);
        const uint32_t nhere = ncell - base < WAVE ? ncell - base : WAVE;
        unsigned long long off;
        uint32_t rslot;
        const bool fits = swmi_reserve(A, lane, total, nhere, off, rslot);
        const bool too_long = BALLOT(mine && nops > max_ops) != 0ull;
        if (fits && !too_long) {
            if (mine) {
                uint32_t *dst = A.arena + off + (incl - words);
                swmi_write_rec(A, rslot + lane, pd.out_id, SWMI_RANK_BY_CELL, begin, c0.x, c0.y, nops, off + (incl - words));
                for (uint32_t w = 0; w < opw; ++w) dst[w] = my_ops[w];
            }
            if (A.raw) {
                const uint8_t *__restrict__ raw_ref = A.raw + A.raw_off[pd.ref_id];
                const uint8_t *__restrict__ raw_read = A.raw + A.raw_off[A.raw_reads_at + pd.read_id];
                for (uint32_t a = 0; a < nhere; ++a) {
                    const uint32_t na = (uint32_t)__builtin_amdgcn_readlane((int)nops, (int)a);
                    const uint32_t at = (uint32_t)__builtin_amdgcn_readlane((int)(incl - words), (int)a);
                    const uint32_t ai = (uint32_t)__builtin_amdgcn_readlane((int)c0.x, (int)a);
                    const uint32_t aj = (uint32_t)__builtin_amdgcn_readlane((int)c0.y, (int)a);
                    swmi_emit_strings(A.arena + off + at, SwmiOpsPacked{opsb + a * X.res_ops_words},
                                      na, ai, aj, raw_ref, raw_read, lane, scratch);
                }
            }
        } else if (lane == 0) {
            atomicOr(&A.out[pd.out_id].flags, SWMI_F_ARENA_OVF);
            if (A.ovf_host) *A.ovf_host = 1u;
        }
        WAVE_SYNC();
    }
}

extern "C" __global__ void __launch_bounds__(WAVE * FILL_WAVES)
sw_resident_pairs_kernel(const TraceArgs A, const ResidentArgs X) {
    extern __shared__ uint32_t rp_lds[];
    const uint32_t wave = threadIdx.x >> 6, lane = threadIdx.x & 63u;
    const uint32_t item = blockIdx.x * FILL_WAVES + wave;
    if (item >= X.n_res) return;
    const PairDesc pd = A.pairs[X.res_items[item]];
    uint32_t *lds = rp_lds + wave * X.res_lds_words;
    const uint32_t R = swmi_rows_per_lane(A.reads[pd.read_id].len);
    if (A.strict) {
        if (R == 1)      resident_pair<1, true>(A, X, pd, lane, lds);
        else if (R == 2) resident_pair<2, true>(A, X, pd, lane, lds);
        else if (R == 3) resident_pair<3, true>(A, X, pd, lane, lds);
        else             resident_pair<4, true>(A, X, pd, lane, lds);
    } else {
        if (R == 1)      resident_pair<1, false>(A, X, pd, lane, lds);
        else if (R == 2) resident_pair<2, false>(A, X, pd, lane, lds);
        else if (R == 3) resident_pair<3, false>(A, X, pd, lane, lds);
        else             resident_pair<4, false>(A, X, pd, lane, lds);
    }
}

extern "C" hipError_t swmi_launch_resident(const TraceArgs *a, const ResidentArgs *x, hipStream_t st) {
    if (x->n_res == 0) return hipSuccess;
    static const bool attr = [] { swmi_allow_big_lds(sw_resident_pairs_kernel); return true; }();
    (void)attr;
    hipLaunchKernelGGL(sw_resident_pairs_kernel, dim3((x->n_res + FILL_WAVES - 1) / FILL_WAVES), dim3(WAVE * FILL_WAVES),
                       (size_t)FILL_WAVES * x->res_lds_words * sizeof(uint32_t), st, *a, *x);
    return hipGetLastError();
}

extern "C" hipError_t swmi_launch_traceback(const TraceArgs *a, hipStream_t st, hipEvent_t ev_start, hipEvent_t ev_stop) {
    if (a->n_pairs == 0) return hipSuccess;
    const size_t tile = (size_t)(a->mode == 0 ? SWMI_TB_BLOCKS : SWMI_CK_BLOCKS) * SWMI_RMAX * WAVE;
    const size_t per_wave = (size_t)a->lds_words + a->lds_read_words + SWMI_TB_REFWIN_WORDS + tile;
    const dim3 block(WAVE * FILL_WAVES);
    if (a->mode == 1) {
        static int forced = getenv("SWMI_TB_WAVES") ? atoi(getenv("SWMI_TB_WAVES")) : 0;
        static int big = getenv("SWMI_TB_BIG") ? atoi(getenv("SWMI_TB_BIG")) : 10000;
        const uint32_t n_waves = forced ? (uint32_t)forced : (a->n_pairs <= 512u ? SWMI_TB_WAVES : a->n_pairs <= (uint32_t)big ? 4u : 1u);
        const size_t n_walkers = n_waves < SWMI_TB_SLOTS ? n_waves : SWMI_TB_SLOTS;
        const size_t tiles = (size_t)n_waves * SWMI_CK_BLOCKS * SWMI_RMAX * WAVE;
        size_t words = 32 + tiles + n_walkers * ((size_t)a->lds_words + a->lds_read_words + SWMI_TB_REFWIN_WORDS);
        static const int spec_opt = getenv("SWMI_TB_SPEC") ? atoi(getenv("SWMI_TB_SPEC")) : 1;
        TraceArgs t = *a;
        t.pad2 = (spec_opt && (spec_opt == 2 || a->n_pairs <= 384u) && n_waves > 1u && (words + tiles) * sizeof(uint32_t) <= 160u * 1024u) ? 1u : 0u;
        if (t.pad2) words += tiles;
        if (ev_start && ev_stop)
            hipExtLaunchKernelGGL(sw_traceback_winmax_kernel, dim3(a->n_pairs), dim3(WAVE * n_waves), (uint32_t)(words * sizeof(uint32_t)), st, ev_start, ev_stop, 0u, t);
        else
            hipLaunchKernelGGL(sw_traceback_winmax_kernel, dim3(a->n_pairs), dim3(WAVE * n_waves), words * sizeof(uint32_t), st, t);
    } else {
        const dim3 grid((a->n_pairs + FILL_WAVES - 1) / FILL_WAVES, SWMI_TB_SLOTS);
        if (a->mode == 0) hipLaunchKernelGGL(sw_traceback_kernel, grid, block, per_wave * FILL_WAVES * sizeof(uint32_t), st, *a);
        else              hipLaunchKernelGGL(sw_traceback_replay_kernel, grid, block, per_wave * FILL_WAVES * sizeof(uint32_t), st, *a);
    }
    return hipGetLastError();
}
```

Before: 2516.

## Order traceback blocks by predicted cost class from fill kernel

The fill kernel now puts each pair into one of 16 classes, keyed by its max score and by whether the max occurs in several windows. It appends the pair index to per-class lists with atomics. The winmax traceback kernel then maps blockIdx through a prefix scan over the class counts, so the expensive pairs (multiple candidates, high score) are scheduled first to reduce tail imbalance. The cost is extra fill-side work (reading the window-max array, a ballot, an atomic per pair), extra workspace per pair, and an indirection at traceback start.

```diff
diff --git a/include/swmi.h b/include/swmi.h
--- a/include/swmi.h
+++ b/include/swmi.h
@@ -86,6 +86,7 @@
 } swmi_timing;
 int  swmi_batch_timing(const swmi_batch *b, swmi_timing *t);
 int  swmi_batch_mode(const swmi_batch *b, int *mode);
+int  swmi_batch_tb_ordered(const swmi_batch *b, int *ordered);
 
 #define SWMI_PAIR_DEGENERATE 0x1u
 #define SWMI_PAIR_TO_END     0x2u
diff --git a/sparksmithwaterman_amd/_capi.py b/sparksmithwaterman_amd/_capi.py
--- a/sparksmithwaterman_amd/_capi.py
+++ b/sparksmithwaterman_amd/_capi.py
@@ -81,6 +81,7 @@
     ("swmi_batch_free", None, [_P, _P]),
     ("swmi_batch_timing", C.c_int, [_P, C.POINTER(Timing)]),
     ("swmi_batch_mode", C.c_int, [_P, C.POINTER(C.c_int)]),
+    ("swmi_batch_tb_ordered", C.c_int, [_P, C.POINTER(C.c_int)]),
     ("swmi_batch_n_pairs", C.c_uint64, [_P]),
     ("swmi_pair_score", C.c_int, [_P, C.c_uint64, C.POINTER(C.c_int32)]),
     ("swmi_pair_n_alignments", C.c_int, [_P, C.c_uint64, _u64p, C.POINTER(C.c_uint32)]),
diff --git a/sparksmithwaterman_amd/aligner.py b/sparksmithwaterman_amd/aligner.py
--- a/sparksmithwaterman_amd/aligner.py
+++ b/sparksmithwaterman_amd/aligner.py
@@ -175,6 +175,11 @@
         check(self._lib.swmi_batch_mode(self._h, C.byref(v)))
         return v.value
 
+    def tb_ordered(self):
+        v = C.c_int()
+        check(self._lib.swmi_batch_tb_ordered(self._h, C.byref(v)))
+        return bool(v.value)
+
     def score(self, pair):
         v = C.c_int32()
         check(self._lib.swmi_pair_score(self._h, pair, C.byref(v)))
diff --git a/sparksmithwaterman_amd/csrc/swmi_ctx.cpp b/sparksmithwaterman_amd/csrc/swmi_ctx.cpp
--- a/sparksmithwaterman_amd/csrc/swmi_ctx.cpp
+++ b/sparksmithwaterman_amd/csrc/swmi_ctx.cpp
@@ -141,6 +141,9 @@
     } else if (!strcmp(name, "tb_split")) {
         if (value < -1 || value > 1) return fail(SWMI_ERR_INVALID, "tb_split must be -1 (automatic), 0 or 1");
         ctx->tb_split = (int)value;
+    } else if (!strcmp(name, "tb_order")) {
+        if (value < -1 || value > 1) return fail(SWMI_ERR_INVALID, "tb_order must be -1 (automatic), 0 or 1");
+        ctx->tb_order = (int)value;
     } else if (!strcmp(name, "col_chunks")) {
         if (value < 0 || value > 4096) return fail(SWMI_ERR_INVALID, "col_chunks out of range");
         ctx->col_chunks = (uint32_t)value;
diff --git a/sparksmithwaterman_amd/csrc/swmi_device.h b/sparksmithwaterman_amd/csrc/swmi_device.h
--- a/sparksmithwaterman_amd/csrc/swmi_device.h
+++ b/sparksmithwaterman_amd/csrc/swmi_device.h
@@ -94,6 +94,11 @@
 };
 #define SWMI_HDR_WORD_BITS 36u
 #define SWMI_HDR_WORD_MASK ((1ull << SWMI_HDR_WORD_BITS) - 1ull)
+
+#define SWMI_ORD_CLASSES    16u
+#define SWMI_ORD_CNT_STRIDE 16u
+#define SWMI_ORD_SET_WORDS  (SWMI_ORD_CLASSES * SWMI_ORD_CNT_STRIDE)
+SWMI_HD static inline uint64_t swmi_order_words(uint64_t n_pairs) { return 2ull * SWMI_ORD_SET_WORDS + (uint64_t)SWMI_ORD_CLASSES * n_pairs; }
 
 struct FillArgs {
     const uint32_t *seqw;
@@ -125,6 +130,11 @@
     uint32_t        n_col_items;
     uint32_t        strip_spins;
     uint32_t       *q_reset;
+    uint32_t       *order;
+    uint32_t        ord_set;
+    int32_t         ord_key_lo;
+    uint32_t        ord_key_shift;
+    uint32_t        ord_pad;
 };
 
 struct TraceArgs {
@@ -156,12 +166,13 @@
     uint32_t       *q_count;
     uint4          *q_items;
     uint32_t        q_cap;
-    uint32_t        pad4;
+    uint32_t        ord_set;
     const uint8_t  *raw;
     const uint64_t *raw_off;
     uint32_t        raw_reads_at;
     uint32_t        rec_tab_cap;
     AlnRec         *rec_tab;
+    uint32_t       *order;
 };
 
 struct ResidentArgs {
diff --git a/sparksmithwaterman_amd/csrc/swmi_diag.cpp b/sparksmithwaterman_amd/csrc/swmi_diag.cpp
--- a/sparksmithwaterman_amd/csrc/swmi_diag.cpp
+++ b/sparksmithwaterman_amd/csrc/swmi_diag.cpp
@@ -57,6 +57,29 @@
     for (int c = 0; c < 4; c++)
         if (cn[c]) fprintf(stderr, "[swmi tb dbg]   %d%s alignment(s): %zu pairs, wave ticks mean=%.0f max=%llu, walk(slot 0) mean=%.0f\n",
                            c + 1, c == 3 ? "+" : "", cn[c], cs[c] / cn[c], cm[c], cw[c] / cn[c]);
+    std::vector<int> cls(np, -1);
+    if (ta.order) {
+        std::vector<uint32_t> ob(swmi_order_words(np));
+        HIP_TRY(hipMemcpy(ob.data(), ta.order, ob.size() * 4, hipMemcpyDeviceToHost));
+        for (uint32_t c = 0; c < SWMI_ORD_CLASSES; c++) {
+            const uint32_t n = std::min<uint32_t>(ob[ta.ord_set * SWMI_ORD_SET_WORDS + c * SWMI_ORD_CNT_STRIDE], (uint32_t)np);
+            double t = 0; unsigned long long tm = 0;
+            for (uint32_t k = 0; k < n; k++) {
+                const uint32_t p = ob[2u * SWMI_ORD_SET_WORDS + c * np + k];
+                if (p >= np) continue;
+                cls[p] = (int)c; t += d[4 * p]; tm = std::max(tm, d[4 * p]);
+            }
+            if (n) fprintf(stderr, "[swmi tb dbg]   class %2u: %u pairs, wave ticks mean=%.0f max=%llu\n", c, n, t / n, tm);
+        }
+    }
+    if (const char *path = getenv("SWMI_DEBUG_FILL_TABLE")) {
+        if (FILE *f = fopen(path, "w")) {
+            fprintf(f, "pair class score alignments ticks\n");
+            for (size_t k = 0; k < np; k++)
+                fprintf(f, "%zu %d %d %llu %llu\n", k, cls[k], po_dbg[k].score, (unsigned long long)po_dbg[k].n_cells, d[4 * k]);
+            fclose(f);
+        }
+    }
     return SWMI_OK;
 }
 
diff --git a/sparksmithwaterman_amd/csrc/swmi_host.h b/sparksmithwaterman_amd/csrc/swmi_host.h
--- a/sparksmithwaterman_amd/csrc/swmi_host.h
+++ b/sparksmithwaterman_amd/csrc/swmi_host.h
@@ -151,6 +151,9 @@
     uint32_t auto_ties_x100 = 300;
     uint32_t col_chunks = 0;
     int tb_split = -1;
+    int tb_order = -1;
+    bool ord_range = false;
+    int32_t ord_smin = 0, ord_smax = 0;
     bool ext_events = false;
     int tfused = -1;
     int resident = -1;
@@ -265,6 +268,10 @@
     DevBuf d_win_off, d_queue;
     DevBuf d_tf_items;
     DevBuf d_res_items;
+    DevBuf d_order;
+    uint32_t ord_next = 0;
+    bool ord_clean = false;
+    bool tb_ordered = false;
     bool views_built = false;
     bool tb_split_used = false;
     bool acgt_known = false;
diff --git a/sparksmithwaterman_amd/csrc/swmi_launch.h b/sparksmithwaterman_amd/csrc/swmi_launch.h
--- a/sparksmithwaterman_amd/csrc/swmi_launch.h
+++ b/sparksmithwaterman_amd/csrc/swmi_launch.h
@@ -1,6 +1,7 @@
 #pragma once
 #include <hip/hip_runtime.h>
 #include <stdint.h>
+#include <stdlib.h>
 #include "swmi_device.h"
 
 template <class K>
@@ -10,6 +11,11 @@
 
 extern "C" hipError_t swmi_launch_fill(const FillArgs *a, hipStream_t st, hipEvent_t ev_start, hipEvent_t ev_stop);
 extern "C" hipError_t swmi_launch_traceback(const TraceArgs *a, hipStream_t st, hipEvent_t ev_start, hipEvent_t ev_stop);
+static inline uint32_t swmi_tb_group_waves(uint32_t n_pairs, uint32_t max_waves) {
+    static const int forced = getenv("SWMI_TB_WAVES") ? atoi(getenv("SWMI_TB_WAVES")) : 0;
+    static const int big = getenv("SWMI_TB_BIG") ? atoi(getenv("SWMI_TB_BIG")) : 10000;
+    return forced ? (uint32_t)forced : (n_pairs <= 512u ? max_waves : n_pairs <= (uint32_t)big ? 4u : 1u);
+}
 extern "C" hipError_t swmi_launch_traceback_split(const TraceArgs *a, uint32_t n_windows, hipStream_t st);
 extern "C" hipError_t swmi_launch_resident(const TraceArgs *a, const ResidentArgs *x, hipStream_t st);
 extern "C" hipError_t swmi_launch_tfused(const TraceArgs *a, const TFusedArgs *x, hipStream_t st);
diff --git a/sparksmithwaterman_amd/csrc/swmi_run.cpp b/sparksmithwaterman_amd/csrc/swmi_run.cpp
--- a/sparksmithwaterman_amd/csrc/swmi_run.cpp
+++ b/sparksmithwaterman_amd/csrc/swmi_run.cpp
@@ -38,6 +38,10 @@
     bool split = false;
     bool zc = false;
     bool sweep_only = false;
+    bool ordered = false;
+    uint32_t ord_set = 0;
+    int32_t ord_key_lo = 0;
+    uint32_t ord_key_shift = 0;
     bool sub = false;
     bool endb = false;
     uint32_t hits = 0;
@@ -128,6 +132,8 @@
     L.q_cap = std::min<uint64_t>(std::max<uint64_t>(L.cells_total, 1), 1ull << 24);
     if (L.split && (rc = b->d_queue.reserve(256 + L.q_cap * sizeof(uint4)))) return rc;
     fa.q_reset = L.split ? b->d_queue.as<uint32_t>() : nullptr;
+    fa.order = L.ordered ? b->d_order.as<uint32_t>() : nullptr;
+    fa.ord_set = L.ord_set; fa.ord_key_lo = L.ord_key_lo; fa.ord_key_shift = L.ord_key_shift; fa.ord_pad = 0;
     return SWMI_OK;
 }
 
@@ -156,7 +162,8 @@
     ta.out_host = nullptr;
     ta.ovf_host = (uint32_t *)ctx->h_err.dp + 4;
     ((volatile uint32_t *)ctx->h_err.p)[4] = 0u; ((volatile uint32_t *)ctx->h_err.p)[5] = 0u;
-    ta.win_off = nullptr; ta.q_count = nullptr; ta.q_items = nullptr; ta.q_cap = 0; ta.pad4 = 0;
+    ta.win_off = nullptr; ta.q_count = nullptr; ta.q_items = nullptr; ta.q_cap = 0;
+    ta.order = L.ordered ? b->d_order.as<uint32_t>() : nullptr; ta.ord_set = L.ord_set;
     const int cigar = b->eff_mode == 3 ? b->opt.modes.cigar : 0;
     const bool strings = !cigar && ctx->device_strings != 0 && b->d_raw.p != nullptr;
     ta.raw = strings ? b->d_raw.as<uint8_t>() : nullptr;
@@ -438,6 +445,44 @@
     return SWMI_OK;
 }
 
+static int prepare_order(RunState &rs, Launch &L) {
+    swmi_ctx *ctx = rs.ctx;
+    swmi_batch *b = rs.b;
+    const ChunkPlan &plan = b->plan;
+    const bool plain = b->eff_mode == 1 && !L.split && !L.cells_exact && !L.sweep_only && !plan.n_strip_items && !plan.n_col_items &&
+                       !plan.n_res && !plan.n_tf && L.np < (1u << 27);
+    L.ordered = plain && ctx->tb_order != 0 &&
+                (ctx->tb_order == 1 || (uint64_t)L.np * swmi_tb_group_waves((uint32_t)L.np, 8u) > 4u * 1024u);
+    if (!L.cells_exact) b->tb_ordered = L.ordered;
+    if (!L.ordered) return SWMI_OK;
+    int rc;
+    const void *was = b->d_order.p;
+    if ((rc = b->d_order.reserve(swmi_order_words(L.np) * 4))) return rc;
+    if (b->d_order.p != was) b->ord_clean = false;
+    if (!b->ord_clean) {
+        HIP_TRY(hipMemsetAsync(b->d_order.p, 0, 2u * SWMI_ORD_SET_WORDS * sizeof(uint32_t), ctx->stream));
+        b->ord_next = 0;
+    }
+    L.ord_set = b->ord_next;
+    b->ord_clean = false;
+    const int64_t lo = ctx->ord_range ? ctx->ord_smin : 0;
+    const int64_t hi = ctx->ord_range ? ctx->ord_smax : (int64_t)plan.max_read * std::max(b->params.match, 0);
+    L.ord_key_lo = (int32_t)lo;
+    L.ord_key_shift = 0;
+    while (((hi - lo) >> L.ord_key_shift) > (int64_t)SWMI_ORD_CLASSES - 2) L.ord_key_shift++;
+    return SWMI_OK;
+}
+
+static void finish_order(RunState &rs, const std::vector<PairOut> &outs) {
+    swmi_ctx *ctx = rs.ctx;
+    rs.b->ord_next ^= 1u;
+    rs.b->ord_clean = true;
+    int32_t smin = INT32_MAX, smax = INT32_MIN;
+    for (const PairOut &o : outs)
+        if (!(o.flags & SWMI_F_DEGENERATE)) { smin = std::min(smin, o.score); smax = std::max(smax, o.score); }
+    if (smin <= smax) { ctx->ord_range = true; ctx->ord_smin = smin; ctx->ord_smax = smax; }
+}
+
 static int run_chunk(RunState &rs, const std::vector<Work> &work, size_t lo, size_t hi,
                      const std::vector<uint64_t> *cells_exact, std::vector<PairOut> &outs) {
     swmi_ctx *ctx = rs.ctx;
@@ -465,6 +510,7 @@
     L.sub = b->eff_mode == 3 && b->opt.modes.subopt != 0;
     L.hits = L.sub ? (uint32_t)b->opt.modes.hits : 0u;
     L.endb = b->eff_mode == 3 && b->opt.modes.end_bonus != 0;
+    if ((rc = prepare_order(rs, L))) return rc;
 
     const auto c0 = Clock::now();
     L.arena_cap = std::max<uint64_t>(np * ctx->arena_words_per_pair, 1024);
@@ -527,7 +573,9 @@
         }
         if (L.sweep_only) { collect_scores(b, work, L, outs); return SWMI_OK; }
         bool retry;
-        if ((rc = collect_launch(rs, L, c2, saved_outs, outs, retry)) || !retry) return rc;
+        if ((rc = collect_launch(rs, L, c2, saved_outs, outs, retry)) || retry) { if (rc) return rc; continue; }
+        if (L.ordered) finish_order(rs, outs);
+        return SWMI_OK;
     }
 }
 
@@ -777,10 +825,10 @@
     b->work_key = key;
 }
 
-static size_t next_launch(const std::vector<Work> &work, size_t lo, uint64_t cap_bytes, uint64_t &words) {
+static size_t next_launch(const std::vector<Work> &work, size_t lo, uint64_t cap_bytes, uint64_t &words, uint64_t pair_words = 0) {
     words = 0;
     size_t hi = lo;
-    while (hi < work.size() && (hi == lo || (words + work[hi].dir_words) * 4 <= cap_bytes)) {
+    while (hi < work.size() && (hi == lo || (words + work[hi].dir_words + (hi - lo + 1) * pair_words) * 4 <= cap_bytes)) {
         words += work[hi].dir_words;
         hi++;
     }
@@ -877,13 +925,16 @@
                   (ctx->tb_split == 1 || (ctx->tb_split < 0 && (work.size() < 64 || (work.size() <= 256 && b->auto_choice == 0 &&
                                                                                       memcmp(&b->auto_params, p, sizeof(swmi_params)) == 0))));
     b->tb_split_used = rs.tb_split;
+    b->tb_ordered = false;
+    const uint64_t ord_pair_words = b->eff_mode == 1 && !rs.tb_split && !ctx->scores_only &&
+                                    (ctx->tb_order == 1 || (ctx->tb_order < 0 && work.size() > 1024u)) ? SWMI_ORD_CLASSES : 0u;
 
     std::vector<PairOut> outs;
     std::vector<size_t> ovf;
     uint64_t dir_bytes = 0;
     for (size_t lo = 0, hi; lo < work.size(); lo = hi) {
         uint64_t words;
-        hi = next_launch(work, lo, ctx->max_workspace_bytes, words);
+        hi = next_launch(work, lo, ctx->max_workspace_bytes, words, ord_pair_words);
         dir_bytes += words * 4;
         rs.defer_copy = lo == 0 && hi == work.size();
         rc = run_chunk(rs, work, lo, hi, nullptr, outs);
@@ -978,6 +1029,13 @@
     return SWMI_OK;
 }
 
+extern "C" int swmi_batch_tb_ordered(const swmi_batch *b, int *ordered) {
+    if (!b || !ordered) return fail(SWMI_ERR_INVALID, "null argument");
+    if (!b->has_run) return fail(SWMI_ERR_INVALID, "batch has no results (run it first)");
+    *ordered = b->tb_ordered ? 1 : 0;
+    return SWMI_OK;
+}
+
 extern "C" int swmi_batch_timing(const swmi_batch *b, swmi_timing *t) {
     if (!b || !t) return fail(SWMI_ERR_INVALID, "null argument");
     *t = b->timing;
diff --git a/sparksmithwaterman_amd/csrc/swmi_sweep.hip b/sparksmithwaterman_amd/csrc/swmi_sweep.hip
--- a/sparksmithwaterman_amd/csrc/swmi_sweep.hip
+++ b/sparksmithwaterman_amd/csrc/swmi_sweep.hip
@@ -213,7 +213,7 @@
 }
 
 template <int R, bool COLS>
-__device__ __forceinline__ void sweep_fast(const FillArgs &A, const PairDesc pd, const uint32_t lane, const ColItem ci) {
+__device__ __forceinline__ uint32_t sweep_fast(const FillArgs &A, const PairDesc pd, const uint32_t lane, const ColItem ci) {
     const SeqDesc rd = A.refs[pd.ref_id];
     const SeqDesc qd = A.reads[pd.read_id];
     const uint32_t n_full = rd.len, m = qd.len;
@@ -313,7 +313,20 @@
         const int sm = wave_max_i32(steady_max);
         pair_max = pair_max > sm ? pair_max : sm;
     }
-    if (lane != 0) return;
+    uint32_t cls = 0u;
+    if (!COLS && A.order && pair_max > 0) {
+        asm volatile("s_waitcnt vmcnt(0)" ::: "memory");
+        const uint32_t *__restrict__ wm = A.dir + pd.dir_off + G.wmax_off;
+        uint32_t ncand = 0u;
+        for (uint32_t g0 = 0; g0 < G.n_ck; g0 += WAVE) {
+            const uint32_t g = g0 + lane;
+            const int wv = g < G.n_ck ? (int)ld_l2(wm + g) : -1;
+            ncand += (uint32_t)__builtin_popcountll(BALLOT(wv == pair_max));
+        }
+        const int key = (pair_max - A.ord_key_lo) >> A.ord_key_shift;
+        cls = ncand >= 2u ? SWMI_ORD_CLASSES - 1u : (uint32_t)(key < 0 ? 0 : key > (int)SWMI_ORD_CLASSES - 2 ? (int)SWMI_ORD_CLASSES - 2 : key);
+    }
+    if (lane != 0) return cls;
     if (A.dbg) {
         A.dbg[2 * pd.out_id] = (unsigned long long)__builtin_amdgcn_s_getreg((4 ) | (0 << 6) | (31 << 11)) |
                                ((unsigned long long)__builtin_amdgcn_s_getreg((20 ) | (0 << 6) | (31 << 11)) << 32);
@@ -322,21 +335,28 @@
     PairOut *o = &A.out[pd.out_id];
     if (COLS) {
         if (pair_max > 0) atomicMax(&o->score, pair_max);
-        return;
+        return 0u;
     }
     PairOut v;
     if (pair_max <= 0) { v.score = 0; v.flags = SWMI_F_DEGENERATE; v.n_cells = (uint64_t)m * n_full; }
     else               { v.score = pair_max; v.flags = 0u; v.n_cells = 0; }
     *o = v;
+    return cls;
 }
 
 template <bool COLS>
-__device__ __forceinline__ void sweep_fast_dispatch(const FillArgs &A, const PairDesc pd, uint32_t lane, uint32_t m, const ColItem ci) {
+__device__ __forceinline__ uint32_t sweep_fast_dispatch(const FillArgs &A, const PairDesc pd, uint32_t lane, uint32_t m, const ColItem ci) {
     const uint32_t R = swmi_rows_per_lane(m);
-    if (R == 1)      sweep_fast<1, COLS>(A, pd, lane, ci);
-    else if (R == 2) sweep_fast<2, COLS>(A, pd, lane, ci);
-    else if (R == 3) sweep_fast<3, COLS>(A, pd, lane, ci);
-    else             sweep_fast<4, COLS>(A, pd, lane, ci);
+    if (R == 1)      return sweep_fast<1, COLS>(A, pd, lane, ci);
+    else if (R == 2) return sweep_fast<2, COLS>(A, pd, lane, ci);
+    else if (R == 3) return sweep_fast<3, COLS>(A, pd, lane, ci);
+    else             return sweep_fast<4, COLS>(A, pd, lane, ci);
+}
+
+__device__ __forceinline__ void order_append(const FillArgs &A, const uint32_t lane, const uint32_t cls, const uint32_t pair) {
+    if (lane != 0) return;
+    const uint32_t idx = atomicAdd(A.order + A.ord_set * SWMI_ORD_SET_WORDS + cls * SWMI_ORD_CNT_STRIDE, 1u);
+    if (idx < A.n_pairs) A.order[2u * SWMI_ORD_SET_WORDS + cls * A.n_pairs + idx] = pair;
 }
 
 template <bool ACGT, bool STRICT, int MODE>
@@ -356,6 +376,8 @@
     const uint32_t lane = threadIdx.x & 63u;
     if (pair == 0 && lane == 0 && A.hdr) { A.hdr->reserved = 0; A.hdr->pad = 0; }
     if (pair == 0 && lane == 0 && A.q_reset) *A.q_reset = 0u;
+    if (MODE == SWMI_MODE_WINMAX && pair == 0 && lane < SWMI_ORD_CLASSES && A.order)
+        A.order[(A.ord_set ^ 1u) * SWMI_ORD_SET_WORDS + lane * SWMI_ORD_CNT_STRIDE] = 0u;
     const PairDesc pd = A.pairs[pair];
     if (MODE == SWMI_MODE_WINMAX && (pd.pad & SWMI_PAD_RESIDENT)) return;
     const SeqDesc rd = A.refs[pd.ref_id];
@@ -371,12 +393,14 @@
         return;
     }
     if (MODE == SWMI_MODE_WINMAX && acgt && qd.len <= WAVE * SWMI_RMAX && A.gap <= 0) {
-        sweep_fast_dispatch<false>(A, pd, lane, qd.len, ColItem{0u, 0u, 0u, 0u});
+        const uint32_t cls = sweep_fast_dispatch<false>(A, pd, lane, qd.len, ColItem{0u, 0u, 0u, 0u});
+        if (A.order) order_append(A, lane, cls, pair);
         return;
     }
     if (MODE == SWMI_MODE_SCORE || MODE == SWMI_MODE_WINMAX) {
         if (acgt) fill_dispatch<true, false, MODE>(A, pd, lane, qd.len);
         else      fill_dispatch<false, false, MODE>(A, pd, lane, qd.len);
+        if (MODE == SWMI_MODE_WINMAX && A.order) order_append(A, lane, 0u, pair);
     } else if (acgt) {
         if (A.strict) fill_dispatch<true, true, MODE>(A, pd, lane, qd.len);
         else          fill_dispatch<true, false, MODE>(A, pd, lane, qd.len);
diff --git a/sparksmithwaterman_amd/csrc/swmi_traceback.hip b/sparksmithwaterman_amd/csrc/swmi_traceback.hip
--- a/sparksmithwaterman_amd/csrc/swmi_traceback.hip
+++ b/sparksmithwaterman_amd/csrc/swmi_traceback.hip
@@ -181,8 +181,19 @@
 extern "C" __global__ void __launch_bounds__(WAVE * SWMI_TB_WAVES) __attribute__((amdgpu_waves_per_eu(4, 4)))
 sw_traceback_winmax_kernel(const TraceArgs A) {
     extern __shared__ uint32_t wm_lds[];
-    const uint32_t pair = blockIdx.x;
+    uint32_t pair = blockIdx.x;
     if (pair >= A.n_pairs) return;
+    if (A.order) {
+        const uint32_t l = threadIdx.x & 63u;
+        const uint32_t v = l < SWMI_ORD_CLASSES ? A.order[A.ord_set * SWMI_ORD_SET_WORDS + (SWMI_ORD_CLASSES - 1u - l) * SWMI_ORD_CNT_STRIDE] : 0u;
+        const uint32_t incl = wave_scan_add_u32(v);
+        const uint64_t hit = BALLOT(l < SWMI_ORD_CLASSES && blockIdx.x < incl);
+        if (hit == 0ull) return;
+        const uint32_t k = (uint32_t)__builtin_ctzll(hit);
+        const uint32_t before = (uint32_t)__builtin_amdgcn_readlane((int)(incl - v), (int)k);
+        pair = uni(A.order[2u * SWMI_ORD_SET_WORDS + (SWMI_ORD_CLASSES - 1u - k) * A.n_pairs + (blockIdx.x - before)]);
+        if (pair >= A.n_pairs) return;
+    }
     const uint32_t wave = threadIdx.x >> 6, lane = threadIdx.x & 63u;
     const PairDesc pd = A.pairs[pair];
     PairOut po = A.out[pd.out_id];
@@ -603,9 +614,7 @@
     const size_t per_wave = (size_t)a->lds_words + a->lds_read_words + SWMI_TB_REFWIN_WORDS + tile;
     const dim3 block(WAVE * FILL_WAVES);
     if (a->mode == 1) {
-        static int forced = getenv("SWMI_TB_WAVES") ? atoi(getenv("SWMI_TB_WAVES")) : 0;
-        static int big = getenv("SWMI_TB_BIG") ? atoi(getenv("SWMI_TB_BIG")) : 10000;
-        const uint32_t n_waves = forced ? (uint32_t)forced : (a->n_pairs <= 512u ? SWMI_TB_WAVES : a->n_pairs <= (uint32_t)big ? 4u : 1u);
+        const uint32_t n_waves = swmi_tb_group_waves(a->n_pairs, SWMI_TB_WAVES);
         const size_t n_walkers = n_waves < SWMI_TB_SLOTS ? n_waves : SWMI_TB_SLOTS;
         const size_t tiles = (size_t)n_waves * SWMI_CK_BLOCKS * SWMI_RMAX * WAVE;
         size_t words = 32 + tiles + n_walkers * ((size_t)a->lds_words + a->lds_read_words + SWMI_TB_REFWIN_WORDS);
```

New measurement: 2581, median of 6. +2.6%, better.
